# TrungMasterChef/CSWin-SimAM-UNet

Hardware: AMD Instinct MI355X
Metric: images/sec at 512×512 bf16, 1/2/4/8 MI355X; Dice parity vs reference (higher is better)
Workload: dtype bf16; 1 GPU; CSWin-UNet train step 512x512 depth [1, 2, 9, 1] split [1, 2, 8, 8] +SimAM, AdamW; model=CSWinTransformer, params=23567980, global_batch=16, per_gpu_batch=16, img=512, parallelism=dp1, workload_key=cswin|d1,2,9,1|s1,2,8,8|simam|bf16|512|16

## Files before the change

### cswin-simam-unet_amd/csrc/conv.hip

```cpp
#include <cstdlib>

#include "common.hpp"
#include "lds_dma.hpp"

namespace csu {
namespace {

constexpr int NT = 256;
constexpr int TBM = 64, TBN = 64, TBK = 32;

template <typename T> struct CT;
template <> struct CT<bf16> { static constexpr int AS = TBK; };
template <> struct CT<float> { static constexpr int AS = TBK + 4; };

__device__ __forceinline__ int cswz(int row, int col) {
    return row * TBK + ((((col >> 3) ^ (row >> 2)) & 3) << 3) + (col & 7);
}

struct Geo {
    int B, H, W, C, OH, OW, N, KH, KW, s, p;
};

template <int MODE>
__device__ __forceinline__ long gather_index(const Geo& g, long m, int k, long Mrows) {
// ... 1630 lines not shown
    if (!dy || !w_ihwo || !dx) return fail(CSU_E_ARG, "conv2d_dgrad: null buffer");
    const Geo g = to_geo(gm);
    const long M = (long)g.B * g.H * g.W;
    const int K = g.KH * g.KW * g.N;
    const bool vec = g.N % 8 == 0;
    hipStream_t st = as_stream(stream);
    if (dtype == CSU_BF16 && g.N % 4 == 0) {
        IG ph[4];
        int np = 0;
        for (int py = 0; py < g.s; ++py)
            for (int px = 0; px < g.s; ++px) {
                const IG ig = ig_dgrad_phase(*gm, py, px);
                if (ig.M == 0) continue;
                if (np == 4) {
                    if (int e = launch_ig(ph, np, dy, w_ihwo, bias, dx, st, cfg)) return e;
                    np = 0;
                }
                ph[np++] = ig;
            }
        if (np == 1) return launch_ig(ph, 1, dy, w_ihwo, bias, dx, st, cfg, (float*)ws, ws_bytes);
        return np ? launch_ig(ph, np, dy, w_ihwo, bias, dx, st, cfg) : 0;
    }
    if (cfg > 0) return fail(CSU_E_ARG, "conv2d_dgrad: igemm_dma needs bf16 with N % 64 == 0");
    if (dtype == CSU_BF16) return launch_gemm<bf16, 1>(g, M, g.C, K, dy, w_ihwo, bias, dx, vec, st);
    if (dtype == CSU_F32) return launch_gemm<float, 1>(g, M, g.C, K, dy, w_ihwo, bias, dx, vec, st);
    return fail(CSU_E_ARG, "conv2d_dgrad: bad dtype");
}

extern "C" int csu_conv2d_fwd(const csu_conv_geom* gm, int dtype, const void* x, const void* w_ohwi, const float* bias,
                              void* out, void* stream) {
    return conv_fwd_impl(gm, dtype, x, w_ohwi, bias, out, -1, stream);
}

extern "C" int csu_conv2d_dgrad(const csu_conv_geom* gm, int dtype, const void* dy, const void* w_ihwo,
                                const float* bias, void* dx, void* stream) {
    return conv_dgrad_impl(gm, dtype, dy, w_ihwo, bias, dx, -1, stream);
}

extern "C" size_t csu_conv2d_workspace(int op, const csu_conv_geom* gm, int dtype) {
    if (check_geo(gm) || dtype != CSU_BF16 || (op != 0 && op != 1)) return 0;
    if (op == 0) {
        if (gm->C % 4) return 0;
        const IG g = ig_forward(*gm);
        return id_pick(g, true) >= 0 ? 0 : ksplit_bytes(g, id_cus());
    }
    if (gm->N % 4 || gm->stride != 1) return 0;
    const IG g = ig_dgrad_phase(*gm, 0, 0);
    return id_pick(g, true) >= 0 ? 0 : ksplit_bytes(g, id_cus());
}

extern "C" int csu_conv2d_fwd_ws(const csu_conv_geom* gm, int dtype, const void* x, const void* w_ohwi, const float* bias,
                                 void* out, void* workspace, size_t ws_bytes, void* stream) {
    return conv_fwd_impl(gm, dtype, x, w_ohwi, bias, out, -1, stream, workspace, ws_bytes);
}

extern "C" int csu_conv2d_dgrad_ws(const csu_conv_geom* gm, int dtype, const void* dy, const void* w_ihwo, const float* bias,
                                   void* dx, void* workspace, size_t ws_bytes, void* stream) {
    return conv_dgrad_impl(gm, dtype, dy, w_ihwo, bias, dx, -1, stream, workspace, ws_bytes);
}

extern "C" int csu_conv2d_ex(int op, const csu_conv_geom* gm, int dtype, const void* src, const void* w, const float* bias,
                             void* out, int cfg, void* stream) {
    if (op == 0) return conv_fwd_impl(gm, dtype, src, w, bias, out, cfg, stream);
    if (op == 1) return conv_dgrad_impl(gm, dtype, src, w, bias, out, cfg, stream);
    return fail(CSU_E_ARG, "conv2d_ex: op must be 0 (forward) or 1 (input gradient)");
}

extern "C" size_t csu_conv2d_wgrad_workspace(const csu_conv_geom* gm) {
    if (check_geo(gm)) return 0;
    const size_t a = wgrad_ws(gm, -1);
    const int pk = wd_pick(gm, CSU_BF16, -1);
    const size_t b = pk >= 0 ? wgrad_ws(gm, pk) : 0;
    return a > b ? a : b;
}

extern "C" size_t csu_conv2d_wgrad_workspace_ex(const csu_conv_geom* gm, int cfg) {
    if (check_geo(gm)) return 0;
    if (cfg < 0) return csu_conv2d_wgrad_workspace(gm);
    const int pk = wd_pick(gm, CSU_BF16, cfg);
    return pk == -2 ? 0 : wgrad_ws(gm, pk);
}

static int conv_wgrad_impl(const csu_conv_geom* gm, int dtype, const void* x, const void* dy, int creal, float* dw_db,
                           void* workspace, size_t ws_bytes, int cfg, void* stream, const void* x2 = nullptr, int csplit = 0) {
    if (int e = check_geo(gm)) return e;
    if (!x || !dy || !dw_db) return fail(CSU_E_ARG, "conv2d_wgrad: null buffer");
    const int pick = wd_pick(gm, dtype, cfg);
    if (pick == -2) return fail(CSU_E_ARG, "conv2d_wgrad: configuration not eligible (bf16, C % 8 == 0, N % 8 == 0)");
    if (csplit && pick != kHalo64 && pick != kHalo128)
        return fail(CSU_E_UNSUPPORTED, "conv2d_wgrad: two-source input needs the halo kernel");
    if (!workspace || ws_bytes < wgrad_ws(gm, pick)) return fail(CSU_E_WORKSPACE, "conv2d_wgrad: workspace");
    if (creal > gm->C) return fail(CSU_E_ARG, "conv2d_wgrad: c_real > C");
    const Geo g = to_geo(gm);
    const long M = (long)g.B * g.OH * g.OW;
    const int K = g.KH * g.KW * g.C;
    const WPl p = wplan_any(gm, pick);
    const long used = (long)g.N * K + g.N;
    const long slab = (used + 3) & ~3L;
    float* part = (float*)workspace;
    const dim3 grid((g.N + TBN - 1) / TBN, (K + TBN - 1) / TBN, p.chunks);
    const bool vec = g.C % 8 == 0;
    hipStream_t st = as_stream(stream);
    if (pick >= 0) {
        wd_run(pick, g, M, g.N, K, p, x, dy, part, st, x2, csplit);
    } else if (dtype == CSU_BF16) {
        const bool small = (long)g.B * g.H * g.W * g.C * 2 < (1L << 31) && M * g.N * 2 < (1L << 31);
        if (vec && g.N % 8 == 0 && small)
            conv_wgrad_bf16<false><<<grid, NT, 0, st>>>(g, M, g.N, K, p.rpc, (const bf16*)x, (const bf16*)dy, part);
        else if (vec && g.N % 4 == 0 && small)
            conv_wgrad_bf16<true><<<grid, NT, 0, st>>>(g, M, g.N, K, p.rpc, (const bf16*)x, (const bf16*)dy, part);
        else if (vec) conv_wgrad_kernel<bf16, true><<<grid, NT, 0, st>>>(g, M, g.N, K, p.rpc, (const bf16*)x, (const bf16*)dy, part);
        else conv_wgrad_kernel<bf16, false><<<grid, NT, 0, st>>>(g, M, g.N, K, p.rpc, (const bf16*)x, (const bf16*)dy, part);
    } else if (dtype == CSU_F32) {
        if (vec) conv_wgrad_kernel<float, true><<<grid, NT, 0, st>>>(g, M, g.N, K, p.rpc, (const float*)x, (const float*)dy, part);
        else conv_wgrad_kernel<float, false><<<grid, NT, 0, st>>>(g, M, g.N, K, p.rpc, (const float*)x, (const float*)dy, part);
    } else {
        return fail(CSU_E_ARG, "conv2d_wgrad: bad dtype");
    }
    if (int e = check_launch("conv2d_wgrad")) return e;
    if (creal > 0) {
        const OutMap om{1, g.N, g.KH * g.KW, g.C, creal};
        return colsum_launch(p.chunks, slab, CSU_F32, part, dw_db, part + (size_t)p.chunks * slab, st, &om);
    }
    if (slab == used) return colsum_launch(p.chunks, slab, CSU_F32, part, dw_db, part + (size_t)p.chunks * slab, st);
    float* stage = part + (size_t)p.chunks * slab;
    if (int e = colsum_launch(p.chunks, slab, CSU_F32, part, stage, stage + slab, st)) return e;
    if (hipMemcpyAsync(dw_db, stage, used * sizeof(float), hipMemcpyDeviceToDevice, st) != hipSuccess)
        return fail(CSU_E_ARG, "conv2d_wgrad: copy-out failed");
    return 0;
}

extern "C" int csu_conv2d_wgrad(const csu_conv_geom* gm, int dtype, const void* x, const void* dy, float* dw_db,
                                void* workspace, size_t ws_bytes, void* stream) {
    return conv_wgrad_impl(gm, dtype, x, dy, 0, dw_db, workspace, ws_bytes, -1, stream);
}

extern "C" int csu_conv2d_wgrad_oihw(const csu_conv_geom* gm, int dtype, const void* x, const void* dy, int c_real,
                                     float* dw_db, void* workspace, size_t ws_bytes, void* stream) {
    if (c_real < 1) return fail(CSU_E_ARG, "conv2d_wgrad_oihw: c_real < 1");
    return conv_wgrad_impl(gm, dtype, x, dy, c_real, dw_db, workspace, ws_bytes, -1, stream);
}

extern "C" int csu_conv2d_wgrad_ex(const csu_conv_geom* gm, int dtype, const void* x, const void* dy, int c_real, float* dw_db,
                                   void* workspace, size_t ws_bytes, int cfg, void* stream) {
    if (c_real < 0) return fail(CSU_E_ARG, "conv2d_wgrad_ex: c_real < 0");
    return conv_wgrad_impl(gm, dtype, x, dy, c_real, dw_db, workspace, ws_bytes, cfg, stream);
}

extern "C" int csu_conv2d_split_ok(const csu_conv_geom* gm, int c_split) {
    if (check_geo(gm)) return 0;
    return c_split > 0 && c_split < gm->C && c_split % 64 == 0 && gm->C % 64 == 0 && gm->N % 64 == 0 &&
           (long)gm->B * gm->H * gm->W * gm->C * 2 < (1L << 31) && wd_pick(gm, CSU_BF16, -1) >= kHalo64;
}

extern "C" int csu_conv2d_fwd_split(const csu_conv_geom* gm, int dtype, const void* x, const void* x2, int c_split,
                                    const void* w_ohwi, const float* bias, void* y, void* stream) {
    if (int e = check_geo(gm)) return e;
    if (dtype != CSU_BF16 || !csu_conv2d_split_ok(gm, c_split)) return fail(CSU_E_UNSUPPORTED, "conv2d_fwd_split: not eligible");
    if (!x || !x2 || !w_ohwi || !y) return fail(CSU_E_ARG, "conv2d_fwd_split: null buffer");
    IG g = ig_forward(*gm);
    g.csplit = c_split;
    g.src2 = (const bf16*)x2;
    return launch_ig(g, x, w_ohwi, bias, y, as_stream(stream));
}

extern "C" int csu_conv2d_dgrad_split(const csu_conv_geom* gm, int dtype, const void* dy, const void* w_ihwo, void* dx, void* dx2,
                                      int c_split, void* stream) {
    if (int e = check_geo(gm)) return e;
    if (dtype != CSU_BF16 || !csu_conv2d_split_ok(gm, c_split)) return fail(CSU_E_UNSUPPORTED, "conv2d_dgrad_split: not eligible");
    if (!dy || !w_ihwo || !dx || !dx2) return fail(CSU_E_ARG, "conv2d_dgrad_split: null buffer");
    IG ph[4];
    int np = 0;
    for (int py = 0; py < gm->stride; ++py)
        for (int px = 0; px < gm->stride; ++px) {
            IG ig = ig_dgrad_phase(*gm, py, px);
            if (ig.M == 0) continue;
            ig.nsplit = c_split;
            ig.out2 = (bf16*)dx2;
            ph[np++] = ig;
        }
    return np ? launch_ig(ph, np, dy, w_ihwo, nullptr, dx, as_stream(stream)) : 0;
}

extern "C" int csu_conv2d_wgrad_split_oihw(const csu_conv_geom* gm, int dtype, const void* x, const void* x2, int c_split,
                                           const void* dy, float* dw_db, void* workspace, size_t ws_bytes, void* stream) {
    if (int e = check_geo(gm)) return e;
    if (dtype != CSU_BF16 || !csu_conv2d_split_ok(gm, c_split)) return fail(CSU_E_UNSUPPORTED, "conv2d_wgrad_split: not eligible");
    if (!x2) return fail(CSU_E_ARG, "conv2d_wgrad_split: null buffer");
    return conv_wgrad_impl(gm, dtype, x, dy, gm->C, dw_db, workspace, ws_bytes, -1, stream, x2, c_split);
}
```

### cswin-simam-unet_amd/csrc/glue.hip

```cpp
#include "common.hpp"

namespace csu {
namespace {

constexpr int NT = 256;

__device__ __forceinline__ void load8_any(int dt, const void* p, long e, float* v) {
    if (dt == CSU_BF16) load8((const bf16*)p + e, v);
    else load8((const float*)p + e, v);
}

__global__ __launch_bounds__(NT) void grad_join_kernel(long n8, int adt, const void* __restrict__ a, int bdt,
                                                       const void* __restrict__ b, float* __restrict__ out,
                                                       bf16* __restrict__ outb) {
    for (long g = (long)blockIdx.x * NT + threadIdx.x; g < n8; g += (long)gridDim.x * NT) {
        const long e = g * 8;
        float va[8], vb[8];
        load8_any(adt, a, e, va);
        if (b) {
            load8_any(bdt, b, e, vb);
#pragma unroll
            for (int j = 0; j < 8; ++j) va[j] += vb[j];
        }
        if (out) store8(out + e, va);
        if (outb) store8(outb + e, va);
    }
}

__device__ __forceinline__ float bce_term(float p, float t) {
    const float lp = fmaxf(logf(p), -100.f), lq = fmaxf(log1pf(-p), -100.f);
    return (t - 1.f) * lq - t * lp;
}

constexpr int BCE_BLOCKS = 1024;

__global__ __launch_bounds__(NT) void bce_partial(long n, const float* __restrict__ p, const float* __restrict__ t,
                                                  float* __restrict__ partial, int stats) {
    __shared__ float red[4][NT / 64];
    const long per = (n + gridDim.x - 1) / gridDim.x;
    const long b0 = (long)blockIdx.x * per, b1 = min(n, b0 + per);
    float s = 0.f, si = 0.f, sp = 0.f, st = 0.f;
    auto acc = [&](float pv, float tv) {
        s += bce_term(pv, tv);
        const float pr = pv > 0.5f ? 1.f : 0.f;
        si += pr * tv;
        sp += pr;
        st += tv;
    };
    if ((per & 3) == 0 && (n & 3) == 0) {
        for (long e = b0 + 4 * threadIdx.x; e < b1; e += 4 * NT) {
            float pv[4], tv[4];
            load4(p + e, pv);
            load4(t + e, tv);
#pragma unroll
            for (int j = 0; j < 4; ++j) acc(pv[j], tv[j]);
        }
    } else {
        for (long e = b0 + threadIdx.x; e < b1; e += NT) acc(p[e], t[e]);
    }
    const float v[4] = {s, si, sp, st};
    const int nk = stats ? 4 : 1;
    for (int k = 0; k < nk; ++k) {
        const float w = wave_sum(v[k]);
        if ((threadIdx.x & 63) == 0) red[k][threadIdx.x >> 6] = w;
    }
    __syncthreads();
    if (threadIdx.x < nk) {
        const int k = threadIdx.x;
        partial[(long)k * gridDim.x + blockIdx.x] = (red[k][0] + red[k][1]) + (red[k][2] + red[k][3]);
    }
}

__global__ __launch_bounds__(NT) void bce_final(int nb, long n, const float* __restrict__ partial, float* __restrict__ loss,
                                                float* __restrict__ stats) {
    __shared__ float red[NT / 64];
    const int nk = stats ? 4 : 1;
    for (int k = 0; k < nk; ++k) {
        float s = 0.f;
        for (int i = threadIdx.x; i < nb; i += NT) s += partial[(long)k * nb + i];
        s = wave_sum(s);
        if ((threadIdx.x & 63) == 0) red[threadIdx.x >> 6] = s;
        __syncthreads();
        if (threadIdx.x == 0) {
            const float tot = (red[0] + red[1]) + (red[2] + red[3]);
            if (k == 0) loss[0] = tot / (float)n;
            else stats[k - 1] = tot;
        }
        __syncthreads();
    }
}

__global__ __launch_bounds__(NT) void bce_backward(long n, const float* __restrict__ p, const float* __restrict__ t,
                                                   const float* __restrict__ dloss, float* __restrict__ dp) {
    const float g = dloss[0], inv = 1.f / (float)n;
    for (long e = (long)blockIdx.x * NT + threadIdx.x; e < n; e += (long)gridDim.x * NT) {
        const float pv = p[e];
        dp[e] = (g * (pv - t[e]) / fmaxf((1.f - pv) * pv, 1e-12f)) * inv;
    }
}

__global__ __launch_bounds__(NT) void pack_nhwc(long pixels, int C, int Cp, long hw, const float* __restrict__ x,
                                                bf16* __restrict__ y) {
    for (long q = (long)blockIdx.x * NT + threadIdx.x; q < pixels; q += (long)gridDim.x * NT) {
        const long b = q / hw, s = q - b * hw;
        const float* src = x + b * C * hw + s;
        for (int c0 = 0; c0 < Cp; c0 += 8) {
            bf16x8 v;
#pragma unroll
            for (int j = 0; j < 8; ++j) v[j] = (bf16)(c0 + j < C ? src[(long)(c0 + j) * hw] : 0.f);
            *reinterpret_cast<bf16x8*>(y + q * Cp + c0) = v;
        }
    }
}

unsigned grid_for(long work) {
    const long g = (work + NT - 1) / NT;
    return (unsigned)(g < 1 ? 1 : g > 8192 ? 8192 : g);
}

}
}

using namespace csu;

extern "C" int csu_grad_join(long n, int adtype, const void* a, int bdtype, const void* b, float* out, void* out_bf16,
                             void* stream) {
    if (n < 0 || !a || (!out && !out_bf16) || (n % 8))
        return fail(CSU_E_ARG, "grad_join: bad args (n must be a multiple of 8, one output at least)");
    if ((adtype != CSU_BF16 && adtype != CSU_F32) || (b && bdtype != CSU_BF16 && bdtype != CSU_F32))
        return fail(CSU_E_ARG, "grad_join: bad dtype");
    if (n == 0) return 0;
    grad_join_kernel<<<grid_for(n / 8), NT, 0, as_stream(stream)>>>(n / 8, adtype, a, bdtype, b, out, (bf16*)out_bf16);
    return check_launch("grad_join");
}

extern "C" size_t csu_bce_loss_workspace(long n) { return (size_t)4 * BCE_BLOCKS * sizeof(float); }

static int bce_fwd(long n, const float* p, const float* t, float* loss, float* stats, void* workspace, size_t ws_bytes,
                   void* stream) {
    if (n < 1 || !p || !t || !loss) return fail(CSU_E_ARG, "bce_loss_fwd: bad args");
    if (!workspace || ws_bytes < csu_bce_loss_workspace(n)) return fail(CSU_E_WORKSPACE, "bce_loss_fwd: workspace");
    const long want = (n + 4 * NT - 1) / (4 * NT);
    const int nb = (int)(want < BCE_BLOCKS ? want : BCE_BLOCKS);
    hipStream_t st = as_stream(stream);
    bce_partial<<<nb, NT, 0, st>>>(n, p, t, (float*)workspace, stats != nullptr);
    if (int e = check_launch("bce_loss_fwd")) return e;
    bce_final<<<1, NT, 0, st>>>(nb, n, (const float*)workspace, loss, stats);
    return check_launch("bce_loss_fwd");
}

extern "C" int csu_bce_loss_fwd(long n, const float* p, const float* t, float* loss, void* workspace, size_t ws_bytes,
                                void* stream) {
    return bce_fwd(n, p, t, loss, nullptr, workspace, ws_bytes, stream);
}

extern "C" int csu_bce_loss_fwd_stats(long n, const float* p, const float* t, float* loss, float* stats, void* workspace,
                                      size_t ws_bytes, void* stream) {
    if (!stats) return fail(CSU_E_ARG, "bce_loss_fwd_stats: null stats");
    return bce_fwd(n, p, t, loss, stats, workspace, ws_bytes, stream);
}

extern "C" int csu_bce_loss_bwd(long n, const float* p, const float* t, const float* dloss, float* dp, void* stream) {
    if (n < 1 || !p || !t || !dloss || !dp) return fail(CSU_E_ARG, "bce_loss_bwd: bad args");
    bce_backward<<<grid_for(n), NT, 0, as_stream(stream)>>>(n, p, t, dloss, dp);
    return check_launch("bce_loss_bwd");
}

extern "C" int csu_pack_nhwc_bf16(int B, int C, int H, int W, int Cp, const float* x, void* y, void* stream) {
    if (B < 1 || C < 1 || H < 1 || W < 1 || Cp < C || Cp % 8 || !x || !y) return fail(CSU_E_ARG, "pack_nhwc_bf16: bad args");
    const long pixels = (long)B * H * W;
    pack_nhwc<<<grid_for(pixels), NT, 0, as_stream(stream)>>>(pixels, C, Cp, (long)H * W, x, (bf16*)y);
    return check_launch("pack_nhwc_bf16");
}
```

### cswin-simam-unet_amd/csrc/reduce.hip

```cpp
#include "common.hpp"

namespace csu {
namespace {

constexpr int NT = 256;

__device__ __forceinline__ long out_index(const OutMap& m, long c) {
    if (!m.on) return c;
    const long k = (long)m.khw * m.C, w = (long)m.N * k;
    if (c >= w) return c < w + m.N ? (long)m.N * m.khw * m.creal + (c - w) : -1;
    const long n = c / k, rr = c - n * k, t = rr / m.C, ch = rr - t * m.C;
    return ch < m.creal ? (n * m.creal + ch) * m.khw + t : -1;
}

template <typename T>
__global__ __launch_bounds__(NT) void colsum_pass1(long rows, long cols, int tpr, long rows_per_chunk,
                                                   const T* __restrict__ in, float* __restrict__ out, OutMap om) {
    constexpr int V = 16 / sizeof(T);
    __shared__ float red[NT][V + 1];
    const int cl = threadIdx.x % tpr, rl = threadIdx.x / tpr, rpi = NT / tpr;
    const long c0 = ((long)blockIdx.x * tpr + cl) * V;
    const long r0 = (long)blockIdx.y * rows_per_chunk;
    const long r1 = min(rows, r0 + rows_per_chunk);
    float acc[V];
#pragma unroll
    for (int j = 0; j < V; ++j) acc[j] = 0.f;
    if (c0 < cols) {
        long r = r0 + rl;
        float a1[V], a2[V], a3[V];
#pragma unroll
        for (int j = 0; j < V; ++j) a1[j] = a2[j] = a3[j] = 0.f;
        for (; r + 3 * rpi < r1; r += 4 * rpi) {
            float v0[V], v1[V], v2[V], v3[V];
            if constexpr (V == 8) {
                load8(in + r * cols + c0, v0); load8(in + (r + rpi) * cols + c0, v1);
                load8(in + (r + 2 * rpi) * cols + c0, v2); load8(in + (r + 3 * rpi) * cols + c0, v3);
            } else {
                load4(in + r * cols + c0, v0); load4(in + (r + rpi) * cols + c0, v1);
                load4(in + (r + 2 * rpi) * cols + c0, v2); load4(in + (r + 3 * rpi) * cols + c0, v3);
            }
#pragma unroll
            for (int j = 0; j < V; ++j) { acc[j] += v0[j]; a1[j] += v1[j]; a2[j] += v2[j]; a3[j] += v3[j]; }
        }
        for (; r < r1; r += rpi) {
            float v[V];
            if constexpr (V == 8) load8(in + r * cols + c0, v); else load4(in + r * cols + c0, v);
#pragma unroll
            for (int j = 0; j < V; ++j) acc[j] += v[j];
        }
#pragma unroll
        for (int j = 0; j < V; ++j) acc[j] += (a1[j] + a2[j]) + a3[j];
    }
#pragma unroll
    for (int j = 0; j < V; ++j) red[threadIdx.x][j] = acc[j];
    __syncthreads();
    if (rl == 0 && c0 < cols) {
        for (int q = 1; q < rpi; ++q)
#pragma unroll
            for (int j = 0; j < V; ++j) acc[j] += red[q * tpr + cl][j];
        if (om.on) {
#pragma unroll
            for (int j = 0; j < V; ++j) {
                const long d = c0 + j < cols ? out_index(om, c0 + j) : -1;
                if (d >= 0) out[d] = acc[j];
            }
        } else {
            float* o = out + (long)blockIdx.y * cols + c0;
#pragma unroll
            for (int j = 0; j < V; ++j)
                if (c0 + j < cols) o[j] = acc[j];
        }
    }
}

__global__ __launch_bounds__(NT) void colsum_pass2(long cols, int nchunks, const float* __restrict__ part,
                                                   float* __restrict__ out, OutMap om) {
    __shared__ float red[8][33];
    const int cl = threadIdx.x & 31, lane = threadIdx.x >> 5;
    const long c = (long)blockIdx.x * 32 + cl;
    float s0 = 0.f, s1 = 0.f;
    if (c < cols) {
        int k = lane;
        for (; k + 8 < nchunks; k += 16) {
            s0 += part[(long)k * cols + c];
            s1 += part[(long)(k + 8) * cols + c];
        }
        if (k < nchunks) s0 += part[(long)k * cols + c];
    }
    red[lane][cl] = s0 + s1;
    __syncthreads();
    if (lane == 0 && c < cols) {
        float s = red[0][cl];
        for (int l = 1; l < 8; ++l) s += red[l][cl];
        const long d = out_index(om, c);
        if (d >= 0) out[d] = s;
    }
}

struct Plan {
    int tpr, colblocks, chunks;
    long rpc;
};

Plan plan(long rows, long cols, int V) {
    Plan p;
    const long vecs = (cols + V - 1) / V;
    p.tpr = (int)(vecs >= 64 ? 64 : vecs);
    int t = 1;
    while (t < p.tpr) t <<= 1;
    p.tpr = t;
    p.colblocks = (int)((vecs + p.tpr - 1) / p.tpr);
    const int rpi = NT / p.tpr;
    long want = (rows + 8L * rpi - 1) / (8L * rpi);
    if (want > 256) want = 256;
    if (want < 1) want = 1;
    p.chunks = (int)want;
    p.rpc = (rows + p.chunks - 1) / p.chunks;
    return p;
}

}

size_t colsum_workspace(long rows, long cols, int dtype) {
    const Plan p = plan(rows, cols, dtype == CSU_BF16 ? 8 : 4);
    return p.chunks > 1 ? (size_t)p.chunks * cols * sizeof(float) : 0;
}

int colsum_launch(long rows, long cols, int dtype, const void* in, float* out, float* ws, hipStream_t st,
                  const OutMap* map) {
    const OutMap om = map ? *map : OutMap{0, 0, 0, 0, 0};
    const int V = dtype == CSU_BF16 ? 8 : 4;
    if (cols % V) return fail(CSU_E_ARG, "colsum: cols must be a multiple of 16 bytes");
    const Plan p = plan(rows, cols, V);
    float* dst = p.chunks > 1 ? ws : out;
    const dim3 grid(p.colblocks, p.chunks);
    if (dtype == CSU_BF16)
        colsum_pass1<bf16><<<grid, NT, 0, st>>>(rows, cols, p.tpr, p.rpc, (const bf16*)in, dst,
                                                             p.chunks > 1 ? OutMap{0, 0, 0, 0, 0} : om);
    else
        colsum_pass1<float><<<grid, NT, 0, st>>>(rows, cols, p.tpr, p.rpc, (const float*)in, dst,
                                                              p.chunks > 1 ? OutMap{0, 0, 0, 0, 0} : om);
    if (p.chunks > 1) colsum_pass2<<<(unsigned)((cols + 31) / 32), NT, 0, st>>>(cols, p.chunks, ws, out, om);
    return check_launch("colsum");
}

}

using namespace csu;

extern "C" size_t csu_colsum_workspace(long rows, long cols, int dtype) { return colsum_workspace(rows, cols, dtype); }

extern "C" int csu_colsum(long rows, long cols, int dtype, const void* in, float* out, void* workspace,
                          size_t ws_bytes, void* stream) {
    if (rows < 1 || cols < 1 || !in || !out) return fail(CSU_E_ARG, "colsum: bad args");
    if (dtype != CSU_F32 && dtype != CSU_BF16) return fail(CSU_E_ARG, "colsum: bad dtype");
    if (ws_bytes < colsum_workspace(rows, cols, dtype) || (colsum_workspace(rows, cols, dtype) && !workspace))
        return fail(CSU_E_WORKSPACE, "colsum: workspace too small");
    return colsum_launch(rows, cols, dtype, in, out, (float*)workspace, as_stream(stream));
}
```

### cswin-simam-unet_amd/csrc/wgrad.hip

```cpp
#include <cstdlib>
#include <type_traits>

#include "common.hpp"

namespace csu {
namespace {

constexpr int NT = 256;
constexpr int TM = 64;

#ifdef WG_TIMING
__device__ unsigned long long wg_ts[4][16384];
#define WG_STAMP(k) do { if (threadIdx.x < 1 && blockIdx.x < 16384) wg_ts[k][blockIdx.x + threadIdx.x] = __builtin_amdgcn_s_memrealtime(); } while (0)
__device__ unsigned long long wg_steps[4][64];
#define STEP_STAMP(k, i) do { if (blockIdx.x == 0 && threadIdx.x < 1 && (i) < 64) wg_steps[k][(i) + threadIdx.x] = __builtin_amdgcn_s_memtime(); } while (0)
#else
#define WG_STAMP(k) do {} while (0)
#define STEP_STAMP(k, i) do {} while (0)
#endif

constexpr int TN32 = 64, TK32 = 64, S32 = TM + 4;

__device__ __forceinline__ void stage_t32(const float* __restrict__ g, long M, int ld, int ncols, long m0, int c0,
                                          float* img) {
    for (int it = threadIdx.x; it < (TM / 2) * 16; it += NT) {
        const int pr = it / 16, q = it % 16;
        const long m = m0 + 2 * pr;
        const int c = c0 + q * 4;
        float a[4], b[4];
        const bool cv = c < ncols;
        if (cv && m < M) load4(g + m * ld + c, a); else for (int j = 0; j < 4; ++j) a[j] = 0.f;
        if (cv && m + 1 < M) load4(g + (m + 1) * ld + c, b); else for (int j = 0; j < 4; ++j) b[j] = 0.f;
#pragma unroll
        for (int j = 0; j < 4; ++j) {
            float* p = img + (q * 4 + j) * S32 + 2 * pr;
            p[0] = a[j];
            p[1] = b[j];
        }
    }
}

__global__ __launch_bounds__(NT) void wgrad_f32(long M, int N, int K, long rows_per_chunk, const float* __restrict__ dy,
                                                const float* __restrict__ x, float* __restrict__ part) {
    __shared__ __attribute__((aligned(16))) float At[TN32 * S32];
    __shared__ __attribute__((aligned(16))) float Bt[TK32 * S32];
    __shared__ float bred[NT];
    const int n0 = blockIdx.x * TN32, k0 = blockIdx.y * TK32;
    const long m_begin = (long)blockIdx.z * rows_per_chunk;
    const long m_end = min(M, m_begin + rows_per_chunk);
    const int lane = threadIdx.x & 63, wave = threadIdx.x >> 6;
    const int r = lane & 31, h = lane >> 5;
    const int wn = (wave >> 1) * 32, wk = (wave & 1) * 32;
    const bool do_bias = blockIdx.y == 0;
    f32x16 acc = {};
    float bsum = 0.f;
    for (long m0 = m_begin; m0 < m_end; m0 += TM) {
        __syncthreads();
        stage_t32(dy, m_end, N, N, m0, n0, At);
        stage_t32(x, m_end, K, K, m0, k0, Bt);
        __syncthreads();
        if (do_bias) {
            const int n = threadIdx.x & 63, qq = threadIdx.x >> 6;
#pragma unroll
            for (int j = 0; j < TM / 4; ++j) bsum += At[n * S32 + qq * (TM / 4) + j];
        }
#pragma unroll
        for (int t = 0; t < TM / 2; ++t)
            acc = __builtin_amdgcn_mfma_f32_32x32x2f32(At[(wn + r) * S32 + 2 * t + h], Bt[(wk + r) * S32 + 2 * t + h], acc,
                                                      0, 0, 0);
    }
    const long slab = (long)N * K + N;
    float* out = part + (long)blockIdx.z * slab;
#pragma unroll
    for (int reg = 0; reg < 16; ++reg) {
        const int n = n0 + wn + crow(reg, h), k = k0 + wk + r;
        if (n < N && k < K) out[(long)n * K + k] = acc[reg];
    }
    if (do_bias) {
        bred[threadIdx.x] = bsum;
        __syncthreads();
        if (threadIdx.x < 64 && n0 + threadIdx.x < N)
            out[(long)N * K + n0 + threadIdx.x] =
// ... 164 lines not shown
#pragma unroll
        for (int a = 0; a < C::AN; ++a)
#pragma unroll
            for (int b = 0; b < C::AK; ++b)
#pragma unroll
                for (int reg = 0; reg < 16; ++reg) {
                    const int n = n0 + wn + 32 * a + crow(reg, h), k = k0 + wk + 32 * b + r;
                    const unsigned off = (n < N && k < K) ? (unsigned)(n * K + k) * 4u : kOOB;
                    __builtin_amdgcn_raw_buffer_store_b32(__float_as_uint(acc[a][b][reg]), rd, off, 0, 0);
                }
    } else {
        float* o = slab + ((long)tile * chunks + chunk) * (TN * TK);
#pragma unroll
        for (int a = 0; a < C::AN; ++a)
#pragma unroll
            for (int b = 0; b < C::AK; ++b)
#pragma unroll
                for (int reg = 0; reg < 16; ++reg)
                    o[(wn + 32 * a + crow(reg, h)) * TK + wk + 32 * b + r] = acc[a][b][reg];
    }
    if (do_bias) {
        float* red = reinterpret_cast<float*>(lds);
#pragma unroll
        for (int j = 0; j < 8; ++j) red[threadIdx.x * 9 + j] = bsum[j];
        __syncthreads();
        if (threadIdx.x < TN) {
            const int g = threadIdx.x >> 3, j = threadIdx.x & 7;
            float sum = 0.f;
            for (int q = g; q < NTH; q += C::CPRA) sum += red[q * 9 + j];
            if (chunks == 1) {
                if (n0 + threadIdx.x < N) dst[(long)N * K + n0 + threadIdx.x] = sum;
            } else {
                float* bs = slab + (long)tiles * chunks * (TN * TK);
                bs[((long)ntile * chunks + chunk) * TN + threadIdx.x] = sum;
            }
        }
    }
    asm volatile("s_waitcnt vmcnt(0)" ::: "memory");
}

template <int TN, int TK, int D, int NTH = NT>
__global__ __launch_bounds__(NTH, D > 2 || NTH > NT ? 1 : 2) void wgrad_tile(long M, int N, int K, long rpc, int chunks,
                                                    const bf16* __restrict__ dy, const bf16* __restrict__ x,
                                                    float* __restrict__ dst, float* __restrict__ slab) {
    __shared__ __attribute__((aligned(16))) bf16 lds[2 * TileCfg<TN, TK, NTH>::BUF];
    WG_STAMP(0);
    const int t = __builtin_amdgcn_readfirstlane((int)xcd_tile(blockIdx.x, gridDim.x));
    wgrad_tile_body<TN, TK, D, NTH>(lds, t, M, N, K, rpc, chunks, dy, x, dst, slab);
    WG_STAMP(3);
}

constexpr int WGG_MAX = 48;
struct WgGroup {
    const bf16* dy[WGG_MAX];
    const bf16* x[WGG_MAX];
    float* dst[WGG_MAX];
    float* slab[WGG_MAX];
    int M[WGG_MAX], N[WGG_MAX], K[WGG_MAX], chunks[WGG_MAX], rpc[WGG_MAX], b0[WGG_MAX + 1];
    int count;
};

template <int TN, int TK, int NTH = NT, int D = 2>
__global__ __launch_bounds__(NTH, NTH > NT || TN * TK > 256 * 128 ? 1 : 2) void wgrad_group(WgGroup g) {
    __shared__ __attribute__((aligned(16))) bf16 lds[2 * TileCfg<TN, TK, NTH>::BUF];
    const int lt = __builtin_amdgcn_readfirstlane((int)xcd_tile(blockIdx.x, gridDim.x));
    int i = 0;
    while (i + 1 < g.count && g.b0[i + 1] <= lt) ++i;
    i = __builtin_amdgcn_readfirstlane(i);
    wgrad_tile_body<TN, TK, D, NTH>(lds, lt - g.b0[i], g.M[i], g.N[i], g.K[i], g.rpc[i], g.chunks[i], g.dy[i], g.x[i],
                                    g.dst[i], g.slab[i]);
}

__host__ __device__ inline int wslab_groups(int chunks) {
    int g = 1;
    while (g < 16 && g * 8 < chunks) g <<= 1;
    return g;
}
inline long wslab_blocks(int N, int K, int chunks) {
    const long quads = ((long)N * K + N) / 4, qb = NT / wslab_groups(chunks);
    return (quads + qb - 1) / qb;
}

__device__ __forceinline__ void wslab_sum(long blk, int N, int K, int TN, int TK, int chunks,
                                          const float* __restrict__ slab, float* __restrict__ dst) {
    __shared__ f32x4 red[NT];
    const int G = wslab_groups(chunks), QB = NT / G;
    const int g = threadIdx.x / QB, qi = threadIdx.x % QB;
    const long e = (blk * QB + qi) * 4;
    const long NK = (long)N * K;
    const int kt = (K + TK - 1) / TK, nt = (N + TN - 1) / TN;
    const long step = (long)TN * TK;
    const float* p = slab;
    long stride = 0;
    const bool valid = e < NK + N;
    if (e < NK) {
        const int n = (int)(e / K), k = (int)(e % K);
        const long tile = (long)(n / TN) * kt + k / TK;
        p = slab + tile * chunks * step + (long)(n % TN) * TK + (k % TK);
        stride = step;
    } else if (valid) {
        const int n = (int)(e - NK);
        p = slab + (long)nt * kt * chunks * step + ((long)(n / TN) * chunks) * TN + (n % TN);
        stride = TN;
    }
    f32x4 a0 = {}, a1 = {}, a2 = {}, a3 = {};
    if (valid) {
        int c = g;
        for (; c + 3 * G < chunks; c += 4 * G) {
            a0 += *reinterpret_cast<const f32x4*>(p + c * stride);
            a1 += *reinterpret_cast<const f32x4*>(p + (c + G) * stride);
            a2 += *reinterpret_cast<const f32x4*>(p + (c + 2 * G) * stride);
            a3 += *reinterpret_cast<const f32x4*>(p + (c + 3 * G) * stride);
        }
        for (; c < chunks; c += G) a0 += *reinterpret_cast<const f32x4*>(p + c * stride);
    }
    const f32x4 s = (a0 + a1) + (a2 + a3);
    if (G == 1) {
        if (valid) *reinterpret_cast<f32x4*>(dst + e) = s;
        return;
    }
    red[threadIdx.x] = s;
    __syncthreads();
    if (g == 0 && valid) {
        f32x4 t = red[qi];
        for (int j = 1; j < G; ++j) t += red[j * QB + qi];
        *reinterpret_cast<f32x4*>(dst + e) = t;
    }
}

__global__ __launch_bounds__(NT) void wslab_reduce(int N, int K, int TN, int TK, int chunks,
                                                   const float* __restrict__ slab, float* __restrict__ dst) {
    wslab_sum(blockIdx.x, N, K, TN, TK, chunks, slab, dst);
}

constexpr int WSB_MAX = 40;
struct WsBatch {
    const float* slab[WSB_MAX];
    float* dst[WSB_MAX];
    int N[WSB_MAX], K[WSB_MAX], tn[WSB_MAX], tk[WSB_MAX], chunks[WSB_MAX], b0[WSB_MAX + 1];
    int count;
};

__global__ __launch_bounds__(NT) void wslab_reduce_batch(WsBatch t) {
    const int b = blockIdx.x;
    int i = 0;
    while (i + 1 < t.count && t.b0[i + 1] <= b) ++i;
    wslab_sum(b - t.b0[i], t.N[i], t.K[i], t.tn[i], t.tk[i], t.chunks[i], t.slab[i], t.dst[i]);
}

int num_cus() {
    static int v = 0;
    if (!v) {
        int dev = 0, n = 0;
        if (hipGetDevice(&dev) == hipSuccess && hipDeviceGetAttribute(&n, hipDeviceAttributeMultiprocessorCount, dev) == hipSuccess
            && n > 0)
            v = n;
        else
            v = 256;
    }
    return v;
}

struct Plan {
    int tn, tk, nt, kt, chunks, depth;
    long rpc;
};

double model_us(long M, int N, int K, int tn, int tk, long c) {
    const long cus = num_cus();
    const long tiles = (long)((N + tn - 1) / tn) * ((K + tk - 1) / tk);
    const long rounds = (tiles * c + cus - 1) / cus;
    const double tile_us = (double)M * (tn + tk) * 2.0 / 70e3;
    double t = (double)rounds * (tile_us / (double)c + 3.0);
    if (c > 1) t += 2.0 + (double)c * ((double)N * K + N) * 8.0 / 8e6;
    return t;
}

Plan make_plan(long M, int N, int K, int tn, int tk, int chunks) {
    Plan p;
    if (tn == 256) {
        p.tn = 256;
        p.tk = 128;
        p.nt = (N + 255) / 256;
        p.kt = (K + 127) / 128;
        const long c = chunks > 0 ? chunks : 1;
        p.rpc = ((M + c - 1) / c + TM - 1) / TM * TM;
        p.chunks = (int)((M + p.rpc - 1) / p.rpc);
        p.depth = 2;
        return p;
    }
    double best = 1e30;
    p.tn = p.tk = 64;
    long want = 1;
    const int sizes[2] = {64, 128};
    for (int a = 0; a < 2; ++a)
        for (int b = 0; b < 2; ++b) {
            const int ctn = sizes[a], ctk = sizes[b];
            if ((tn > 0 && ctn != tn) || (tk > 0 && ctk != tk)) continue;
            if (tn <= 0 && tk <= 0 && ctn != ctk) continue;
            if ((ctn == 128 && N % 128) || (ctk == 128 && K % 128)) continue;
            const long tiles = (long)((N + ctn - 1) / ctn) * ((K + ctk - 1) / ctk);
            const long mintok = tiles <= 2 ? 2048 : 1024;
            const long maxc = chunks > 0 ? chunks : (M + mintok - 1) / mintok;
            for (long c = chunks > 0 ? chunks : 1; c <= maxc && c <= 4 * num_cus(); ++c) {
                const double t = model_us(M, N, K, ctn, ctk, c);
                if (t < best - 1e-9) {
                    best = t;
                    p.tn = ctn;
                    p.tk = ctk;
                    want = c;
                }
            }
        }
    p.nt = (N + p.tn - 1) / p.tn;
    p.kt = (K + p.tk - 1) / p.tk;
    if (want < 1) want = 1;
    p.rpc = ((M + want - 1) / want + TM - 1) / TM * TM;
    p.chunks = (int)((M + p.rpc - 1) / p.rpc);
    p.depth = 2;
    return p;
}

size_t plan_bytes(const Plan& p) {
    if (p.chunks == 1) return 0;
    return ((size_t)p.nt * p.kt * p.tn * p.tk + (size_t)p.nt * p.tn) * p.chunks * sizeof(float);
}

template <int TN, int TK>
void launch_tile(const Plan& p, unsigned grid, long M, int N, int K, const bf16* dy, const bf16* x, float* dst,
                 float* slab, hipStream_t st) {
// ... 75 lines not shown
    *item = csu_wslab_item{(const float*)workspace, dw_db, N, K, p.tn, p.tk, p.chunks, 0};
    return run_bf16(p, M, N, K, (const bf16*)dy, (const bf16*)x, dw_db, workspace, as_stream(stream), true);
}

constexpr int kSlabDiv = 32;
#ifndef WG_RECT
#define WG_RECT 1
#endif
static void group_plan(long M, int N, int K, int* tn, int* tk, int* chunks, long* rpc) {
    const int t = (N % 256 == 0 && K % 128 == 0) ? 256 : (N % 128 == 0 && K % 128 == 0) ? 128 : 64;
    long c = (long)((double)M * (N + K) / ((double)kSlabDiv * N * K) + 0.5);
    const long maxc = M / 1024 > 0 ? M / 1024 : 1;
    if (c > maxc) c = maxc;
    if (c < 1) c = 1;
    long r = ((M + c - 1) / c + TM - 1) / TM * TM;
    c = (M + r - 1) / r;
    *tn = t;
    *tk = t == 256 ? 128 : t;
    if (WG_RECT && t == 64) {
        if (N % 128 == 0) *tn = 128;
        else if (K % 128 == 0) *tk = 128;
    }
    *chunks = (int)c;
    *rpc = r;
}

extern "C" size_t csu_linear_wgrad_group_plan(long M, int N, int K, int* tn, int* tk, int* chunks) {
    int a, b, c;
    long r;
    group_plan(M, N, K, &a, &b, &c, &r);
    if (tn) *tn = a;
    if (tk) *tk = b;
    if (chunks) *chunks = c;
    if (c == 1) return 0;
    const long nt = (N + a - 1) / a, kt = (K + b - 1) / b;
    return ((size_t)nt * kt * a * b + (size_t)nt * a) * c * sizeof(float);
}

extern "C" int csu_linear_wgrad_group(const csu_wgrad_group_item* items, int count, void* stream) {
    if (count < 0 || (count && !items)) return fail(CSU_E_ARG, "linear_wgrad_group: bad args");
    hipStream_t st = as_stream(stream);
    constexpr int kPass[5][2] = {{256, 128}, {128, 128}, {128, 64}, {64, 128}, {64, 64}};
    for (int pass = 0; pass < 5; ++pass) {
        const int T = kPass[pass][0], TK = kPass[pass][1];
        WgGroup g;
        g.count = 0;
        g.b0[0] = 0;
        auto flush = [&]() -> int {
            if (!g.count) return 0;
            if (T == 256) wgrad_group<256, 128, 2 * NT><<<(unsigned)g.b0[g.count], 2 * NT, 0, st>>>(g);
            else if (T == 128 && TK == 128) wgrad_group<128, 128><<<(unsigned)g.b0[g.count], NT, 0, st>>>(g);
            else if (T == 128) wgrad_group<128, 64><<<(unsigned)g.b0[g.count], NT, 0, st>>>(g);
            else if (TK == 128) wgrad_group<64, 128><<<(unsigned)g.b0[g.count], NT, 0, st>>>(g);
            else wgrad_group<64, 64><<<(unsigned)g.b0[g.count], NT, 0, st>>>(g);
            g.count = 0;
            return check_launch("linear_wgrad_group");
        };
        for (int i = 0; i < count; ++i) {
            const csu_wgrad_group_item& it = items[i];
            if (it.M < 1 || it.N % 8 || it.K % 8 || !it.dy || !it.x || !it.dw_db)
                return fail(CSU_E_ARG, "linear_wgrad_group: bad item");
            int tn, tk, c;
            long r;
            group_plan(it.M, it.N, it.K, &tn, &tk, &c, &r);
            if (tn != T || tk != TK) continue;
            if (c > 1 && !it.slab) return fail(CSU_E_WORKSPACE, "linear_wgrad_group: item needs a slab workspace");
            const long tiles = (long)((it.N + tn - 1) / tn) * ((it.K + tk - 1) / tk);
            if (g.count == WGG_MAX || (long)g.b0[g.count] + tiles * c > (1L << 30))
                if (int e = flush()) return e;
            const int k = g.count;
            g.dy[k] = (const bf16*)it.dy;
            g.x[k] = (const bf16*)it.x;
            g.dst[k] = it.dw_db;
            g.slab[k] = it.slab;
            g.M[k] = (int)it.M; g.N[k] = it.N; g.K[k] = it.K; g.chunks[k] = c; g.rpc[k] = (int)r;
            g.b0[k + 1] = g.b0[k] + (int)(tiles * c);
            g.count = k + 1;
        }
        if (int e = flush()) return e;
    }
    return 0;
}

extern "C" int csu_wslab_reduce_batch(const csu_wslab_item* items, int count, void* stream) {
    if (count < 0 || (count && !items)) return fail(CSU_E_ARG, "wslab_reduce_batch: bad args");
    WsBatch t;
    t.count = 0;
    t.b0[0] = 0;
    auto flush = [&]() -> int {
        if (!t.count) return 0;
        wslab_reduce_batch<<<(unsigned)t.b0[t.count], NT, 0, as_stream(stream)>>>(t);
        t.count = 0;
        return check_launch("wslab_reduce_batch");
    };
    for (int i = 0; i < count; ++i) {
        const csu_wslab_item& it = items[i];
        if (it.chunks <= 1) continue;
        if (!it.slab || !it.dst || it.N % 4 || it.K % 4) return fail(CSU_E_ARG, "wslab_reduce_batch: bad item");
        const long blocks = wslab_blocks(it.N, it.K, it.chunks);
        if (t.count == WSB_MAX || (long)t.b0[t.count] + blocks > (1L << 30))
            if (int e = flush()) return e;
        const int c = t.count;
        t.slab[c] = it.slab;
        t.dst[c] = it.dst;
        t.N[c] = it.N; t.K[c] = it.K; t.tn[c] = it.tn; t.tk[c] = it.tk; t.chunks[c] = it.chunks;
        t.b0[c + 1] = t.b0[c] + (int)blocks;
        t.count = c + 1;
    }
    return flush();
}

#ifdef WG_TIMING
extern "C" int csu_debug_wgrad_ts(unsigned long long* host) {
    return (int)hipMemcpyFromSymbol(host, HIP_SYMBOL(csu::wg_ts), sizeof(csu::wg_ts), 0, hipMemcpyDeviceToHost);
}
extern "C" int csu_debug_wgrad_steps(unsigned long long* host) {
    return (int)hipMemcpyFromSymbol(host, HIP_SYMBOL(csu::wg_steps), sizeof(csu::wg_steps), 0, hipMemcpyDeviceToHost);
}
#endif
```

### cswin-simam-unet_amd/csu/_lib.py

```python
from __future__ import annotations

import ctypes
import os
import threading

import torch

LIB_PATH = os.environ.get("CSU_LIB_PATH") or os.path.join(os.path.dirname(os.path.abspath(__file__)), "_lib", "libcsu_hip.so")

c_int32, c_float, c_void_p, c_size_t = ctypes.c_int32, ctypes.c_float, ctypes.c_void_p, ctypes.c_size_t

CSU_F32, CSU_BF16 = 0, 1


class StripeBranch(ctypes.Structure):
    _fields_ = [("H_sp", c_int32), ("W_sp", c_int32), ("ch_off", c_int32), ("_pad", c_int32),
                ("lepe_w", c_void_p), ("lepe_b", c_void_p), ("lepe_dw", c_void_p), ("lepe_db", c_void_p)]


class StripeArgs(ctypes.Structure):
    _fields_ = [("B", c_int32), ("reso", c_int32), ("C", c_int32), ("heads", c_int32), ("head_dim", c_int32),
                ("nbranch", c_int32), ("scale", c_float), ("_pad", c_int32), ("br", StripeBranch * 2),
                ("drop_rng", c_void_p), ("drop_site", ctypes.c_uint32), ("drop_p", c_float)]


class LnParamItem(ctypes.Structure):
    _fields_ = [("workspace", c_void_p), ("dgamma", c_void_p), ("dbeta", c_void_p), ("rows", c_int32), ("C", c_int32),
                ("nblocks", c_int32), ("_pad", c_int32)]


class WslabItem(ctypes.Structure):
    _fields_ = [("slab", c_void_p), ("dst", c_void_p), ("N", c_int32), ("K", c_int32), ("tn", c_int32), ("tk", c_int32),
                ("chunks", c_int32), ("_pad", c_int32)]


class WgradGroupItem(ctypes.Structure):
    _fields_ = [("dy", c_void_p), ("x", c_void_p), ("dw_db", c_void_p), ("slab", c_void_p), ("M", ctypes.c_int64),
                ("N", c_int32), ("K", c_int32)]


class LepeReduceItem(ctypes.Structure):
    _fields_ = [("part", c_void_p), ("dw", c_void_p * 2), ("db", c_void_p * 2), ("nblk", c_int32), ("channels", c_int32),
                ("nbranch", c_int32), ("_pad", c_int32)]


class MlpDropout(ctypes.Structure):
    _fields_ = [("rng", c_void_p), ("site_hidden", ctypes.c_uint32), ("site_out", ctypes.c_uint32), ("p", c_float),
                ("row_scale", c_void_p), ("rows_per_sample", ctypes.c_int64)]


class GemmDesc(ctypes.Structure):
    _fields_ = [("M", ctypes.c_int64), ("N", c_int32), ("K", c_int32), ("a", c_void_p), ("b", c_void_p),
                ("lda", c_int32), ("ldb", c_int32), ("b_trans", c_int32), ("a_gelu", c_int32), ("bias", c_void_p),
                ("gelu_aux", c_void_p), ("resid", c_void_p), ("out", c_void_p), ("gelu_out", c_void_p),
                ("ldc", c_int32), ("out_dtype", c_int32), ("cfg", c_int32), ("_pad", c_int32)]


class HeadFold(ctypes.Structure):
    _fields_ = [("O", c_int32), ("w_out", c_void_p), ("b_out", c_void_p), ("w_h", c_void_p), ("dw_out", c_void_p),
                ("db_out", c_void_p), ("dw_h", c_void_p)]


class AugmentConfig(ctypes.Structure):
    _fields_ = [(n, c_float) for n in ("p_hflip", "p_vflip", "p_rot90", "p_rotate", "rotate_lo", "rotate_hi", "p_scale",
                                       "scale_lo", "scale_hi", "p_translate", "translate_x", "translate_y", "p_contrast",
                                       "contrast_lo", "contrast_hi", "p_brightness", "brightness_lo", "brightness_hi",
                                       "p_gamma", "gamma_lo", "gamma_hi", "p_noise", "noise_lo", "noise_hi", "p_elastic",
                                       "elastic_lo", "elastic_hi")] + [("spacing", c_int32)]


class ConvGeom(ctypes.Structure):
    _fields_ = [(n, c_int32) for n in ("B", "H", "W", "C", "OH", "OW", "N", "KH", "KW", "stride", "pad")]


_SIGS = {
    "csu_last_error_string": (ctypes.c_char_p, []),
    "csu_build_info": (ctypes.c_char_p, []),
    "csu_event_create": (ctypes.c_int, [ctypes.POINTER(c_void_p)]),
    "csu_event_destroy": (ctypes.c_int, [c_void_p]),
    "csu_event_record_ext": (ctypes.c_int, [c_void_p, c_void_p]),
    "csu_event_elapsed_ms": (ctypes.c_int, [c_void_p, c_void_p, ctypes.POINTER(c_float)]),
    "csu_stripe_attn_fwd": (ctypes.c_int, [ctypes.POINTER(StripeArgs), ctypes.c_int, c_void_p, c_void_p, c_void_p, c_void_p]),
    "csu_stripe_attn_bwd_workspace": (c_size_t, [ctypes.POINTER(StripeArgs)]),
    "csu_stripe_attn_bwd": (ctypes.c_int, [ctypes.POINTER(StripeArgs), ctypes.c_int, c_void_p, c_void_p, c_void_p,
                                           c_void_p, c_void_p, c_void_p, c_void_p, c_size_t, c_void_p]),
    "csu_layernorm_fwd": (ctypes.c_int, [ctypes.c_int, ctypes.c_int, c_float, ctypes.c_int, c_void_p, c_void_p, c_void_p,
                                         ctypes.c_int, c_void_p, c_void_p, c_void_p, c_void_p]),
    "csu_layernorm_bwd_workspace": (c_size_t, [ctypes.c_int, ctypes.c_int]),
    "csu_layernorm_bwd": (ctypes.c_int, [ctypes.c_int, ctypes.c_int, ctypes.c_int, c_void_p, c_void_p, c_void_p, c_void_p,
                                         ctypes.c_int, c_void_p, c_void_p, c_void_p, c_void_p, c_void_p, c_size_t,
                                         c_void_p]),
    "csu_layernorm_bwd_ex": (ctypes.c_int, [ctypes.c_int, ctypes.c_int, ctypes.c_int, c_void_p, c_void_p, c_void_p,
                                            c_void_p, ctypes.c_int, c_void_p, c_void_p, c_void_p, c_void_p, c_void_p,
                                            c_void_p, c_void_p, c_size_t, c_void_p]),
    "csu_simam_workspace": (c_size_t, [ctypes.c_int, ctypes.c_int, ctypes.c_int]),
    "csu_simam_fwd": (ctypes.c_int, [ctypes.c_int, ctypes.c_int, ctypes.c_int, c_float, ctypes.c_int, c_void_p, ctypes.c_int,
                                     c_void_p, c_void_p, c_void_p, c_size_t, c_void_p]),
    "csu_simam_bwd": (ctypes.c_int, [ctypes.c_int, ctypes.c_int, ctypes.c_int, ctypes.c_int, c_void_p, c_void_p, ctypes.c_int,
                                     c_void_p, c_void_p, c_void_p, c_size_t, c_void_p]),
    "csu_simam_fwd_fork": (ctypes.c_int, [ctypes.c_int, ctypes.c_int, ctypes.c_int, c_float, c_void_p, c_void_p, c_void_p,
                                          c_void_p, c_void_p, c_size_t, c_void_p]),
    "csu_simam_bwd_join": (ctypes.c_int, [ctypes.c_int, ctypes.c_int, ctypes.c_int, c_void_p, c_void_p, ctypes.c_int,
                                          c_void_p, c_void_p, c_void_p, c_void_p, c_void_p, c_size_t, c_void_p]),
    "csu_carafe_fwd": (ctypes.c_int, [ctypes.c_int] * 6 + [c_void_p] * 5),
    "csu_carafe_bwd": (ctypes.c_int, [ctypes.c_int] * 6 + [c_void_p] * 6),
    "csu_carafe_head_fwd": (ctypes.c_int, [ctypes.c_int] * 6 + [c_void_p] * 7),
    "csu_carafe_head_bwd_workspace": (c_size_t, [ctypes.c_int] * 5),
    "csu_carafe_head_bwd": (ctypes.c_int, [ctypes.c_int] * 6 + [c_void_p] * 11 + [c_size_t, c_void_p]),
    "csu_carafe_head_bwd_fold": (ctypes.c_int, [ctypes.c_int] * 6 + [c_void_p] * 9 + [ctypes.POINTER(HeadFold), c_void_p,
                                                                                     c_size_t, c_void_p]),
    "csu_head_fold_fwd": (ctypes.c_int, [ctypes.c_int, ctypes.c_int] + [c_void_p] * 6),
    "csu_head_fwd": (ctypes.c_int, [ctypes.c_long, ctypes.c_int, ctypes.c_int, c_void_p, c_void_p, c_void_p, c_void_p]),
    "csu_head_bwd_workspace": (c_size_t, [ctypes.c_long, ctypes.c_int]),
    "csu_head_bwd": (ctypes.c_int, [ctypes.c_long, ctypes.c_int, ctypes.c_int] + [c_void_p] * 7 + [c_size_t, c_void_p]),
    "csu_colsum_workspace": (c_size_t, [ctypes.c_long, ctypes.c_long, ctypes.c_int]),
    "csu_colsum": (ctypes.c_int, [ctypes.c_long, ctypes.c_long, ctypes.c_int, c_void_p, c_void_p, c_void_p, c_size_t,
                                  c_void_p]),
    "csu_linear_wgrad_workspace": (c_size_t, [ctypes.c_long, ctypes.c_int, ctypes.c_int]),
    "csu_linear_wgrad": (ctypes.c_int, [ctypes.c_long, ctypes.c_int, ctypes.c_int, ctypes.c_int, c_void_p, c_void_p,
                                        c_void_p, c_void_p, c_size_t, c_void_p]),
    "csu_linear_wgrad_tuned_workspace": (c_size_t, [ctypes.c_long, ctypes.c_int, ctypes.c_int, ctypes.c_int, ctypes.c_int,
                                                    ctypes.c_int]),
    "csu_linear_wgrad_tuned": (ctypes.c_int, [ctypes.c_long, ctypes.c_int, ctypes.c_int, ctypes.c_int, c_void_p, c_void_p,
                                              c_void_p, c_void_p, c_size_t, ctypes.c_int, ctypes.c_int, ctypes.c_int,
                                              c_void_p]),
    "csu_gemm": (ctypes.c_int, [ctypes.c_long, ctypes.c_int, ctypes.c_int, c_void_p, ctypes.c_int, c_void_p, ctypes.c_int,
                                ctypes.c_int, ctypes.c_int, c_void_p, c_void_p, c_void_p, c_void_p, ctypes.c_int,
                                ctypes.c_int, c_void_p]),
    "csu_cast_bf16_batch": (ctypes.c_int, [c_void_p, ctypes.c_int, ctypes.c_long, c_void_p]),
    "csu_adamw_chunk_elems": (ctypes.c_long, []),
    "csu_adamw_step": (ctypes.c_int, [c_void_p, ctypes.c_int, ctypes.c_long, c_void_p, c_float, c_float, c_float, c_float,
                                      c_float, c_void_p, c_float, c_void_p]),
    "csu_adam_l2_step": (ctypes.c_int, [c_void_p, ctypes.c_int, ctypes.c_long, c_void_p, c_float, c_float, c_float, c_float,
                                      c_float, c_void_p, c_float, c_void_p]),
    "csu_grad_norm_workspace": (c_size_t, [ctypes.c_long]),
    "csu_grad_sumsq": (ctypes.c_int, [c_void_p, ctypes.c_int, ctypes.c_long, c_void_p, c_void_p]),
    "csu_grad_norm_finish": (ctypes.c_int, [c_void_p, ctypes.c_long, c_float, c_void_p, c_void_p]),
    "csu_grad_scale": (ctypes.c_int, [c_void_p, ctypes.c_int, ctypes.c_long, c_void_p, c_void_p]),
    "csu_adamw_step_ex": (ctypes.c_int, [c_void_p, ctypes.c_int, ctypes.c_long, c_void_p, c_float, c_float, c_float,
                                         c_float, c_float, c_void_p, c_float, c_void_p, ctypes.c_int, ctypes.c_int,
                                         c_void_p]),
    "csu_adamw_step_ema": (ctypes.c_int, [c_void_p, ctypes.c_int, ctypes.c_long, c_void_p, c_float, c_float, c_float,
                                          c_float, c_float, c_void_p, c_float, c_void_p, ctypes.c_int, ctypes.c_int,
                                          c_void_p, c_void_p, c_float, ctypes.c_int, c_void_p]),
    "csu_ema_update": (ctypes.c_int, [c_void_p, c_void_p, ctypes.c_int, ctypes.c_long, c_void_p, c_float, ctypes.c_int,
                                      c_void_p]),
    "csu_ema_swap": (ctypes.c_int, [c_void_p, c_void_p, ctypes.c_int, ctypes.c_long, c_void_p]),
    "csu_gemm_ex": (ctypes.c_int, [ctypes.POINTER(GemmDesc), c_void_p]),
    "csu_mlp_fwd_ln": (ctypes.c_int, [ctypes.c_long, ctypes.c_int] + [c_void_p] * 8 + [c_void_p, c_void_p, c_float, c_void_p,
                                                                               c_void_p, c_void_p, c_void_p]),
    "csu_gemm_ws_supported": (ctypes.c_int, [ctypes.c_long, ctypes.c_int, ctypes.c_int, ctypes.c_int, ctypes.c_int]),
    "csu_gemm_ws": (ctypes.c_int, [ctypes.c_long, ctypes.c_int, ctypes.c_int, c_void_p, ctypes.c_int, c_void_p, c_void_p,
                                   c_void_p, ctypes.c_int, c_void_p, c_void_p]),
    "csu_gemm_ws_ln_supported": (ctypes.c_int, [ctypes.c_long, ctypes.c_int, ctypes.c_int]),
    "csu_gemm_ws_ln": (ctypes.c_int, [ctypes.c_long, ctypes.c_int, c_void_p, ctypes.c_int, c_void_p, c_void_p, c_void_p,
                                      c_void_p, c_void_p, c_void_p, c_float, c_void_p, c_void_p, c_void_p, c_void_p]),
    "csu_gemm_ws_lnbwd_supported": (ctypes.c_int, [ctypes.c_long, ctypes.c_int, ctypes.c_int]),
    "csu_gemm_ws_lnbwd": (ctypes.c_int, [ctypes.c_long, ctypes.c_int, ctypes.c_int] + [c_void_p] * 11),
    "csu_frag_layout_batch": (ctypes.c_int, [c_void_p, ctypes.c_int, ctypes.c_long, c_void_p]),
    "csu_frag8_layout_batch": (ctypes.c_int, [c_void_p, ctypes.c_int, ctypes.c_long, c_void_p]),
    "csu_gemm_ws_e4m3": (ctypes.c_int, [ctypes.c_long, ctypes.c_int, ctypes.c_int, c_void_p, ctypes.c_int, c_void_p,
                                        c_void_p, ctypes.c_int, c_void_p, c_void_p, ctypes.c_int, c_void_p, c_void_p]),
    "csu_gemm_ws_ln_e4m3": (ctypes.c_int, [ctypes.c_long, ctypes.c_int, c_void_p, ctypes.c_int, c_void_p, c_void_p,
                                           c_void_p, c_void_p, c_void_p, c_void_p, c_void_p, ctypes.c_float, c_void_p,
                                           c_void_p, c_void_p, c_void_p]),
    "csu_gemm_f32_workspace": (c_size_t, [ctypes.c_int, ctypes.c_long, ctypes.c_int, ctypes.c_long]),
    "csu_gemm_f32": (ctypes.c_int, [ctypes.c_int, ctypes.c_long, ctypes.c_int, ctypes.c_long, c_void_p, c_void_p, c_void_p,
                                    c_void_p, c_void_p, c_void_p, c_void_p, c_size_t, c_void_p]),
    "csu_quant_e4m3_batch": (ctypes.c_int, [c_void_p, ctypes.c_int, ctypes.c_long, c_void_p]),
    "csu_fp8_gemm": (ctypes.c_int, [ctypes.c_long, ctypes.c_int, ctypes.c_int] + [c_void_p] * 7),
    "csu_layernorm_fwd_fp8": (ctypes.c_int, [ctypes.c_int, ctypes.c_int, c_float, ctypes.c_int] + [c_void_p] * 8),
    "csu_layernorm_fwd_fp8_dq": (ctypes.c_int, [ctypes.c_int, ctypes.c_int, c_float, ctypes.c_int] + [c_void_p] * 9),
    "csu_dequant_e4m3_rows": (ctypes.c_int, [ctypes.c_long, ctypes.c_int, c_void_p, c_void_p, c_void_p, c_void_p]),
    "csu_e4m3_layout_batch": (ctypes.c_int, [c_void_p, ctypes.c_int, ctypes.c_long, c_void_p]),
    "csu_quant_e4m3_shadow_batch": (ctypes.c_int, [c_void_p, ctypes.c_int, ctypes.c_long, c_void_p]),
    "csu_mlp_fp8_supported": (ctypes.c_int, [ctypes.c_int]),
    "csu_mlp_fwd_ex": (ctypes.c_int, [ctypes.c_long, ctypes.c_int] + [c_void_p] * 7 + [ctypes.POINTER(MlpDropout), ctypes.c_int,
                                                                                       c_void_p]),
    "csu_mlp_bwd_ex": (ctypes.c_int, [ctypes.c_long, ctypes.c_int] + [c_void_p] * 8 + [ctypes.POINTER(MlpDropout), ctypes.c_int,
                                                                                       c_void_p]),
    "csu_mlp_fp8_fwd": (ctypes.c_int, [ctypes.c_long, ctypes.c_int] + [c_void_p] * 9 + [ctypes.POINTER(MlpDropout), c_void_p]),
    "csu_mlp_fp8_fwd_ln": (ctypes.c_int, [ctypes.c_long, ctypes.c_int] + [c_void_p] * 9 + [ctypes.POINTER(MlpDropout), c_void_p,
                                          c_void_p, c_float, c_void_p, c_void_p, c_void_p, c_void_p]),
    "csu_mlp_fp8_bwd": (ctypes.c_int, [ctypes.c_long, ctypes.c_int] + [c_void_p] * 11 + [ctypes.POINTER(MlpDropout),
                                                                                         c_void_p]),
    "csu_mlp_supported": (ctypes.c_int, [ctypes.c_int]),
    "csu_dropout_apply": (ctypes.c_int, [ctypes.c_long, ctypes.c_int, ctypes.c_int, c_void_p, c_void_p, ctypes.c_int,
                                         c_void_p, c_void_p, ctypes.c_long, c_void_p, ctypes.c_uint, c_float, c_void_p]),
    "csu_dropout_mask": (ctypes.c_int, [ctypes.c_long, c_void_p, ctypes.c_uint, c_float, c_void_p, c_void_p]),
    "csu_rng_advance": (ctypes.c_int, [c_void_p, c_void_p, c_void_p]),
    "csu_droppath_scale": (ctypes.c_int, [ctypes.c_long, c_void_p, ctypes.c_uint, c_float, c_void_p, c_void_p]),
    "csu_layernorm_param_reduce": (ctypes.c_int, [ctypes.c_int, ctypes.c_int, c_void_p, c_void_p, c_void_p, c_void_p]),
    "csu_layernorm_param_reduce_batch": (ctypes.c_int, [c_void_p, ctypes.c_int, c_void_p]),
    "csu_linear_wgrad_deferred": (ctypes.c_int, [ctypes.c_long, ctypes.c_int, ctypes.c_int, c_void_p, c_void_p, c_void_p,
                                                 c_void_p, c_size_t, ctypes.POINTER(WslabItem), c_void_p]),
    "csu_wslab_reduce_batch": (ctypes.c_int, [c_void_p, ctypes.c_int, c_void_p]),
    "csu_stripe_attn_bwd_ex": (ctypes.c_int, [ctypes.POINTER(StripeArgs), ctypes.c_int, c_void_p, c_void_p, c_void_p,
                                              c_void_p, c_void_p, c_void_p, c_void_p, c_size_t, ctypes.c_int, c_void_p]),
    "csu_stripe_lepe_nblk": (ctypes.c_int, [ctypes.POINTER(StripeArgs), ctypes.c_int]),
    "csu_stripe_lepe_reduce_batch": (ctypes.c_int, [c_void_p, ctypes.c_int, c_void_p]),
    "csu_linear_wgrad_group_plan": (c_size_t, [ctypes.c_long, ctypes.c_int, ctypes.c_int, ctypes.POINTER(ctypes.c_int),
                                               ctypes.POINTER(ctypes.c_int), ctypes.POINTER(ctypes.c_int)]),
    "csu_linear_wgrad_group": (ctypes.c_int, [c_void_p, ctypes.c_int, c_void_p]),
    "csu_augment_batch": (ctypes.c_int, [ctypes.c_int, ctypes.c_int, c_void_p, c_void_p, c_void_p, c_void_p, c_void_p,
                                         c_void_p]),
    "csu_augment_draw": (ctypes.c_int, [ctypes.POINTER(AugmentConfig)] + [ctypes.c_int] * 3 + [c_void_p, ctypes.c_uint,
                                                                                                ctypes.c_uint, c_void_p,
                                                                                                c_void_p, c_void_p]),
    "csu_augment_mean": (ctypes.c_int, [ctypes.c_int, ctypes.c_long] + [c_void_p] * 4),
    "csu_augment_warp": (ctypes.c_int, [ctypes.c_int] * 3 + [c_void_p] * 4 + [ctypes.c_int, c_void_p, c_void_p,
                                                                             ctypes.c_uint, ctypes.c_int, c_float,
                                                                             ctypes.c_int, ctypes.c_int, c_void_p, c_void_p,
                                                                             c_void_p]),
    "csu_tile_gather": (ctypes.c_int, [ctypes.c_int] * 5 + [c_void_p] * 4),
    "csu_tile_blend": (ctypes.c_int, [ctypes.c_int] * 7 + [c_void_p] + [ctypes.c_long] * 3 + [ctypes.c_int]
                       + [c_void_p] * 3 + [ctypes.c_int] * 4 + [c_void_p]),
    "csu_tile_finish": (ctypes.c_int, [ctypes.c_int] * 3 + [c_void_p] * 3 + [c_float] + [c_void_p] * 3),
    "csu_surface_workspace": (c_size_t, [ctypes.c_int] * 4),
    "csu_surface_metrics": (ctypes.c_int, [ctypes.c_int] * 7 + [c_void_p, ctypes.c_int, c_void_p] + [ctypes.c_double] * 4
                            + [c_void_p, c_size_t, c_void_p, ctypes.c_int, ctypes.c_int, c_void_p]),
    "csu_edt_workspace": (c_size_t, [ctypes.c_int] * 3),
    "csu_edt": (ctypes.c_int, [ctypes.c_int] * 4 + [c_void_p, ctypes.c_double, ctypes.c_double, c_void_p, c_size_t,
                                                    c_void_p, c_void_p]),
    "csu_signed_distance_workspace": (c_size_t, [ctypes.c_int] * 4),
    "csu_signed_distance": (ctypes.c_int, [ctypes.c_int] * 6 + [c_void_p] + [ctypes.c_double] * 3
                            + [c_void_p, c_size_t, c_void_p, ctypes.c_int, ctypes.c_int, c_void_p]),
    "csu_ccl_workspace": (c_size_t, [ctypes.c_int] * 3),
    "csu_ccl": (ctypes.c_int, [ctypes.c_int] * 4 + [c_void_p, ctypes.c_int, c_void_p, c_size_t] + [c_void_p] * 4),
    "csu_cc_filter_workspace": (c_size_t, [ctypes.c_int] * 3),
    "csu_cc_filter": (ctypes.c_int, [ctypes.c_int] * 4 + [c_void_p, ctypes.c_int, ctypes.c_int, c_void_p, ctypes.c_uint,
                                                          ctypes.c_int, ctypes.c_int, c_void_p, c_size_t, c_void_p, c_void_p]),
    "csu_bn_workspace": (c_size_t, [ctypes.c_long, ctypes.c_int]),
    "csu_bn_relu_fwd": (ctypes.c_int, [ctypes.c_long, ctypes.c_int, ctypes.c_int, c_void_p, c_void_p, c_void_p, c_void_p,
                                       c_void_p, c_float, c_float, ctypes.c_int, ctypes.c_int, c_void_p, c_void_p,
                                       c_void_p, c_size_t, c_void_p]),
    "csu_bn_relu_bwd": (ctypes.c_int, [ctypes.c_long, ctypes.c_int, ctypes.c_int, c_void_p, c_void_p, c_void_p, c_void_p,
                                       ctypes.c_int, ctypes.c_int, ctypes.c_int, c_void_p, c_void_p, c_void_p, c_void_p,
                                       c_void_p, c_size_t, c_void_p]),
    "csu_maxpool2_fwd": (ctypes.c_int, [ctypes.c_int] * 5 + [c_void_p, c_void_p, c_void_p]),
    "csu_maxpool2_bwd": (ctypes.c_int, [ctypes.c_int] * 5 + [c_void_p, ctypes.c_int, c_void_p, c_void_p, c_void_p]),
    "csu_grad_join": (ctypes.c_int, [ctypes.c_long, ctypes.c_int, c_void_p, ctypes.c_int, c_void_p, c_void_p, c_void_p,
                                     c_void_p]),
    "csu_bce_loss_workspace": (c_size_t, [ctypes.c_long]),
    "csu_bce_loss_fwd": (ctypes.c_int, [ctypes.c_long, c_void_p, c_void_p, c_void_p, c_void_p, c_size_t, c_void_p]),
    "csu_bce_loss_fwd_stats": (ctypes.c_int, [ctypes.c_long] + [c_void_p] * 5 + [c_size_t, c_void_p]),
    "csu_bce_loss_bwd": (ctypes.c_int, [ctypes.c_long, c_void_p, c_void_p, c_void_p, c_void_p, c_void_p]),
    "csu_seg_loss_workspace": (c_size_t, [ctypes.c_long, ctypes.c_int]),
    "csu_seg_loss_fwd": (ctypes.c_int, [ctypes.c_long, ctypes.c_int, c_void_p, c_void_p] + [c_float] * 6
                         + [c_void_p] * 4 + [c_size_t, c_void_p]),
    "csu_seg_loss_bwd": (ctypes.c_int, [ctypes.c_long, ctypes.c_int] + [c_void_p] * 4 + [c_float] * 3 + [c_void_p, c_void_p]),
    "csu_seg_ce_workspace": (c_size_t, [ctypes.c_int, ctypes.c_int, ctypes.c_long]),
    "csu_seg_ce_fwd": (ctypes.c_int, [ctypes.c_int, ctypes.c_int, ctypes.c_long, ctypes.c_int, ctypes.c_int, c_void_p]
                       + [ctypes.c_long] * 3 + [ctypes.c_int, ctypes.c_int, c_void_p, ctypes.c_long, c_void_p]
                       + [c_float] * 5 + [ctypes.c_int] + [c_void_p] * 4 + [c_size_t, c_void_p]),
    "csu_seg_ce_bwd": (ctypes.c_int, [ctypes.c_int, ctypes.c_int, ctypes.c_long, ctypes.c_int, ctypes.c_int, c_void_p]
                       + [ctypes.c_long] * 3 + [ctypes.c_int, ctypes.c_int, c_void_p, ctypes.c_long, c_void_p]
                       + [c_void_p, c_void_p, c_float, c_float, ctypes.c_int, c_void_p, c_void_p]),
    "csu_seg_bd_workspace": (c_size_t, [ctypes.c_int, ctypes.c_int, ctypes.c_long]),
    "csu_seg_bd_fwd": (ctypes.c_int, [ctypes.c_int, ctypes.c_int, ctypes.c_long, ctypes.c_int, ctypes.c_int, c_void_p]
                       + [ctypes.c_long] * 3 + [ctypes.c_int, ctypes.c_int, c_void_p, ctypes.c_long, c_void_p]
                       + [c_float] * 5 + [ctypes.c_int, c_void_p, c_void_p, ctypes.c_int] + [c_void_p] * 5
                       + [c_size_t, c_void_p]),
    "csu_seg_bd_bwd": (ctypes.c_int, [ctypes.c_int, ctypes.c_int, ctypes.c_long, ctypes.c_int, ctypes.c_int, c_void_p]
                       + [ctypes.c_long] * 3 + [ctypes.c_int, ctypes.c_int, c_void_p, ctypes.c_long, c_void_p]
                       + [c_void_p, c_void_p, c_float, c_float, ctypes.c_int, c_void_p, c_void_p, ctypes.c_int, c_void_p,
                          c_void_p]),
    "csu_pack_nhwc_bf16": (ctypes.c_int, [ctypes.c_int, ctypes.c_int, ctypes.c_int, ctypes.c_int, ctypes.c_int, c_void_p,
                                          c_void_p, c_void_p]),
    "csu_stripe_lepe_wgrad": (ctypes.c_int, [ctypes.POINTER(StripeArgs), ctypes.c_int, c_void_p, c_void_p, c_void_p, c_size_t,
                                             c_void_p]),
    "csu_mlp_fwd": (ctypes.c_int, [ctypes.c_long, ctypes.c_int, c_void_p, c_void_p, c_void_p, c_void_p, c_void_p, c_void_p,
                                   c_void_p, c_void_p]),
    "csu_mlp_fwd_dp": (ctypes.c_int, [ctypes.c_long, ctypes.c_int, c_void_p, c_void_p, c_void_p, c_void_p, c_void_p, c_void_p,
                                      c_void_p, ctypes.POINTER(MlpDropout), c_void_p]),
    "csu_mlp_bwd_dp": (ctypes.c_int, [ctypes.c_long, ctypes.c_int, c_void_p, c_void_p, c_void_p, c_void_p, c_void_p, c_void_p,
                                      c_void_p, c_void_p, ctypes.POINTER(MlpDropout), c_void_p]),
    "csu_mlp_bwd_ln_supported": (ctypes.c_int, [ctypes.c_long, ctypes.c_int]),
    "csu_mlp_bwd_ln": (ctypes.c_int, [ctypes.c_long, ctypes.c_int] + [c_void_p] * 7 + [ctypes.c_long] + [c_void_p] * 9),
    "csu_mlp_bwd_wgrad_supported": (ctypes.c_int, [ctypes.c_int]),
    "csu_mlp_bwd_wgrad_workspace": (ctypes.c_int, [ctypes.c_long, ctypes.c_int, ctypes.POINTER(c_size_t),
                                                   ctypes.POINTER(c_size_t)]),
    "csu_mlp_bwd_wgrad": (ctypes.c_int, [ctypes.c_long, ctypes.c_int] + [c_void_p] * 6 + [ctypes.POINTER(MlpDropout), c_void_p,
                                                                                          c_void_p, ctypes.POINTER(WslabItem),
                                                                                          ctypes.POINTER(WslabItem), c_void_p,
                                                                                          c_void_p, c_void_p]),
    "csu_mlp_bwd": (ctypes.c_int, [ctypes.c_long, ctypes.c_int, c_void_p, c_void_p, c_void_p, c_void_p, c_void_p, c_void_p,
                                   c_void_p, c_void_p, c_void_p]),
    "csu_conv2d_fwd": (ctypes.c_int, [ctypes.POINTER(ConvGeom), ctypes.c_int, c_void_p, c_void_p, c_void_p, c_void_p,
                                      c_void_p]),
    "csu_conv2d_dgrad": (ctypes.c_int, [ctypes.POINTER(ConvGeom), ctypes.c_int, c_void_p, c_void_p, c_void_p, c_void_p,
                                        c_void_p]),
    "csu_conv2d_ex": (ctypes.c_int, [ctypes.c_int, ctypes.POINTER(ConvGeom), ctypes.c_int, c_void_p, c_void_p, c_void_p,
                                     c_void_p, ctypes.c_int, c_void_p]),
    "csu_conv2d_workspace": (c_size_t, [ctypes.c_int, ctypes.POINTER(ConvGeom), ctypes.c_int]),
    "csu_conv2d_fwd_ws": (ctypes.c_int, [ctypes.POINTER(ConvGeom), ctypes.c_int] + [c_void_p] * 5 + [c_size_t, c_void_p]),
    "csu_conv2d_dgrad_ws": (ctypes.c_int, [ctypes.POINTER(ConvGeom), ctypes.c_int] + [c_void_p] * 5 + [c_size_t, c_void_p]),
    "csu_conv2d_wgrad_workspace": (c_size_t, [ctypes.POINTER(ConvGeom)]),
    "csu_conv2d_wgrad_workspace_ex": (c_size_t, [ctypes.POINTER(ConvGeom), ctypes.c_int]),
    "csu_conv2d_split_ok": (ctypes.c_int, [ctypes.POINTER(ConvGeom), ctypes.c_int]),
    "csu_conv2d_fwd_split": (ctypes.c_int, [ctypes.POINTER(ConvGeom), ctypes.c_int, c_void_p, c_void_p, ctypes.c_int, c_void_p,
                                            c_void_p, c_void_p, c_void_p]),
    "csu_conv2d_dgrad_split": (ctypes.c_int, [ctypes.POINTER(ConvGeom), ctypes.c_int, c_void_p, c_void_p, c_void_p, c_void_p,
                                              ctypes.c_int, c_void_p]),
    "csu_conv2d_wgrad_split_oihw": (ctypes.c_int, [ctypes.POINTER(ConvGeom), ctypes.c_int, c_void_p, c_void_p, ctypes.c_int,
                                                   c_void_p, c_void_p, c_void_p, c_size_t, c_void_p]),
    "csu_conv2d_wgrad_ex": (ctypes.c_int, [ctypes.POINTER(ConvGeom), ctypes.c_int, c_void_p, c_void_p, ctypes.c_int,
                                           c_void_p, c_void_p, c_size_t, ctypes.c_int, c_void_p]),
    "csu_conv2d_wgrad": (ctypes.c_int, [ctypes.POINTER(ConvGeom), ctypes.c_int, c_void_p, c_void_p, c_void_p, c_void_p,
                                        c_size_t, c_void_p]),
    "csu_conv2d_wgrad_oihw": (ctypes.c_int, [ctypes.POINTER(ConvGeom), ctypes.c_int, c_void_p, c_void_p, ctypes.c_int,
                                             c_void_p, c_void_p, c_size_t, c_void_p]),
}

_lib = None
_lock = threading.Lock()


class CsuError(RuntimeError):
    pass


def lib():
    global _lib
    if _lib is None:
        with _lock:
            if _lib is None:
                if not os.path.exists(LIB_PATH):
                    raise CsuError(f"libcsu_hip.so not built ({LIB_PATH}); run `python __graft_entry__.py build` "
                                   "or `make -C cswin-simam-unet_amd/csrc`")
                L = ctypes.CDLL(LIB_PATH)
                for name, (res, args) in _SIGS.items():
                    fn = getattr(L, name)
                    fn.restype, fn.argtypes = res, args
                _lib = L
    return _lib


def check(rc: int, what: str):
    if rc != 0:
        msg = lib().csu_last_error_string().decode(errors="replace")
        raise CsuError(f"{what} failed (code {rc}): {msg}")


def dtype_code(t: torch.Tensor) -> int:
    if t.dtype == torch.float32:
        return CSU_F32
    if t.dtype == torch.bfloat16:
        return CSU_BF16
    raise CsuError(f"unsupported dtype {t.dtype} (float32 or bfloat16)")


def ptr(t):
    return None if t is None else ctypes.c_void_p(t.data_ptr())


def stream_ptr(device=None):
    return ctypes.c_void_p(torch.cuda.current_stream(device).cuda_stream)


def require_device(*ts: torch.Tensor):
    for t in ts:
        if t is not None and not t.is_cuda:
            raise CsuError("csu kernels run on the MI355X only: got a CPU tensor (there is no CPU fallback)")
```

### cswin-simam-unet_amd/csu/ops.py

```python
from __future__ import annotations

import ctypes
import os
import threading
import weakref
from typing import List, Optional, Sequence, Tuple

import torch

from . import _lib
from ._lib import CSU_BF16, CSU_F32, CsuError, check, dtype_code, lib, ptr, require_device, stream_ptr
from .ledger import esize, launch as _launch, prec_of


def _stripe_fwd_work(geom, B, esize):
    L = geom.reso * geom.reso
    nb = len(geom.branches)
    hs, ws, _ = geom.branches[0]
    N = hs * ws
    nbytes = B * L * (3 * geom.C + geom.C) * esize + nb * B * geom.heads * L * 4
    flops = B * L * nb * geom.heads * 4 * N * geom.head_dim + 18 * B * L * geom.C
    return nbytes, flops


# ... 182 lines not shown
            e = _USES.get(id(p))
            if e is not None and e[0]() is p:
                e[1] += 1
            else:
                _USES[id(p)] = [weakref.ref(p), 1]


def _uses(p) -> int:
    e = _USES.get(id(p))
    return e[1] if e is not None and e[0]() is p else 0


_LATE_DEFER: list = []
_LATE_SIDE: list = []
STATS = {"late_grad_fixups": 0}


def _late(params, grads, side: bool = False):
    lst = _LATE_SIDE if side else _LATE_DEFER
    for p, g in zip(params, grads):
        p = _leaf(p)
        if p is not None and g is not None:
            lst.append((weakref.ref(p), g.data_ptr(), g.untyped_storage(), g.storage_offset(), tuple(g.shape),
                        tuple(g.stride()), g.dtype))


def _check_late(lst):
    items, lst[:] = list(lst), []
    for pref, dptr, st, off, shape, stride, dt in items:
        p = pref()
        if p is None or p.grad is None or p.grad.data_ptr() == dptr:
            continue
        src = torch.empty(0, dtype=dt, device=p.grad.device).set_(st, off, shape, stride)
        p.grad.copy_(src)
        STATS["late_grad_fixups"] += 1


def take_late(params):
    want = {id(_leaf(p)) for p in params}
    out = []
    for lst in (_LATE_DEFER, _LATE_SIDE):
        keep = []
        for e in lst:
            p = e[0]()
            if p is not None and id(p) in want:
                pref, dptr, st, off, shape, stride, dt = e
                out.append((p, torch.empty(0, dtype=dt, device=st.device).set_(st, off, shape, stride)))
            else:
                keep.append(e)
        lst[:] = keep
    return out


def _reducer_hooks_only(hooks) -> bool:
    from .dist import GradAllReduce
    return all(getattr(h, "__func__", None) is GradAllReduce._hook for h in hooks.values())


def _deferrable(*params) -> bool:
    _queue_flush()
    if torch.is_grad_enabled():
        return False
    if not _DIST_SAFE[0]:
        dist = torch.distributed
        if dist.is_available() and dist.is_initialized() and dist.get_world_size() > 1:
            return False
    for p in params:
        p = _leaf(p)
        if p is None:
            continue
        if not p.is_leaf:
            return False
        if p.grad is not None or p._backward_hooks:
            return False
        hooks = getattr(p, "_post_accumulate_grad_hooks", None)
        if hooks and not _reducer_hooks_only(hooks):
            return False
        if _uses(p) > 1:
            return False
    return True


def deferred_pending() -> bool:
    return bool(_LN_PENDING or _WG_DEFER or _WG_PENDING or _WG_POST or _LEPE_PENDING)


def _ln_param_reduce(pend, nbytes):
    dev = pend[0][1].device
    items = (_lib.LnParamItem * len(pend))()
    for i, (work, dgb, rows, C, nblk) in enumerate(pend):
        items[i].workspace, items[i].dgamma, items[i].dbeta = work.data_ptr(), dgb.data_ptr(), dgb.data_ptr() + C * 4
        items[i].rows, items[i].C, items[i].nblocks = rows, C, nblk
    _launch("layernorm_bwd", lambda: lib().csu_layernorm_param_reduce_batch(items, len(pend), stream_ptr(dev)), 0, nbytes)


def _ln_param_flush():
    pend, _LN_PENDING[:] = list(_LN_PENDING), []
    if pend:
        _ln_param_reduce(pend, sum(e[0].numel() for e in pend) + sum(2 * e[3] for e in pend) * 4)


def _queue_flush():
    if not _LN_QUEUED[0] and torch._C._current_graph_task_id() != -1:
        torch.autograd.Variable._execution_engine.queue_callback(_end_of_backward_flush)
        _LN_QUEUED[0] = True


def _end_of_backward_flush():
    _LN_QUEUED[0] = False
    flush_deferred()
    _check_late(_LATE_DEFER)
    _USES.clear()


def flush_deferred():
    _ln_param_flush()
    _wgrad_flush()
    _lepe_flush()


_LEPE_PENDING: list = []


def _lepe_flush():
    pend, _LEPE_PENDING[:] = list(_LEPE_PENDING), []
    if not pend:
        return
    dev = pend[0][1].device
    items = (_lib.LepeReduceItem * len(pend))()
    nbytes = 0
    for i, (it, work, _) in enumerate(pend):
        items[i] = it
        nbytes += it.nbranch * it.channels * 10 * (it.nblk + 1) * 4
    _launch("stripe_attn_bwd", lambda: lib().csu_stripe_lepe_reduce_batch(items, len(pend), stream_ptr(dev)), 0, nbytes)


def _ln_params(ctx, rows, C, work, dgb, nblocks=0):
    if not (DEFER_LN and all(dt == torch.float32 for dt in ctx.pdtypes) and _deferrable(*ctx.params)):
        return False
    _LN_PENDING.append((work, dgb, rows, C, nblocks))
    _late(ctx.params, (dgb[:C], dgb[C:]))
    _queue_flush()
    return True


def _ln_param_grads(ctx, rows, C, work, nblk):
    dgb = _grad_dest(ctx.params)
    if dgb is None:
        dgb = torch.empty(2 * C, dtype=torch.float32, device=work.device)
    if not _ln_params(ctx, rows, C, work, dgb, nblocks=nblk):
        _ln_param_reduce([(work, dgb, rows, C, nblk)], work.numel() * 4 + 2 * C * 4)
    return dgb[:C].to(ctx.pdtypes[0]), dgb[C:].to(ctx.pdtypes[1])


DEFER_WGRAD = True
GROUP_WGRAD = True
_WG_PENDING: list = []
_WG_DEFER: list = []
_WG_POST: list = []


def _wgrad_flush():
    defer, _WG_DEFER[:] = list(_WG_DEFER), []
    if defer:
        L = lib()
        dev = defer[0][0].device
        gitems = (_lib.WgradGroupItem * len(defer))()
        keep, flops, nbytes = [], 0, 0
        for i, (dy2, x2, out) in enumerate(defer):
            M, N = dy2.shape
            K = x2.shape[1]
            tn, tk, ch = ctypes.c_int(), ctypes.c_int(), ctypes.c_int()
            nws = L.csu_linear_wgrad_group_plan(M, N, K, ctypes.byref(tn), ctypes.byref(tk), ctypes.byref(ch))
            slab = torch.empty(nws // 4, dtype=torch.float32, device=dev) if nws else None
            keep.append(slab)
            it = gitems[i]
            it.dy, it.x, it.dw_db, it.slab, it.M, it.N, it.K = dy2.data_ptr(), x2.data_ptr(), out.data_ptr(), \
                (slab.data_ptr() if slab is not None else None), M, N, K
            if ch.value > 1:
                w = _lib.WslabItem()
                w.slab, w.dst, w.N, w.K, w.tn, w.tk, w.chunks = slab.data_ptr(), out.data_ptr(), N, K, tn.value, tk.value, \
                    ch.value
                _WG_PENDING.append((w, out, slab))
            flops += 2 * M * N * K
            nbytes += M * (N + K) * 2 + (N * K + N) * 4
        _launch("linear_wgrad", lambda: L.csu_linear_wgrad_group(gitems, len(defer), stream_ptr(dev)), flops, nbytes)
    pend, _WG_PENDING[:] = list(_WG_PENDING), []
    if not pend:
        _wgrad_post()
        return
    dev = pend[0][1].device
    items = (_lib.WslabItem * len(pend))()
    nbytes = 0
    for i, (it, out, work) in enumerate(pend):
        items[i] = it
        nbytes += it.chunks * (it.N * it.K + it.N) * 4 + (it.N * it.K + it.N) * 4
    _launch("linear_wgrad", lambda: lib().csu_wslab_reduce_batch(items, len(pend), stream_ptr(dev)), 0, nbytes)
    _wgrad_post()


def _wgrad_post():
    post, _WG_POST[:] = list(_WG_POST), []
    for fn in post:
        fn()


def _wgrad_deferrable(dy2, wdt, bdt, params) -> bool:
    return (DEFER_WGRAD and dy2.dtype == torch.bfloat16 and bool(params) and wdt in (None, torch.float32)
            and bdt in (None, torch.float32) and _deferrable(*params))


def _ln_forward(x, weight, bias, eps, out_dtype, pre):
    C = x.shape[-1]
    rows = x.numel() // C
    w = _f32(weight)
    if pre is not None:
        return w, pre[3].view(x.shape), pre[4], pre[5]
    b = _f32(bias)
    y = torch.empty(x.shape, dtype=out_dtype, device=x.device)
    mean = torch.empty(rows, dtype=torch.float32, device=x.device)
    rstd = torch.empty(rows, dtype=torch.float32, device=x.device)
    _launch("layernorm_fwd", lambda: lib().csu_layernorm_fwd(rows, C, float(eps), dtype_code(x), ptr(x), ptr(w), ptr(b),
                                                             dtype_code(y), ptr(y), ptr(mean), ptr(rstd),
                                                             stream_ptr(x.device)),
            8 * rows * C, rows * C * (esize(x) + esize(y)) + rows * 8, prec=prec_of(x))
    return w, y, mean, rstd


class _LayerNormFn(torch.autograd.Function):
    @staticmethod
    def forward(ctx, x, weight, bias, eps: float, out_dtype, pre=None):
        require_device(x, weight, bias)
        x = x.contiguous()
        w, y, mean, rstd = _ln_forward(x, weight, bias, eps, out_dtype, pre)
        ctx.save_for_backward(x, w, mean, rstd)
        ctx.pdtypes = (weight.dtype, bias.dtype)
        ctx.params = (weight, bias)
        _note_use(ctx, *ctx.params)
        return y

    @staticmethod
    def backward(ctx, dy):
        x, w, mean, rstd = ctx.saved_tensors
        dx, dg, db = _ln_fork_backward(ctx, x, w, mean, rstd, None, dy)
        return dx, dg, db, None, None, None


def _ln_pre(x, weight, bias, eps, od):
    pre = getattr(x, "_csu_ln", None)
    if (pre is not None and pre[0] is weight and pre[1] is bias and pre[2] == float(eps) and pre[3].dtype == od
            and pre[3].numel() == x.numel() and x.is_contiguous() and pre[6] == x._version):
        return pre
    return None


def layer_norm(x: torch.Tensor, weight: torch.Tensor, bias: torch.Tensor, eps: float = 1e-5,
               out_dtype: Optional[torch.dtype] = None) -> torch.Tensor:
    od = out_dtype or x.dtype
    pre = _ln_pre(x, weight, bias, eps, od)
    if pre is not None:
        return _LayerNormFn.apply(x, weight, bias, eps, od, pre)
    return _LayerNormFn.apply(x, weight, bias, eps, od)


def _bf16_of(g: torch.Tensor) -> torch.Tensor:
    b = getattr(g, "_csu_bf16", None)
    if b is not None and b.shape == g.shape:
        return b
    return g.reshape(g.shape).to(torch.bfloat16).contiguous()


class _LayerNormForkFn(torch.autograd.Function):

    @staticmethod
    def forward(ctx, x, weight, bias, eps: float, out_dtype, pre=None):
        require_device(x, weight, bias)
        x = x.contiguous()
        w, y, mean, rstd = _ln_forward(x, weight, bias, eps, out_dtype, pre)
        ctx.save_for_backward(x, w, mean, rstd)
        ctx.pdtypes = (weight.dtype, bias.dtype)
        ctx.params = (weight, bias)
# ... 552 lines not shown
        _note_use(ctx, *ctx.params)
        return y

    @staticmethod
    def backward(ctx, dy):
        xc, wc = ctx.saved_tensors
        xdt, wdt, bdt = ctx.meta
        K, N = xc.shape[-1], dy.shape[-1]
        if dy.dtype != wc.dtype and wc.dtype == torch.bfloat16:
            dy2 = _bf16_of(dy).reshape(-1, N)
        else:
            dy2 = dy.reshape(-1, N)
            if dy2.dtype != wc.dtype:
                dy2 = dy2.to(wc.dtype)
        dy2 = dy2.contiguous()
        dx = dw = db = None
        if ctx.needs_input_grad[0]:
            if ctx.fast:
                odt = xdt if xdt in (torch.float32, torch.bfloat16) else wc.dtype
                dx = _token_gemm(dy2, wc, ctx.wtf, K, odt).view(xc.shape)
            else:
                dx = gemm_f32(1, dy2, wc.contiguous(), dy2.shape[0], K, N).view(xc.shape)
            if dx.dtype != xdt:
                dx = dx.to(xdt)
        vec = 16 // dy2.element_size()
        if N % vec == 0 and K % vec == 0 and dy2.dtype in (torch.float32, torch.bfloat16):
            dw, db = _linear_param_grads(ctx.needs_input_grad[1:3], dy2, xc.reshape(-1, K), wdt, bdt, ctx.params)
            return dx, dw, db, None, None, None
        if ctx.needs_input_grad[1] or (bdt is not None and ctx.needs_input_grad[2]):
            raise CsuError(f"linear backward: no csu weight-gradient kernel for {dy2.dtype} with in/out features "
                           f"{K}/{N}")
        return dx, dw, db, None, None, None


class _SharedCastFn(torch.autograd.Function):

    @staticmethod
    def forward(ctx, x, dtype):
        ctx.xdt = x.dtype
        if x.dtype == dtype:
            return x.view_as(x), x.view_as(x)
        if x.is_cuda and dtype == torch.bfloat16 and x.dtype == torch.float32 and x.numel() % 8 == 0:
            xc = x.contiguous()
            y = torch.empty(x.shape, dtype=dtype, device=x.device)
            n = x.numel()
            _launch("grad_join", lambda: lib().csu_grad_join(n, CSU_F32, ptr(xc), 0, None, None, ptr(y),
                                                             stream_ptr(x.device)), 0, n * 6, prec="f32")
        else:
            y = x.to(dtype)
        return y, y.view_as(y)

    @staticmethod
    def backward(ctx, g1, g2):
        if g1 is None and g2 is None:
            return None, None
        return grad_join(g1, g2, ctx.xdt), None


def grad_join(g1: Optional[torch.Tensor], g2: Optional[torch.Tensor], dtype: torch.dtype) -> torch.Tensor:
    a, b = (g1, g2) if g1 is not None else (g2, None)
    if dtype == torch.bfloat16 and a.is_cuda and a.numel() % 8 == 0 and b is not None:
        a, b = a.contiguous(), b.contiguous()
        outb = torch.empty(a.shape, dtype=torch.bfloat16, device=a.device)
        n = a.numel()
        _launch("grad_join", lambda: lib().csu_grad_join(n, dtype_code(a), ptr(a), dtype_code(b), ptr(b), None, ptr(outb),
                                                         stream_ptr(a.device)),
                n, n * (esize(a) + esize(b) + 2), prec="bf16")
        return outb
    if dtype != torch.float32 or not a.is_cuda or a.numel() % 8:
        g = a.to(dtype)
        return g.add_(b) if b is not None else g
    a = a.contiguous()
    b = b.contiguous() if b is not None else None
    out = torch.empty(a.shape, dtype=torch.float32, device=a.device)
    outb = torch.empty(a.shape, dtype=torch.bfloat16, device=a.device)
    n = a.numel()
    _launch("grad_join", lambda: lib().csu_grad_join(n, dtype_code(a), ptr(a), dtype_code(b) if b is not None else 0,
                                                     ptr(b), ptr(out), ptr(outb), stream_ptr(a.device)),
            n, n * (esize(a) + (esize(b) if b is not None else 0) + 6), prec="f32")
    out._csu_bf16 = outb
    return out


class _BCELossFn(torch.autograd.Function):

    @staticmethod
    def forward(ctx, p, t, with_stats: bool = False):
        p, t = p.contiguous(), t.contiguous()
        n = p.numel()
        loss = torch.empty((), dtype=torch.float32, device=p.device)
        stats = torch.empty(3, dtype=torch.float32, device=p.device) if with_stats else None
        nws = lib().csu_bce_loss_workspace(n)
        ws = torch.empty(nws // 4, dtype=torch.float32, device=p.device)
        if with_stats:
            _launch("bce_loss", lambda: lib().csu_bce_loss_fwd_stats(n, ptr(p), ptr(t), ptr(loss), ptr(stats), ptr(ws), nws,
                                                                     stream_ptr(p.device)), 12 * n, 8 * n, prec="f32")
        else:
            _launch("bce_loss", lambda: lib().csu_bce_loss_fwd(n, ptr(p), ptr(t), ptr(loss), ptr(ws), nws,
                                                               stream_ptr(p.device)), 8 * n, 8 * n, prec="f32")
        ctx.save_for_backward(p, t)
        if with_stats:
            ctx.mark_non_differentiable(stats)
            return loss, stats
        return loss

    @staticmethod
    def backward(ctx, g, *unused):
        p, t = ctx.saved_tensors
        g = g.float().contiguous()
        dp = torch.empty_like(p)
        n = p.numel()
        _launch("bce_loss_bwd", lambda: lib().csu_bce_loss_bwd(n, ptr(p), ptr(t), ptr(g), ptr(dp), stream_ptr(p.device)),
                6 * n, 12 * n, prec="f32")
        return dp, None, None


def bce_loss(prob: torch.Tensor, target: torch.Tensor) -> torch.Tensor:
    require_device(prob, target)
    if prob.dtype != torch.float32 or target.dtype != torch.float32 or prob.shape != target.shape:
        raise ValueError("bce_loss: fp32 probabilities and targets of one shape")
    return _BCELossFn.apply(prob, target)


def bce_loss_stats(prob: torch.Tensor, target: torch.Tensor) -> Tuple[torch.Tensor, torch.Tensor]:
    require_device(prob, target)
    if prob.dtype != torch.float32 or target.dtype != torch.float32 or prob.shape != target.shape:
        raise ValueError("bce_loss: fp32 probabilities and targets of one shape")
    return _BCELossFn.apply(prob, target, True)


class _SegLossFn(torch.autograd.Function):

    @staticmethod
    def forward(ctx, p, t, params, rows: int, with_stats: bool = False):
        p, t = p.contiguous(), t.contiguous()
        n = p.numel()
        w_bce, pos_weight, w_tv, alpha, beta, smooth = (float(v) for v in params)
        loss = torch.empty((), dtype=torch.float32, device=p.device)
        stats = torch.empty(3, dtype=torch.float32, device=p.device) if with_stats else None
        coef = torch.empty(rows, 2, dtype=torch.float32, device=p.device)
        nws = lib().csu_seg_loss_workspace(n, rows)
        ws = torch.empty(nws // 4, dtype=torch.float32, device=p.device)
        _launch("seg_loss", lambda: lib().csu_seg_loss_fwd(n, rows, ptr(p), ptr(t), w_bce, pos_weight, w_tv, alpha, beta,
                                                           smooth, ptr(loss), ptr(stats), ptr(coef), ptr(ws), nws,
                                                           stream_ptr(p.device)), 16 * n, 8 * n, prec="f32")
        ctx.save_for_backward(p, t, coef)
        ctx.seg = (rows, w_bce, pos_weight, w_tv)
        if with_stats:
            ctx.mark_non_differentiable(stats)
            return loss, stats
        return loss

    @staticmethod
    def backward(ctx, g, *unused):
        p, t, coef = ctx.saved_tensors
        rows, w_bce, pos_weight, w_tv = ctx.seg
        g = g.float().contiguous()
        dp = torch.empty_like(p)
        n = p.numel()
        _launch("seg_loss_bwd", lambda: lib().csu_seg_loss_bwd(n, rows, ptr(p), ptr(t), ptr(g), ptr(coef), w_bce, pos_weight,
                                                               w_tv, ptr(dp), stream_ptr(p.device)),
                10 * n, 12 * n, prec="f32")
        return dp, None, None, None, None


def seg_loss(prob: torch.Tensor, target: torch.Tensor, params, rows: int, with_stats: bool = False):
    require_device(prob, target)
    if prob.dtype != torch.float32 or target.dtype != torch.float32 or prob.shape != target.shape:
        raise ValueError("seg_loss: fp32 probabilities and targets of one shape")
    rows = int(rows)
    if rows < 1 or prob.numel() < 1 or prob.numel() % rows:
        raise ValueError("seg_loss: rows must divide the number of elements")
    if len(params) != 6:
        raise ValueError("seg_loss: params = (w_bce, pos_weight, w_tversky, alpha, beta, smooth)")
    return _SegLossFn.apply(prob, target, tuple(params), rows, bool(with_stats))


SEG_CE_MAX_CLASSES = 32


def _seg_ce_bucket(K: int) -> int:
    return 4 if K <= 4 else 8 if K <= 8 else 16 if K <= 16 else 32


def _seg_ce_layout(z: torch.Tensor):
    B, K = z.shape[0], z.shape[1]
    sp, n = z.stride(-1) if z.dim() > 2 else 1, 1
    ok = z.stride(0) >= 0 and z.stride(1) >= 1 and sp >= 1
    for d in range(z.dim() - 1, 1, -1):
        ok = ok and (z.shape[d] == 1 or z.stride(d) == sp * n)
        n *= z.shape[d]
    if not ok:
        z = z.contiguous()
        sp = 1
    sb, sk = z.stride(0), z.stride(1)
    KB = _seg_ce_bucket(K)
# ... 214 lines not shown
    from .augment import control_grid
    require_device(snap)
    if snap.dtype != torch.int64 or snap.numel() != 2:
        raise ValueError("augment_draw: snap is an int64 [seed, counter] snapshot (csu.rng)")
    B, H, W = int(B), int(H), int(W)
    site = rng.SITE_AUGMENT_DRAW if site is None else int(site)
    site_ctrl = rng.SITE_AUGMENT_CTRL if site_ctrl is None else int(site_ctrl)
    table = torch.empty(B, AUGMENT_P, dtype=torch.float32, device=snap.device)
    ctrl = None
    if elastic:
        if int(cfg.spacing) < 4:
            raise ValueError("augment_draw: elastic control-grid spacing must be >= 4 pixels")
        ctrl = torch.empty((B, 2) + control_grid(H, W, int(cfg.spacing)), dtype=torch.float32, device=snap.device)
    _launch("augment_draw", lambda: lib().csu_augment_draw(ctypes.byref(cfg), B, H, W, ptr(snap), site, site_ctrl,
                                                           ptr(table), ptr(ctrl), stream_ptr(snap.device)),
            0, 4 * (table.numel() + (ctrl.numel() if ctrl is not None else 0)), prec="f32")
    return table, ctrl


def augment_mean(images: torch.Tensor) -> torch.Tensor:
    require_device(images)
    if images.dtype != torch.uint8 or images.dim() < 2:
        raise ValueError("augment_mean: uint8 images (B, ...)")
    img = images.contiguous()
    B, n = img.shape[0], img[0].numel()
    sums = torch.empty(B, dtype=torch.int64, device=img.device)
    mean = torch.empty(B, dtype=torch.float32, device=img.device)
    _launch("augment_mean", lambda: lib().csu_augment_mean(B, n, ptr(img), ptr(sums), ptr(mean), stream_ptr(img.device)),
            0, B * n + 12 * B, prec="f32")
    return mean


def augment_warp(images: torch.Tensor, masks: torch.Tensor, table: torch.Tensor, ctrl: Optional[torch.Tensor] = None,
                 spacing: int = 0, mean: Optional[torch.Tensor] = None, snap: Optional[torch.Tensor] = None,
                 border: str = "constant", image_fill: float = 0.0, pad_label: int = 0, mask_mode: str = "bilinear",
                 out: str = "binary", noise_site: Optional[int] = None) -> Tuple[torch.Tensor, torch.Tensor]:
    from . import rng
    from .augment import control_grid
    require_device(images, masks, table, ctrl, mean, snap)
    if images.dtype != torch.uint8 or masks.dtype != torch.uint8:
        raise ValueError("augment_warp: uint8 images and masks")
    if images.dim() != 4 or images.shape[3] != 3 or tuple(masks.shape) != tuple(images.shape[:3]):
        raise ValueError("augment_warp: images (B, H, W, 3) and masks (B, H, W)")
    B, H, W = images.shape[:3]
    if table.dtype != torch.float32 or tuple(table.shape) != (B, AUGMENT_P):
        raise ValueError(f"augment_warp: table is fp32 (B, {AUGMENT_P})")
    if border not in AUGMENT_BORDERS or (mask_mode, out) not in AUGMENT_MASK_MODES:
        raise ValueError("augment_warp: border constant / replicate; mask_mode bilinear / nearest; out binary, or labels "
                         "with nearest")
    if not 0 <= int(pad_label) <= 255 and out != "labels":
        raise ValueError("augment_warp: pad_label outside 0..255 needs out='labels'")
    if ctrl is not None:
        spacing = int(spacing)
        if spacing < 4 or ctrl.dtype != torch.float32 or tuple(ctrl.shape) != (B, 2) + control_grid(H, W, spacing):
            raise ValueError("augment_warp: ctrl is fp32 (B, 2, ceil(H / spacing) + 3, ceil(W / spacing) + 3), spacing >= 4")
        ctrl = ctrl.contiguous()
    if snap is not None and (snap.dtype != torch.int64 or snap.numel() != 2):
        raise ValueError("augment_warp: snap is an int64 [seed, counter] snapshot (csu.rng)")
    img, msk, tab = images.contiguous(), masks.contiguous(), table.contiguous()
    if mean is None:
        mean = augment_mean(img)
    elif mean.dtype != torch.float32 or tuple(mean.shape) != (B,) or not mean.is_contiguous():
        raise ValueError("augment_warp: mean is a contiguous fp32 (B,)")
    mode = AUGMENT_MASK_MODES[(mask_mode, out)]
    oimg = torch.empty(B, 3, H, W, dtype=torch.float32, device=img.device)
    if out == "labels":
        om = torch.empty(B, H, W, dtype=torch.int64, device=img.device)
    else:
        om = torch.empty(B, 1, H, W, dtype=torch.float32, device=img.device)
    site = rng.SITE_AUGMENT_NOISE if noise_site is None else int(noise_site)
    _launch("augment_warp", lambda: lib().csu_augment_warp(B, H, W, ptr(img), ptr(msk), ptr(tab), ptr(ctrl), int(spacing),
                                                           ptr(mean), ptr(snap), site, AUGMENT_BORDERS[border],
                                                           float(image_fill), int(pad_label), mode, ptr(oimg), ptr(om),
                                                           stream_ptr(img.device)),
            0, B * H * W * (4 + 12 + om.element_size()), prec="f32")
    return oimg, om


def shared_cast(x: torch.Tensor, dtype: torch.dtype):
    return _SharedCastFn.apply(x, dtype)


def _concat_wgrad(dy2, a2, b2, defer: bool = False, dest=None):
    dwa, db = linear_wgrad(dy2, a2, defer=defer)
    dwb, _ = linear_wgrad(dy2, b2, defer=defer)
    if not defer:
        return torch.cat([dwa, dwb], 1), db
    N, K = dwa.shape[0], dwa.shape[1] + dwb.shape[1]
    if dest is None:
        buf = torch.empty(N * K, dtype=torch.float32, device=dy2.device)
        _WG_POST.append(lambda: torch.cat([dwa, dwb], 1, out=buf.view(N, K)))
        return buf.view(N, K), db

    def join():
        torch.cat([dwa, dwb], 1, out=dest[:N * K].view(N, K))
        dest[N * K:].copy_(db)
    _WG_POST.append(join)
    return dest[:N * K].view(N, K), dest[N * K:]


class _ConcatLinearFn(torch.autograd.Function):

    @staticmethod
    def forward(ctx, a, b, weight, bias, wc):
        Ca, Cb, N = a.shape[-1], b.shape[-1], weight.shape[0]
        a2 = a.reshape(-1, Ca).contiguous()
        b2 = b.reshape(-1, Cb).contiguous()
        bf = _f32(bias)
        y1 = gemm(a2, wc[:, :Ca], False, torch.float32, bias=bf)
        y = gemm(b2, wc[:, Ca:], False, torch.float32, resid=y1)
        ctx.save_for_backward(a2, b2, _weight_t(weight, wc))
        ctx.meta = (a.shape, b.shape, a.dtype, b.dtype, weight.dtype, bias.dtype)
        ctx.params = (weight, bias)
        _note_use(ctx, *ctx.params)
        return y.view(*a.shape[:-1], N)

    @staticmethod
    def backward(ctx, dy):
        a2, b2, wt = ctx.saved_tensors
        ashape, bshape, adt, bdt_in, wdt, bdt = ctx.meta
        Ca = a2.shape[1]
        dy2 = _bf16_of(dy).reshape(-1, dy.shape[-1]).contiguous()
        da = gemm(dy2, wt[:Ca], False, adt).view(ashape) if ctx.needs_input_grad[0] else None
        db_in = gemm(dy2, wt[Ca:], False, bdt_in).view(bshape) if ctx.needs_input_grad[1] else None
        if _wgrad_deferrable(dy2, wdt, bdt, ctx.params):
            dw, dbias = _concat_wgrad(dy2, a2, b2, defer=True, dest=_grad_dest(ctx.params))
            _late(ctx.params, (dw, dbias))
        elif _side_ok(dy2, wdt, bdt, params=ctx.params):
            dw, dbias = _side_run(lambda: _concat_wgrad(dy2, a2, b2), dy2, a2, b2)
            _late(ctx.params, (dw, dbias), side=True)
        else:
            dw, dbias = _concat_wgrad(dy2, a2, b2)
        return da, db_in, dw.to(wdt), dbias.to(bdt), None


def concat_linear(a: torch.Tensor, b: torch.Tensor, weight: torch.Tensor, bias: torch.Tensor) -> torch.Tensor:
    Ca, Cb, N = a.shape[-1], b.shape[-1], weight.shape[0]
    if fused_ok(a, Ca, Cb, N) and a.dtype == b.dtype == torch.bfloat16 and bias is not None:
        wc = _cached(weight, torch.bfloat16)
        if wc is None:
            wc = weight.to(torch.bfloat16)
        with torch.autocast("cuda", enabled=False):
            return _ConcatLinearFn.apply(a, b, weight, bias, wc)
    return linear(torch.cat([a, b], -1), weight, bias, out_dtype=torch.float32 if a.is_cuda else None)


class _LinearResidualFn(torch.autograd.Function):

    @staticmethod
    def forward(ctx, res, x, weight, bias, wc, ln=None):
        res2 = res.float().contiguous().view(-1, res.shape[-1])
        x2 = x.reshape(-1, x.shape[-1]).contiguous()
        M, K, N = x2.shape[0], x2.shape[1], wc.shape[0]
        bf = _f32(bias)
        wf = _ws_operand(weight)
        if (ln is not None and wf is not None and USE_GEMM_WS and K == N
                and lib().csu_gemm_ws_ln_supported(M, N, K)):
            gf, bf_, eps, h, mean, rstd, stash = _mlp_ln_side(ln, M, N, x2.device)
            y = torch.empty(M, N, dtype=torch.float32, device=x2.device)
            if isinstance(wf, tuple):
                wq, sc, _ = wf
                _launch("gemm", lambda: lib().csu_gemm_ws_ln_e4m3(M, N, ptr(x2), K, ptr(wq), ptr(sc), ptr(bf), ptr(res2),
                                                                  ptr(y), ptr(gf), ptr(bf_), eps, ptr(h), ptr(mean),
                                                                  ptr(rstd), stream_ptr(x2.device)),
                        2 * M * N * K + 8 * M * N, M * K * 2 + N * K + M * N * (4 + 4 + 2) + 8 * M,
                        tag=f"{M}x{N}x{K}rbln:ws8")
# ... 906 lines not shown
        return y.view(x.shape)

    @staticmethod
    def backward(ctx, dy):
        x, g, mean, rstd, h2, w1c, b1f, w2c = ctx.saved_tensors
        w1dt, b1dt, w2dt, b2dt = ctx.mmeta
        M, C = h2.shape
        dev = x.device
        dyb = _bf16_of(dy).reshape(M, C).contiguous()
        dres = dy.float().contiguous()
        dh = torch.empty(M, 4 * C, dtype=torch.bfloat16, device=dev)
        gl = torch.empty_like(dh)
        dx = torch.empty_like(x)
        dxb = torch.empty(x.shape, dtype=torch.bfloat16, device=dev)
        nblk = M // 64
        work = torch.empty(nblk * 2 * C, dtype=torch.float32, device=dev)
        _launch("mlp_bwd", lambda: lib().csu_mlp_bwd_ln(M, C, ptr(h2), ptr(dyb), ptr(w1c), ptr(b1f), ptr(w2c), ptr(dh), ptr(gl),
                                                        ctx.rpi, ptr(x), ptr(g), ptr(mean), ptr(rstd), ptr(dres), ptr(dx),
                                                        ptr(dxb), ptr(work), stream_ptr(dev)),
                24 * M * C * C + 12 * M * C,
                M * C * (2 + 2) + M * 4 * C * (2 + 2) + 16 * C * C + M * C * (4 + 4) + M * 8 + C * 4 + M * C * (4 + 2)
                + work.numel() * 4,
                prec="bf16", tag=f"{M}x{C}:lnbwd")
        dg, dbeta = _ln_param_grads(ctx, M, C, work, nblk)
        dw2, db2 = wgrad_maybe_side(dyb, gl, w2dt, b2dt, params=ctx.mlp[2:])
        dw1, db1 = wgrad_maybe_side(dh, h2, w1dt, b1dt, params=ctx.mlp[:2])
        dx._csu_bf16 = dxb
        return dx, dg, dbeta, None, dw1.to(w1dt), db1.to(b1dt), dw2.to(w2dt), db2.to(b2dt), None, None, None, None


FUSE_LN_MLP = os.environ.get("CSU_FUSE_LN_MLP", "1") != "0"


def ln_mlp_residual(x: torch.Tensor, ln: torch.nn.LayerNorm, fc1: torch.nn.Linear, fc2: torch.nn.Linear,
                    drop: Optional[MlpDrop] = None, ln_next=None):
    C = x.shape[-1]
    if not (FUSE_LN_MLP and FUSED_MLP and drop is None and _ACTIVE_FP8 is None and x.dtype == torch.float32
            and fused_ok(x, C, fc1.out_features)):
        return None
    if (fc1.out_features != 4 * C or fc2.in_features != 4 * C or ln.weight.numel() != C
            or ln.weight.dtype != torch.float32 or ln.bias.dtype != torch.float32):
        return None
    M = x.numel() // C
    if not (lib().csu_mlp_supported(C) and lib().csu_mlp_bwd_ln_supported(M, C)):
        return None
    lnn = _usable_ln_next(ln_next, C, FUSE_NEXT_LN)
    pre = _ln_pre(x, ln.weight, ln.bias, ln.eps, torch.bfloat16)
    return _apply_ln_stash(_LnMlpResidualFn, lnn, x, ln.weight, ln.bias, ln.eps, fc1.weight, fc1.bias, fc2.weight, fc2.bias,
                           _weight_bf16(fc1.weight), _weight_bf16(fc2.weight), pre, lnn)


FP8_QKV = os.environ.get("CSU_FP8_QKV", "0") != "0"


def ln_linear_fp8(x: torch.Tensor, ln: torch.nn.LayerNorm, lin: torch.nn.Linear):
    if _ACTIVE_FP8 is None or not x.is_cuda or not FP8_QKV:
        return None
    got = _ACTIVE_FP8.lookup(lin.weight)
    N, K = lin.weight.shape
    if got is None or N % 64 or K % 64 or K > 512:
        return None
    wc = _cached(lin.weight, torch.bfloat16)
    if wc is None:
        return None
    wt = _weight_t(lin.weight, wc)
    with torch.autocast("cuda", enabled=False):
        return _LnLinearFp8Fn.apply(x, ln.weight, ln.bias, lin.weight, lin.bias, ln.eps, got[0], got[1], wt)


def linear(x: torch.Tensor, weight: torch.Tensor, bias: Optional[torch.Tensor] = None,
           out_dtype: Optional[torch.dtype] = None) -> torch.Tensor:
    cd = _compute_dtype(x, weight)
    with torch.autocast("cuda", enabled=False):
        return _LinearFn.apply(x, weight, bias, cd, _cached(weight, cd), out_dtype)


def _conv_geom(B, H, W, C, N, KH, KW, stride, pad):
    g = _lib.ConvGeom()
    g.B, g.H, g.W, g.C, g.N, g.KH, g.KW, g.stride, g.pad = B, H, W, C, N, KH, KW, stride, pad
    g.OH, g.OW = (H + 2 * pad - KH) // stride + 1, (W + 2 * pad - KW) // stride + 1
    return g


def _conv_wgrad(g, x, dy, dt, c_real=None, out=None):
    L = lib()
    cr = g.C if c_real is None else c_real
    if out is None:
        out = torch.empty(g.N * g.KH * g.KW * cr + g.N, dtype=torch.float32, device=x.device)
    n = L.csu_conv2d_wgrad_workspace(ctypes.byref(g))
    work = torch.empty(max(n, 16), dtype=torch.uint8, device=x.device)
    _launch("conv_wgrad", lambda: L.csu_conv2d_wgrad_oihw(ctypes.byref(g), dt, ptr(x), ptr(dy), cr, ptr(out), ptr(work),
                                                          n, stream_ptr(x.device)),
            2 * g.B * g.OH * g.OW * g.N * g.KH * g.KW * g.C,
            (g.B * g.H * g.W * g.C + g.B * g.OH * g.OW * g.N) * x.element_size() + out.numel() * 4, prec=prec_of(x))
    k = g.N * g.KH * g.KW * cr
    return out[:k].view(g.N, cr, g.KH, g.KW), out[k:]


def _pad_channels(C: int) -> int:
    return (C + 7) // 8 * 8 if (C % 8 and PAD_CHANNELS) else C


def _conv_ws(op: int, g, t: torch.Tensor):
    n = lib().csu_conv2d_workspace(op, ctypes.byref(g), dtype_code(t))
    if not n:
        return None, 0
    return torch.empty(n, dtype=torch.uint8, device=t.device), n


class _Conv2dFn(torch.autograd.Function):
    @staticmethod
    def forward(ctx, x, weight, bias, stride: int, pad: int, cd):
        require_device(x, weight)
        B, H, W, C = x.shape
        N, Cw, KH, KW = weight.shape
        if Cw != C:
            raise ValueError(f"conv2d: input has {C} channels, weight expects {Cw}")
        cp = _pad_channels(C)
        if cp != C:
            xn = x.permute(0, 3, 1, 2)
            if cd == torch.bfloat16 and x.dtype == torch.float32 and xn.is_contiguous():
                xc = torch.empty(B, H, W, cp, dtype=cd, device=x.device)
                _launch("pack_nhwc", lambda: lib().csu_pack_nhwc_bf16(B, C, H, W, cp, ptr(xn), ptr(xc), stream_ptr(x.device)),
                        0, x.numel() * 4 + xc.numel() * 2, prec="f32")
            else:
                xc = torch.zeros(B, H, W, cp, dtype=cd, device=x.device)
                xc[..., :C] = x
            cached = _cached_conv(weight, cd)
            if cached is not None and cached[0].shape[-1] == cp:
                w_ohwi = cached[0]
            else:
                w_ohwi = torch.nn.functional.pad(weight.detach().permute(0, 2, 3, 1).to(cd), (0, cp - C)).contiguous()
            cached = None
        else:
            xc = (x if x.dtype == cd else x.to(cd)).contiguous()
            cached = _cached_conv(weight, cd)
            w_ohwi = cached[0] if cached else weight.detach().permute(0, 2, 3, 1).to(cd).contiguous()
        g = _conv_geom(B, H, W, cp, N, KH, KW, stride, pad)
        y = torch.empty(B, g.OH, g.OW, N, dtype=cd, device=x.device)
        bf = _f32(bias)
        ws, nws = _conv_ws(0, g, xc)
        _launch("conv_fwd", lambda: lib().csu_conv2d_fwd_ws(ctypes.byref(g), dtype_code(xc), ptr(xc), ptr(w_ohwi), ptr(bf),
                                                            ptr(y), ptr(ws), nws, stream_ptr(x.device)),
                2 * y.numel() * KH * KW * cp, (xc.numel() + w_ohwi.numel() + y.numel()) * xc.element_size(), prec=prec_of(xc))
        ctx.save_for_backward(xc, weight)
        ctx.w_ihwo = cached[1] if cached else None
        ctx.bias = bias
        _note_use(ctx, weight, bias)
        ctx.conf = (stride, pad, cd, x.dtype, bias is not None, None if bias is None else bias.dtype)
        return y

    @staticmethod
    def backward(ctx, dy):
        xc, weight = ctx.saved_tensors
        stride, pad, cd, xdt, has_b, bdt = ctx.conf
        B, H, W, cp = xc.shape
        N, C, KH, KW = weight.shape
        g = _conv_geom(B, H, W, cp, N, KH, KW, stride, pad)
        dy = dy.to(cd).contiguous()
        dx = None
        if ctx.needs_input_grad[0]:
            if cp != C:
                w_ihwo = torch.nn.functional.pad(weight.detach().permute(1, 2, 3, 0).to(cd), (0, 0, 0, 0, 0, 0, 0, cp - C))
                w_ihwo = w_ihwo.contiguous()
            else:
                w_ihwo = ctx.w_ihwo if ctx.w_ihwo is not None else weight.detach().permute(1, 2, 3, 0).to(cd).contiguous()
            dx = torch.empty(B, H, W, cp, dtype=cd, device=dy.device)
            ws, nws = _conv_ws(1, g, dy)
            _launch("conv_dgrad", lambda: lib().csu_conv2d_dgrad_ws(ctypes.byref(g), dtype_code(dy), ptr(dy), ptr(w_ihwo),
                                                                    None, ptr(dx), ptr(ws), nws, stream_ptr(dy.device)),
                    2 * dy.numel() * KH * KW * cp, (dy.numel() + w_ihwo.numel() + dx.numel()) * dy.element_size(),
                    prec=prec_of(dy))
            if cp != C:
                dx = dx[..., :C]
            if dx.dtype != xdt:
                dx = dx.to(xdt)

        dest = None
        if has_b and weight.dtype == torch.float32 and bdt == torch.float32:
            dest = _grad_dest((weight, ctx.bias))
            if dest is not None and dest.numel() != N * KH * KW * C + N:
                dest = None

        def wg():
            return _conv_wgrad(g, xc, dy, dtype_code(dy), C, out=dest)
        if _side_ok(dy, weight.dtype, bdt if has_b else None, params=(weight, ctx.bias)):
            dw, db = _side_run(wg, xc, dy)
            _late((weight, ctx.bias), (dw, db if has_b else None), side=True)
            return dx, dw, (db if has_b else None), None, None, None
        dw, db = wg()
        return dx, dw.to(weight.dtype), (db.to(bdt) if has_b else None), None, None, None


def conv2d(x_nhwc: torch.Tensor, weight: torch.Tensor, bias: Optional[torch.Tensor], stride: int = 1,
           pad: int = 0) -> torch.Tensor:
    cd = _compute_dtype(x_nhwc, weight)
    with torch.autocast("cuda", enabled=False):
        return _Conv2dFn.apply(x_nhwc, weight, bias, stride, pad, cd)


class _CatConv2dFn(torch.autograd.Function):

    @staticmethod
    def forward(ctx, xa, xb, weight, bias, pad: int, cd):
        require_device(xa, xb, weight)
        xa, xb = xa.to(cd).contiguous(), xb.to(cd).contiguous()
        B, H, W, Ca = xa.shape
        N, C, KH, KW = weight.shape
        g = _conv_geom(B, H, W, C, N, KH, KW, 1, pad)
        cached = _cached_conv(weight, cd)
        w_ohwi = cached[0] if cached else weight.detach().permute(0, 2, 3, 1).to(cd).contiguous()
        y = torch.empty(B, g.OH, g.OW, N, dtype=cd, device=xa.device)
        bf = _f32(bias)
        _launch("conv_fwd", lambda: lib().csu_conv2d_fwd_split(ctypes.byref(g), dtype_code(xa), ptr(xa), ptr(xb), Ca, ptr(w_ohwi),
                                                               ptr(bf), ptr(y), stream_ptr(xa.device)),
                2 * y.numel() * KH * KW * C, (xa.numel() + xb.numel() + w_ohwi.numel() + y.numel()) * 2, prec=prec_of(xa))
        ctx.save_for_backward(xa, xb, weight)
        ctx.w_ihwo = cached[1] if cached else None
        ctx.bias = bias
        _note_use(ctx, weight, bias)
        ctx.conf = (pad, cd, bias is not None, None if bias is None else bias.dtype)
        return y

    @staticmethod
    def backward(ctx, dy):
        xa, xb, weight = ctx.saved_tensors
        pad, cd, has_b, bdt = ctx.conf
        B, H, W, Ca = xa.shape
        N, C, KH, KW = weight.shape
        g = _conv_geom(B, H, W, C, N, KH, KW, 1, pad)
        dy = dy.to(cd).contiguous()
        dxa = dxb = None
        if ctx.needs_input_grad[0] or ctx.needs_input_grad[1]:
            w_ihwo = ctx.w_ihwo if ctx.w_ihwo is not None else weight.detach().permute(1, 2, 3, 0).to(cd).contiguous()
            dxa = torch.empty_like(xa)
            dxb = torch.empty_like(xb)
            _launch("conv_dgrad", lambda: lib().csu_conv2d_dgrad_split(ctypes.byref(g), dtype_code(dy), ptr(dy), ptr(w_ihwo),
                                                                       ptr(dxa), ptr(dxb), Ca, stream_ptr(dy.device)),
                    2 * dy.numel() * KH * KW * C, (dy.numel() + w_ihwo.numel() + dxa.numel() + dxb.numel()) * 2, prec=prec_of(dy))

        def wg():
            L = lib()
            out = torch.empty(N * KH * KW * C + N, dtype=torch.float32, device=dy.device)
            n = L.csu_conv2d_wgrad_workspace(ctypes.byref(g))
            work = torch.empty(max(n, 16), dtype=torch.uint8, device=dy.device)
            _launch("conv_wgrad", lambda: L.csu_conv2d_wgrad_split_oihw(ctypes.byref(g), dtype_code(dy), ptr(xa), ptr(xb), Ca,
                                                                        ptr(dy), ptr(out), ptr(work), n, stream_ptr(dy.device)),
                    2 * dy.numel() * KH * KW * C, (xa.numel() + xb.numel() + dy.numel()) * 2 + out.numel() * 4, prec=prec_of(dy))
            k = N * KH * KW * C
            return out[:k].view(N, C, KH, KW), out[k:]
        if _side_ok(dy, weight.dtype, bdt if has_b else None, params=(weight, ctx.bias)):
            dw, db = _side_run(wg, xa, xb, dy)
            _late((weight, ctx.bias), (dw, db if has_b else None), side=True)
            return dxa, dxb, dw, (db if has_b else None), None, None
        dw, db = wg()
        return dxa, dxb, dw.to(weight.dtype), (db.to(bdt) if has_b else None), None, None


def conv2d_cat(xa: torch.Tensor, xb: torch.Tensor, weight: torch.Tensor, bias: Optional[torch.Tensor],
               pad: int = 1) -> torch.Tensor:
    cd = _compute_dtype(xa, xb, weight)
    B, H, W, Ca = xa.shape
    N, C, KH, KW = weight.shape
    if Ca + xb.shape[-1] != C:
        raise ValueError(f"conv2d_cat: {Ca} + {xb.shape[-1]} input channels, weight expects {C}")
    g = _conv_geom(B, H, W, C, N, KH, KW, 1, pad)
    if cd == torch.bfloat16 and xa.is_cuda and lib().csu_conv2d_split_ok(ctypes.byref(g), Ca):
        with torch.autocast("cuda", enabled=False):
            return _CatConv2dFn.apply(xa, xb, weight, bias, pad, cd)
    return conv2d(torch.cat([xa.to(cd), xb.to(cd)], dim=-1), weight, bias, 1, pad)


# ... 49 lines not shown
```

### cswin-simam-unet_amd/csu/train.py

```python
from __future__ import annotations

from typing import Dict, List, Optional

import contextlib
import gc
import warnings

import torch
import torch.distributed as dist
import torch.nn.functional as F

try:
    from tqdm import tqdm
except ImportError:
    tqdm = None


def sync_shadows(model):
    from .ops import sync_shadows as sync
    sync(model)


def bce_loss(prob: torch.Tensor, target: torch.Tensor) -> torch.Tensor:
    with torch.autocast(prob.device.type, enabled=False):
        if prob.is_cuda:
            from . import ops
            return ops.bce_loss(prob.float(), target.float())
        return F.binary_cross_entropy(prob.float(), target.float())


def bce_loss_stats(prob: torch.Tensor, target: torch.Tensor):
    with torch.autocast(prob.device.type, enabled=False):
        if prob.is_cuda:
            from . import ops
            return ops.bce_loss_stats(prob.float(), target.float())
        p, t = prob.float(), target.float()
        pred = (p > 0.5).float()
        return F.binary_cross_entropy(p, t), torch.stack([(pred * t).sum(), pred.sum(), t.sum()]).detach()


def _dice_t(pred, target, smooth=1e-6):
    pred, target = pred.reshape(-1), target.reshape(-1)
    inter = (pred * target).sum()
    return (2.0 * inter + smooth) / (pred.sum() + target.sum() + smooth)


def _iou_t(pred, target, smooth=1e-6):
    pred, target = pred.reshape(-1), target.reshape(-1)
    inter = (pred * target).sum()
    return (inter + smooth) / (pred.sum() + target.sum() - inter + smooth)


def dice_coefficient(pred, target, smooth=1e-6) -> float:
    return _dice_t(pred, target, smooth).item()


def iou_score(pred, target, smooth=1e-6) -> float:
    return _iou_t(pred, target, smooth).item()


def _world():
    return dist.get_world_size() if dist.is_available() and dist.is_initialized() else 1


def _is_label_map(outputs, masks) -> bool:
    if masks.is_floating_point() or masks.dtype == torch.bool or outputs.dim() < 2:
        return False
    return masks.dim() == outputs.dim() - 1 or (masks.dim() == outputs.dim() and masks.shape[1] == 1 and outputs.shape[1] > 1)


def _step_stats(loss, outputs, masks):
    if _is_label_map(outputs, masks):
        K = outputs.shape[1]
        t = (masks[:, 0] if masks.dim() == outputs.dim() else masks).reshape(-1).long()
        o = outputs.detach().reshape(outputs.shape[0], K, -1)
        ar = torch.arange(K, device=o.device).view(1, K, 1)
        pred = torch.where(o == o.max(1, keepdim=True).values, ar, torch.full_like(ar, K)).min(1).values.reshape(-1)
        cls = torch.arange(K, device=o.device).view(K, 1)
        pm, tm = pred.view(1, -1) == cls, t.view(1, -1) == cls
        sums = torch.cat([(pm & tm).sum(1), pm.sum(1), tm.sum(1)])
        return torch.cat([loss.detach().double().view(1), sums.double()])
    preds = (outputs > 0.5).to(torch.float64).reshape(-1)
    t = masks.to(torch.float64).reshape(-1)
    return torch.stack([loss.detach().double(), (preds * t).sum(), preds.sum(), t.sum()])


def _epoch_means(stats: List[torch.Tensor], smooth: float = 1e-6, per_class: bool = False):
# ... 271 lines not shown
            criterion.on_epoch(epoch)
        if hasattr(criterion, "boundary_weight"):
            history["boundary_weight"].append(criterion.boundary_weight)
        model.train()
        sampler = getattr(train_loader, "sampler", None)
        if hasattr(sampler, "set_epoch"):
            sampler.set_epoch(epoch)
        it = train_loader
        if verbose and rank0 and tqdm is not None:
            it = tqdm(train_loader, desc=f"Epoch {epoch + 1}/{num_epochs} [TRAIN]")
        stats, norms = [], []
        skipped0 = getattr(optimizer, "skipped_steps", None)
        skipped0 = skipped0.clone() if isinstance(skipped0, torch.Tensor) else None
        for images, masks in it:
            images = images.to(device, non_blocking=True)
            masks = masks.to(device, non_blocking=True)
            if use_graph:
                key = ("train", tuple(images.shape), tuple(masks.shape), amp_dtype, criterion,
                       id(getattr(optimizer, "ema", None)), id(optimizer), id(reducer))
                g = cache.get(key)
                if g is None:
                    g = cache[key] = _GraphedTrain(model, optimizer, criterion, amp_dtype, reducer)
                stats.append(g(images, masks))
            else:
                stats.append(train_step(model, images, masks, criterion, optimizer, reducer, amp_dtype=amp_dtype))
            if clips and isinstance(getattr(optimizer, "grad_norm", None), torch.Tensor):
                norms.append(optimizer.grad_norm.detach().clone())
        train_loss, train_dice, train_iou, train_cd, train_ci = _epoch_means(stats, per_class=True)
        if clips:
            gn, sk = _clip_epoch(norms, optimizer, skipped0)
            history["grad_norm"].append(gn)
            history["skipped_steps"].append(sk)
        test_loss, test_dice, test_iou, test_cd, test_ci = evaluate_model(model, test_loader, criterion, device,
                                                                          amp_dtype=amp_dtype, graph=use_graph, per_class=True)
        ema_cd = ema_ci = None
        if ema is not None:
            with ema.applied():
                ema_loss, ema_dice, ema_iou, ema_cd, ema_ci = evaluate_model(
                    model, test_loader, criterion, device, amp_dtype=amp_dtype, graph=use_graph, per_class=True)
            for k, v in (("ema_test_loss", ema_loss), ("ema_test_dice", ema_dice), ("ema_test_iou", ema_iou)):
                history[k].append(v)
        if scheduler is not None:
            scheduler.step(test_loss)
            if hasattr(optimizer, "sync_lr"):
                optimizer.sync_lr()
        current_lr = optimizer.param_groups[0]["lr"]
        for k, v in zip(history, (train_loss, train_dice, train_iou, test_loss, test_dice, test_iou, current_lr)):
            history[k].append(v)
        for k, v in (("train_class_dice", train_cd), ("train_class_iou", train_ci), ("test_class_dice", test_cd),
                     ("test_class_iou", test_ci), ("ema_test_class_dice", ema_cd), ("ema_test_class_iou", ema_ci)):
            if v is not None:
                history.setdefault(k, []).append(v)
        if checkpoint_path is not None:
            from .report import save_checkpoint
            save_checkpoint(checkpoint_path, model, optimizer, scheduler, epoch + 1, history, ema=ema)
        if verbose and rank0:
            print(f'\n{"=" * 70}\nEpoch {epoch + 1}/{num_epochs}:')
            print(f"  [TRAIN] Loss: {train_loss:.4f} | Dice: {train_dice:.4f} | IoU: {train_iou:.4f}")
            print(f"  [TEST]  Loss: {test_loss:.4f} | Dice: {test_dice:.4f} | IoU: {test_iou:.4f}")
            print(f'  [LR]    Learning Rate: {current_lr:.6f}\n{"=" * 70}\n')
    return history


def make_optimizer(model, lr=1e-4, weight_decay=1e-4, capturable=False, max_grad_norm=None, skip_nonfinite=False,
                   ema_decay=None, ema_warmup=True):
    if max_grad_norm is not None and not float(max_grad_norm) > 0.0:
        raise ValueError(f"invalid max_grad_norm {max_grad_norm} (None: no clipping)")
    ema = None
    if ema_decay is not None:
        from .ema import WeightEMA
        ema = WeightEMA(model, decay=ema_decay, warmup=ema_warmup)
    if next(model.parameters()).is_cuda:
        from .optim import FusedAdamW
        return FusedAdamW(model.parameters(), lr=lr, weight_decay=weight_decay, capturable=capturable,
                          max_grad_norm=max_grad_norm, skip_nonfinite=skip_nonfinite, ema=ema)
    if skip_nonfinite:
        raise ValueError("make_optimizer(skip_nonfinite=True) needs csu.optim.FusedAdamW (a model on the GPU)")
    opt = torch.optim.AdamW(model.parameters(), lr=lr, weight_decay=weight_decay)
    opt.max_grad_norm = None if max_grad_norm is None else float(max_grad_norm)
    opt.ema = ema
    return opt


class GraphedTrainStep:

    def __init__(self, model, optimizer, criterion, example_x, example_t, autocast_dtype=None, warmup=3,
                 reducer=None, metrics=False, capture=True):
        self.model, self.opt, self.crit = model, optimizer, criterion
        self.metrics = metrics
        self.stats = None
        self.reducer = reducer
        self.x = example_x.clone()
        self.t = example_t.clone()
        self.dtype = autocast_dtype
        self.capture = bool(capture)
        self.graph = None
        if not self.capture:
            for _ in range(warmup):
                self._body()
            return
        side = torch.cuda.Stream()
        side.wait_stream(torch.cuda.current_stream())
        with warnings.catch_warnings(record=True) as caught:
            warnings.simplefilter("always")
            with torch.cuda.stream(side):
                for _ in range(warmup):
                    self._body()
        torch.cuda.current_stream().wait_stream(side)
        for w in caught:
            if "AccumulateGrad node's stream does not match" in str(w.message):
                raise RuntimeError(
                    "GraphedTrainStep: an autograd graph of an earlier step is still referenced (a kept "
                    "output or loss of an eager step); delete those references before capturing")
            warnings.warn_explicit(w.message, w.category, w.filename, w.lineno)
        torch.cuda.synchronize()
        mode = "global"
        if reducer is not None:
            from .dist import drain_collectives
            drain_collectives()
            mode = "thread_local"
        prep = getattr(self.opt, "prepare_capture", None)
        if prep is not None:
            prep()
        self.graph = torch.cuda.CUDAGraph()
        self.opt.zero_grad(set_to_none=True)
        with _gc_paused(), torch.cuda.graph(self.graph, capture_error_mode=mode):
            self.loss, self.out = self._body(zero=False)
            self.stats = self._stats
        fin = getattr(self.opt, "finish_capture", None)
        if fin is not None:
            fin()

    def _body(self, zero=True):
        if zero:
            self.opt.zero_grad(set_to_none=True)
        with torch.autocast("cuda", dtype=self.dtype or torch.float32, enabled=self.dtype is not None):
            out = self.model(self.x)
        if self.metrics:
            if self.crit is bce_loss:
                loss, self._stats = bce_loss_stats(out, self.t)
            elif hasattr(self.crit, "loss_stats"):
                loss, self._stats = self.crit.loss_stats(out, self.t)
            else:
                raise ValueError("GraphedTrainStep(metrics=True) needs criterion=csu.train.bce_loss or one with a "
                                 "loss_stats method (csu.losses.SegLoss)")
        else:
            loss, self._stats = self.crit(out, self.t), None
        loss.backward()
        if self.reducer is not None:
            self.reducer.finish()
        _clip_for(self.opt)
        self.opt.step()
        _ema_for(self.opt)
        return loss.detach(), out.detach()

    def __call__(self, x, t):
        self.x.copy_(x, non_blocking=True)
        self.t.copy_(t, non_blocking=True)
        if not self.capture:
            self.loss, self.out = self._body()
            self.stats = self._stats
            return self.loss, self.out
        sync_shadows(self.model)
        self.graph.replay()
        return self.loss, self.out


def make_scheduler(optimizer, factor=0.5, patience=5, min_lr=1e-7):
    return torch.optim.lr_scheduler.ReduceLROnPlateau(optimizer, mode="min", factor=factor, patience=patience,
                                                      min_lr=min_lr)
```

### include/csu.h

```cpp
#ifndef CSU_H_
#define CSU_H_

#include <stddef.h>
#include <stdint.h>

#ifdef __cplusplus
extern "C" {
#endif

enum csu_dtype { CSU_F32 = 0, CSU_BF16 = 1 };

enum csu_status {
    CSU_OK = 0,
    CSU_E_ARG = -1,
    CSU_E_UNSUPPORTED = -2,
    CSU_E_WORKSPACE = -3
};

const char* csu_last_error_string(void);
const char* csu_build_info(void);

int csu_event_create(void** event);
int csu_event_destroy(void* event);
int csu_event_record_ext(void* event, void* stream);
// ... 32 lines not shown
                        void* workspace, size_t workspace_bytes, void* stream);
int csu_stripe_lepe_wgrad(const csu_stripe_args* a, int dtype, const void* qkv, const void* dout,
                          void* workspace, size_t workspace_bytes, void* stream);
int csu_stripe_attn_bwd_ex(const csu_stripe_args* a, int dtype, const void* qkv, const void* out, const void* dout,
                           const float* lse, float* delta, void* dqkv, void* workspace, size_t workspace_bytes,
                           int lepe_deferred, void* stream);
int csu_stripe_lepe_nblk(const csu_stripe_args* a, int dtype);
typedef struct {
    const float* part;
    float* dw[2];
    float* db[2];
    int32_t nblk, channels, nbranch, _pad;
} csu_lepe_reduce_item;
int csu_stripe_lepe_reduce_batch(const csu_lepe_reduce_item* items, int count, void* stream);

int csu_layernorm_fwd(int rows, int C, float eps, int xdtype, const void* x, const float* gamma,
                      const float* beta, int ydtype, void* y, float* mean, float* rstd, void* stream);
size_t csu_layernorm_bwd_workspace(int rows, int C);
int csu_layernorm_bwd(int rows, int C, int xdtype, const void* x, const float* gamma,
                      const float* mean, const float* rstd, int dydtype, const void* dy,
                      void* dx, float* dgamma, float* dbeta, void* workspace, size_t ws_bytes,
                      void* stream);
int csu_layernorm_bwd_ex(int rows, int C, int xdtype, const void* x, const float* gamma,
                         const float* mean, const float* rstd, int dydtype, const void* dy,
                         const float* dres, void* dx, void* dx_bf16, float* dgamma, float* dbeta,
                         void* workspace, size_t ws_bytes, void* stream);

int csu_layernorm_param_reduce(int rows, int C, const void* workspace, float* dgamma, float* dbeta, void* stream);
typedef struct {
    const void* workspace;
    float* dgamma;
    float* dbeta;
    int32_t rows, C;
    int32_t nblocks;
    int32_t _pad;
} csu_ln_param_item;
int csu_layernorm_param_reduce_batch(const csu_ln_param_item* items, int count, void* stream);

size_t csu_simam_workspace(int B, int L, int C);
int csu_simam_fwd(int B, int L, int C, float lambda, int xdtype, const void* x, int ydtype, void* y, float* stats,
                  void* workspace, size_t ws_bytes, void* stream);
int csu_simam_bwd(int B, int L, int C, int xdtype, const void* x, const float* stats, int gdtype, const void* dy,
                  void* dx, void* workspace, size_t ws_bytes, void* stream);
int csu_simam_fwd_fork(int B, int L, int C, float lambda, const float* x, void* y, void* xc, float* stats,
                       void* workspace, size_t ws_bytes, void* stream);
int csu_simam_bwd_join(int B, int L, int C, const float* x, const float* stats, int gdtype, const void* dy,
                       const void* g2, float* dx, void* dxb, void* workspace, size_t ws_bytes, void* stream);

int csu_carafe_fwd(int B, int H, int W, int C, int s, int dtype, const void* x, const void* enc,
                   void* out, float* wsave, void* stream);
int csu_carafe_bwd(int B, int H, int W, int C, int s, int dtype, const void* x, const float* wsave,
                   const void* dout, void* dx, void* denc, void* stream);

int csu_head_fwd(long P, int C, int dtype, const void* x, const float* w, float* prob, void* stream);
size_t csu_head_bwd_workspace(long P, int C);
int csu_head_bwd(long P, int C, int dtype, const void* x, const float* w, const float* prob,
                 const float* dprob, void* dx, float* dw, void* workspace, size_t ws_bytes, void* stream);

int csu_carafe_head_fwd(int B, int H, int W, int C, int s, int dtype, const void* x, const void* enc,
                        const float* u, const float* cb, float* z, float* prob, void* stream);
size_t csu_carafe_head_bwd_workspace(int B, int H, int W, int C, int s);
int csu_carafe_head_bwd(int B, int H, int W, int C, int s, int dtype, const void* x, const void* enc,
                        const float* z, const float* u, const float* prob, const float* dprob, void* dx,
                        void* denc, float* du, float* dcb, void* workspace, size_t ws_bytes, void* stream);
int csu_head_fold_fwd(int O, int C, const float* w_out, const float* b_out, const float* w_h, float* u, float* cb,
                      void* stream);
typedef struct {
    int32_t O;
    const float* w_out;
    const float* b_out;
    const float* w_h;
    float* dw_out;
    float* db_out;
    float* dw_h;
} csu_head_fold;
int csu_carafe_head_bwd_fold(int B, int H, int W, int C, int s, int dtype, const void* x, const void* enc,
                             const float* z, const float* u, const float* prob, const float* dprob, void* dx,
                             void* denc, float* du, const csu_head_fold* fold, void* workspace, size_t ws_bytes,
                             void* stream);

size_t csu_colsum_workspace(long rows, long cols, int dtype);
int csu_colsum(long rows, long cols, int dtype, const void* in, float* out, void* workspace,
               size_t ws_bytes, void* stream);

size_t csu_linear_wgrad_workspace(long M, int N, int K);
int csu_linear_wgrad(long M, int N, int K, int dtype, const void* dy, const void* x, float* dw_db,
                     void* workspace, size_t ws_bytes, void* stream);
typedef struct {
    const float* slab;
    float* dst;
    int32_t N, K, tn, tk, chunks, _pad;
} csu_wslab_item;
int csu_linear_wgrad_deferred(long M, int N, int K, const void* dy, const void* x, float* dw_db,
                              void* workspace, size_t ws_bytes, csu_wslab_item* item, void* stream);
int csu_wslab_reduce_batch(const csu_wslab_item* items, int count, void* stream);
typedef struct {
    const void* dy;
    const void* x;
    float* dw_db;
    float* slab;
    int64_t M;
    int32_t N, K;
} csu_wgrad_group_item;
size_t csu_linear_wgrad_group_plan(long M, int N, int K, int* tn, int* tk, int* chunks);
int csu_linear_wgrad_group(const csu_wgrad_group_item* items, int count, void* stream);
size_t csu_linear_wgrad_tuned_workspace(long M, int N, int K, int tn, int tk, int chunks);
int csu_linear_wgrad_tuned(long M, int N, int K, int dtype, const void* dy, const void* x, float* dw_db,
                           void* workspace, size_t ws_bytes, int tn, int tk, int chunks, void* stream);

int csu_gemm(long M, int N, int K, const void* a, int lda, const void* b, int ldb, int b_trans, int a_gelu,
             const float* bias, const void* gelu_aux, const float* resid, void* out, int ldc, int out_dtype,
             void* stream);
typedef struct {
    int64_t M;
    int32_t N, K;
    const void* a;
    const void* b;
    int32_t lda, ldb;
    int32_t b_trans, a_gelu;
    const float* bias;
    const void* gelu_aux;
    const float* resid;
    void* out;
    void* gelu_out;
    int32_t ldc, out_dtype;
    int32_t cfg, _pad;
} csu_gemm_desc;
int csu_gemm_ex(const csu_gemm_desc* d, void* stream);

int csu_gemm_ws_ln_supported(long M, int C, int K);
int csu_gemm_ws_ln(long M, int C, const void* x, int ldx, const void* w_frag, const float* bias, const float* resid,
                   float* out, const float* gamma, const float* beta, float eps, void* ln_out, float* mean, float* rstd,
                   void* stream);

int csu_gemm_ws_supported(long M, int N, int K, int resid, int out_dtype);
int csu_gemm_ws(long M, int N, int K, const void* x, int ldx, const void* w_frag, const float* bias, const float* resid,
                int out_dtype, void* out, void* stream);
int csu_gemm_ws_lnbwd_supported(long M, int C, int K);
int csu_gemm_ws_lnbwd(long M, int C, int K, const void* dy, const void* wt_frag, const float* x, const float* gamma,
                      const float* mean, const float* rstd, const float* dres, float* dx, void* dx_bf16, float* part,
                      void* stream);
typedef struct {
    const void* src;
    void* dst;
    int32_t rows, cols;
    int64_t chunk0;
} csu_frag_item;
int csu_frag_layout_batch(const csu_frag_item* items, int count, long total_chunks, void* stream);

int csu_gemm_ws_e4m3(long M, int N, int K, const void* x, int ldx, const void* w_frag8, const float* w_scale,
                     int scale_mode, const float* bias, const float* resid, int out_dtype, void* out, void* stream);
int csu_gemm_ws_ln_e4m3(long M, int C, const void* x, int ldx, const void* w_frag8, const float* w_scale,
                        const float* bias, const float* resid, float* out, const float* gamma, const float* beta,
                        float eps, void* ln_out, float* mean, float* rstd, void* stream);
typedef struct {
    const void* src;
    void* dst;
    int32_t N, K;
    int32_t transpose, _pad;
    int64_t block0;
} csu_frag8_item;
int csu_frag8_layout_batch(const csu_frag8_item* items, int count, long total_blocks, void* stream);

typedef struct {
    const float* src;
    void* dst;
    void* dst_t;
    int32_t rows, cols;
    int64_t tile0;
    int32_t taps;
    int32_t cols_pad;
} csu_cast_item;
int csu_cast_bf16_batch(const csu_cast_item* items, int count, long total_tiles, void* stream);

typedef struct {
    const float* src;
    float* dst;
    uint8_t* dst_q;
// ... 77 lines not shown
int csu_rng_advance(uint64_t* state, uint64_t* snap, void* stream);
int csu_droppath_scale(long n, const uint64_t* rng, unsigned site, float p, float* out, void* stream);

size_t csu_gemm_f32_workspace(int layout, long M, int N, long K);
int csu_gemm_f32(int layout, long M, int N, long K, const float* A, const float* B, const float* bias,
                 const float* resid, float* C, float* asum, void* workspace, size_t ws_bytes, void* stream);

int csu_mlp_supported(int C);
int csu_mlp_fwd(long M, int C, const void* x, const void* w1, const float* b1, const void* w2, const float* b2,
                const float* res, float* out, void* stream);
int csu_mlp_bwd(long M, int C, const void* x, const void* dy, const void* w1, const float* b1, const void* w2,
                void* dh, void* g, void* dx, void* stream);
typedef struct {
    const uint64_t* rng;
    uint32_t site_hidden, site_out;
    float p;
    const float* row_scale;
    int64_t rows_per_sample;
} csu_mlp_dropout;
int csu_mlp_fwd_dp(long M, int C, const void* x, const void* w1, const float* b1, const void* w2, const float* b2,
                   const float* res, float* out, const csu_mlp_dropout* d, void* stream);
int csu_mlp_bwd_dp(long M, int C, const void* x, const void* dy, const void* w1, const float* b1, const void* w2,
                   void* dh, void* g, void* dx, const csu_mlp_dropout* d, void* stream);
int csu_mlp_bwd_ln_supported(long M, int C);
int csu_mlp_bwd_ln(long M, int C, const void* h, const void* dy, const void* w1, const float* b1, const void* w2,
                   void* dh, void* g, long rows_per_image, const float* x, const float* gamma, const float* mean,
                   const float* rstd, const float* dres, float* dx, void* dx_bf16, float* part, void* stream);
int csu_mlp_bwd_wgrad_supported(int C);
int csu_mlp_bwd_wgrad_workspace(long M, int C, size_t* slab1_bytes, size_t* slab2_bytes);
int csu_mlp_bwd_wgrad(long M, int C, const void* x, const void* dy, const void* w1, const float* b1, const void* w2,
                      void* dx, const csu_mlp_dropout* d, float* slab1, float* slab2, csu_wslab_item* item1,
                      csu_wslab_item* item2, float* dw1_db1, float* dw2_db2, void* stream);
int csu_mlp_fwd_ln(long M, int C, const void* x, const void* w1, const float* b1, const void* w2, const float* b2,
                   const float* res, float* out, const csu_mlp_dropout* d, const float* ln_gamma, const float* ln_beta,
                   float ln_eps, void* ln_out, float* ln_mean, float* ln_rstd, void* stream);
int csu_mlp_fwd_ex(long M, int C, const void* x, const void* w1, const float* b1, const void* w2, const float* b2,
                   const float* res, float* out, const csu_mlp_dropout* d, int cfg, void* stream);
int csu_mlp_bwd_ex(long M, int C, const void* x, const void* dy, const void* w1, const float* b1, const void* w2,
                   void* dh, void* g, void* dx, const csu_mlp_dropout* d, int cfg, void* stream);
int csu_mlp_fp8_supported(int C);
int csu_mlp_fp8_fwd(long M, int C, const void* x, const void* w1q, const float* sw1, const float* b1,
                    const void* w2p, const float* sw2, const float* b2, const float* res, float* out,
                    const csu_mlp_dropout* d, void* stream);
int csu_mlp_fp8_fwd_ln(long M, int C, const void* x, const void* w1q, const float* sw1, const float* b1,
                       const void* w2p, const float* sw2, const float* b2, const float* res, float* out,
                       const csu_mlp_dropout* d, const float* ln_gamma, const float* ln_beta, float ln_eps, void* ln_out,
                       float* ln_mean, float* ln_rstd, void* stream);
int csu_mlp_fp8_bwd(long M, int C, const void* x, const void* dy, const void* w1q, const float* sw1,
                    const float* b1, const void* w2t, const float* sw2, const void* w1tp, void* dh, void* g,
                    void* dx, const csu_mlp_dropout* d, void* stream);

typedef struct {
    int32_t B, H, W, C;
    int32_t OH, OW, N;
    int32_t KH, KW, stride, pad;
} csu_conv_geom;

int csu_conv2d_fwd(const csu_conv_geom* g, int dtype, const void* x, const void* w_ohwi, const float* bias,
                   void* y, void* stream);
int csu_conv2d_dgrad(const csu_conv_geom* g, int dtype, const void* dy, const void* w_ihwo, const float* bias,
                     void* dx, void* stream);
int csu_conv2d_ex(int op, const csu_conv_geom* g, int dtype, const void* src, const void* w, const float* bias, void* out,
                  int cfg, void* stream);
size_t csu_conv2d_workspace(int op, const csu_conv_geom* g, int dtype);
int csu_conv2d_fwd_ws(const csu_conv_geom* g, int dtype, const void* x, const void* w_ohwi, const float* bias, void* y,
                      void* workspace, size_t ws_bytes, void* stream);
int csu_conv2d_dgrad_ws(const csu_conv_geom* g, int dtype, const void* dy, const void* w_ihwo, const float* bias,
                        void* dx, void* workspace, size_t ws_bytes, void* stream);
size_t csu_conv2d_wgrad_workspace(const csu_conv_geom* g);
int csu_conv2d_wgrad(const csu_conv_geom* g, int dtype, const void* x, const void* dy, float* dw_db,
                     void* workspace, size_t ws_bytes, void* stream);
int csu_conv2d_wgrad_oihw(const csu_conv_geom* g, int dtype, const void* x, const void* dy, int c_real, float* dw_db,
                          void* workspace, size_t ws_bytes, void* stream);
size_t csu_conv2d_wgrad_workspace_ex(const csu_conv_geom* g, int cfg);
int csu_conv2d_split_ok(const csu_conv_geom* g, int c_split);
int csu_conv2d_fwd_split(const csu_conv_geom* g, int dtype, const void* x, const void* x2, int c_split, const void* w_ohwi,
                         const float* bias, void* y, void* stream);
int csu_conv2d_dgrad_split(const csu_conv_geom* g, int dtype, const void* dy, const void* w_ihwo, void* dx, void* dx2,
                           int c_split, void* stream);
int csu_conv2d_wgrad_split_oihw(const csu_conv_geom* g, int dtype, const void* x, const void* x2, int c_split, const void* dy,
                                float* dw_db, void* workspace, size_t ws_bytes, void* stream);
int csu_conv2d_wgrad_ex(const csu_conv_geom* g, int dtype, const void* x, const void* dy, int c_real, float* dw_db,
                        void* workspace, size_t ws_bytes, int cfg, void* stream);

int csu_grad_join(long n, int adtype, const void* a, int bdtype, const void* b, float* out, void* out_bf16,
                  void* stream);
size_t csu_bce_loss_workspace(long n);
int csu_bce_loss_fwd(long n, const float* p, const float* t, float* loss, void* workspace, size_t ws_bytes,
                     void* stream);
int csu_bce_loss_fwd_stats(long n, const float* p, const float* t, float* loss, float* stats, void* workspace,
                           size_t ws_bytes, void* stream);
int csu_bce_loss_bwd(long n, const float* p, const float* t, const float* dloss, float* dp, void* stream);
int csu_pack_nhwc_bf16(int B, int C, int H, int W, int Cp, const float* x, void* y, void* stream);

size_t csu_seg_loss_workspace(long n, int rows);
int csu_seg_loss_fwd(long n, int rows, const float* p, const float* t, float w_bce, float pos_weight, float w_tversky,
                     float alpha, float beta, float smooth, float* loss, float* stats, float* coef, void* workspace,
                     size_t ws_bytes, void* stream);
int csu_seg_loss_bwd(long n, int rows, const float* p, const float* t, const float* dloss, const float* coef,
                     float w_bce, float pos_weight, float w_tversky, float* dp, void* stream);

size_t csu_seg_ce_workspace(int B, int K, long HW);
int csu_seg_ce_fwd(int B, int K, long HW, int rows, int dtype, const void* z, long s_b, long s_k, long s_pix, int pad_ok,
                   int label_dtype, const void* t, long ignore_index, const float* class_weight, float w_ce,
                   float w_tversky, float alpha, float beta, float smooth, int include_background, float* loss,
                   double* stats, float* coef, void* workspace, size_t ws_bytes, void* stream);
int csu_seg_ce_bwd(int B, int K, long HW, int rows, int dtype, const void* z, long s_b, long s_k, long s_pix, int pad_ok,
                   int label_dtype, const void* t, long ignore_index, const float* class_weight, const float* dloss,
                   const float* coef, float w_ce, float w_tversky, int include_background, void* dz, void* stream);

size_t csu_seg_bd_workspace(int B, int K, long HW);
int csu_seg_bd_fwd(int B, int K, long HW, int rows, int dtype, const void* z, long s_b, long s_k, long s_pix, int pad_ok,
                   int label_dtype, const void* t, long ignore_index, const float* class_weight, float w_ce,
                   float w_tversky, float alpha, float beta, float smooth, int include_background, const float* phi,
                   const float* w_bd, int bd_background, float* loss, float* terms, double* stats, float* coef,
                   void* workspace, size_t ws_bytes, void* stream);
int csu_seg_bd_bwd(int B, int K, long HW, int rows, int dtype, const void* z, long s_b, long s_k, long s_pix, int pad_ok,
                   int label_dtype, const void* t, long ignore_index, const float* class_weight, const float* dloss,
                   const float* coef, float w_ce, float w_tversky, int include_background, const float* phi,
                   const float* w_bd, int bd_background, void* dz, void* stream);

int csu_augment_batch(int B, int S, const void* img, const void* mask, const int* params, float* out_img,
                      float* out_mask, void* stream);

#define CSU_AUGMENT_P 20
enum csu_augment_border { CSU_AUG_CONSTANT = 0, CSU_AUG_REPLICATE = 1 };
enum csu_augment_mask_mode { CSU_AUG_MASK_BILINEAR = 0, CSU_AUG_MASK_NEAREST = 1, CSU_AUG_MASK_LABELS = 2 };
typedef struct {
    float p_hflip, p_vflip, p_rot90;
    float p_rotate, rotate_lo, rotate_hi;
    float p_scale, scale_lo, scale_hi;
    float p_translate, translate_x, translate_y;
    float p_contrast, contrast_lo, contrast_hi;
    float p_brightness, brightness_lo, brightness_hi;
    float p_gamma, gamma_lo, gamma_hi;
    float p_noise, noise_lo, noise_hi;
    float p_elastic, elastic_lo, elastic_hi;
    int32_t spacing;
} csu_augment_config;
int csu_augment_draw(const csu_augment_config* cfg, int B, int H, int W, const uint64_t* rng, unsigned site,
                     unsigned site_ctrl, float* table, float* ctrl, void* stream);
int csu_augment_mean(int B, long n, const void* img, uint64_t* sums, float* mean, void* stream);
int csu_augment_warp(int B, int H, int W, const void* img, const void* mask, const float* table, const float* ctrl,
                     int spacing, const float* mean, const uint64_t* rng, unsigned noise_site, int border,
                     float image_fill, int pad_label, int mask_mode, float* out_img, void* out_mask, void* stream);

enum csu_tile_src { CSU_TILE_SRC_U8_HWC = 0, CSU_TILE_SRC_F32_CHW = 1 };
enum csu_tile_form { CSU_TILE_PROB = 0, CSU_TILE_LOGITS = 1 };
int csu_tile_gather(int B, int S, int H, int W, int src_kind, const void* image, const int* table, float* out,
                    void* stream);
int csu_tile_blend(int B, int S, int H, int W, int K, int form, int dtype, const void* z, long s_b, long s_k, long s_pix,
                   int pad_ok, const int* table, const float* w1, float* canvas, int ry0, int rx0, int ry1, int rx1,
                   void* stream);
int csu_tile_finish(int K, int H, int W, const float* canvas, const float* ry, const float* rx, float n_tta, float* prob,
                    void* labels, void* stream);

enum csu_surface_dtype { CSU_SURFACE_U8 = 0, CSU_SURFACE_I64 = 1 };
enum csu_surface_mode { CSU_SURFACE_LABELS = 0, CSU_SURFACE_BINARY = 1 };
size_t csu_surface_workspace(int B, int C, int H, int W);
int csu_surface_metrics(int B, int C, int H, int W, int mode, int class0, int pred_dtype, const void* pred,
                        int target_dtype, const void* target, double sy, double sx, double tolerance, double percentile,
                        void* workspace, size_t ws_bytes, double* out, int out_classes, int out_c0, void* stream);
size_t csu_edt_workspace(int B, int H, int W);
int csu_edt(int B, int H, int W, int dtype, const void* mask, double sy, double sx, void* workspace, size_t ws_bytes,
            float* out, void* stream);

size_t csu_signed_distance_workspace(int B, int C, int H, int W);
int csu_signed_distance(int B, int C, int H, int W, int class0, int dtype, const void* labels, double sy, double sx,
                        double clip, void* workspace, size_t ws_bytes, float* out, int out_classes, int out_c0,
                        void* stream);

enum csu_cc_connectivity { CSU_CC_4 = 4, CSU_CC_8 = 8 };
size_t csu_ccl_workspace(int B, int H, int W);
int csu_ccl(int B, int H, int W, int dtype, const void* labels, int connectivity, void* workspace, size_t ws_bytes,
            int* comp, int* area, int* count, void* stream);
size_t csu_cc_filter_workspace(int B, int H, int W);
// ... 20 lines not shown
```

Measured before the change: 1604 images/sec.

## Batch deferred conv wgrad reductions and read graph inputs through pointer slots

Conv weight-gradient column-sum reductions can now be deferred and run as batched multi-item pass1/pass2 kernels, cutting per-layer launch count. The wslab reduction gains a leading-dimension variant. The graphed train step also gets device-side pointer slots, so the input pack and BCE kernels read the caller's x and t directly instead of copying them into static buffers each step. This removes two input copies and many small launches, at the cost of an extra slot-setting kernel and more complex capture and aliasing logic.

Result: no change. 1611 images/sec, median of 6 (+0.4%).

```diff
diff --git a/cswin-simam-unet_amd/csrc/conv.hip b/cswin-simam-unet_amd/csrc/conv.hip
--- a/cswin-simam-unet_amd/csrc/conv.hip
+++ b/cswin-simam-unet_amd/csrc/conv.hip
@@ -1736,7 +1736,8 @@
 }
 
 static int conv_wgrad_impl(const csu_conv_geom* gm, int dtype, const void* x, const void* dy, int creal, float* dw_db,
-                           void* workspace, size_t ws_bytes, int cfg, void* stream, const void* x2 = nullptr, int csplit = 0) {
+                           void* workspace, size_t ws_bytes, int cfg, void* stream, const void* x2 = nullptr, int csplit = 0,
+                           csu_colsum_item* defer = nullptr) {
     if (int e = check_geo(gm)) return e;
     if (!x || !dy || !dw_db) return fail(CSU_E_ARG, "conv2d_wgrad: null buffer");
     const int pick = wd_pick(gm, dtype, cfg);
@@ -1772,6 +1773,10 @@
         return fail(CSU_E_ARG, "conv2d_wgrad: bad dtype");
     }
     if (int e = check_launch("conv2d_wgrad")) return e;
+    if (defer) {
+        *defer = csu_colsum_item{part, dw_db, part + (size_t)p.chunks * slab, p.chunks, slab, 1, g.N, g.KH * g.KW, g.C, creal, 0};
+        return 0;
+    }
     if (creal > 0) {
         const OutMap om{1, g.N, g.KH * g.KW, g.C, creal};
         return colsum_launch(p.chunks, slab, CSU_F32, part, dw_db, part + (size_t)p.chunks * slab, st, &om);
@@ -1799,6 +1804,13 @@
                                    void* workspace, size_t ws_bytes, int cfg, void* stream) {
     if (c_real < 0) return fail(CSU_E_ARG, "conv2d_wgrad_ex: c_real < 0");
     return conv_wgrad_impl(gm, dtype, x, dy, c_real, dw_db, workspace, ws_bytes, cfg, stream);
+}
+
+extern "C" int csu_conv2d_wgrad_deferred(const csu_conv_geom* gm, int dtype, const void* x, const void* dy, int c_real,
+                                         float* dw_db, void* workspace, size_t ws_bytes, int cfg, csu_colsum_item* item,
+                                         void* stream) {
+    if (c_real < 1 || !item) return fail(CSU_E_ARG, "conv2d_wgrad_deferred: c_real < 1 or null item");
+    return conv_wgrad_impl(gm, dtype, x, dy, c_real, dw_db, workspace, ws_bytes, cfg, stream, nullptr, 0, item);
 }
 
 extern "C" int csu_conv2d_split_ok(const csu_conv_geom* gm, int c_split) {
diff --git a/cswin-simam-unet_amd/csrc/glue.hip b/cswin-simam-unet_amd/csrc/glue.hip
--- a/cswin-simam-unet_amd/csrc/glue.hip
+++ b/cswin-simam-unet_amd/csrc/glue.hip
@@ -34,8 +34,9 @@
 
 constexpr int BCE_BLOCKS = 1024;
 
-__global__ __launch_bounds__(NT) void bce_partial(long n, const float* __restrict__ p, const float* __restrict__ t,
-                                                  float* __restrict__ partial, int stats) {
+__global__ __launch_bounds__(NT) void bce_partial(long n, const float* __restrict__ p, const float* t_arg,
+                                                  const float* const* tslot, float* __restrict__ partial, int stats) {
+    const float* __restrict__ t = tslot ? *tslot : t_arg;
     __shared__ float red[4][NT / 64];
     const long per = (n + gridDim.x - 1) / gridDim.x;
     const long b0 = (long)blockIdx.x * per, b1 = min(n, b0 + per);
@@ -90,8 +91,10 @@
     }
 }
 
-__global__ __launch_bounds__(NT) void bce_backward(long n, const float* __restrict__ p, const float* __restrict__ t,
-                                                   const float* __restrict__ dloss, float* __restrict__ dp) {
+__global__ __launch_bounds__(NT) void bce_backward(long n, const float* __restrict__ p, const float* t_arg,
+                                                   const float* const* tslot, const float* __restrict__ dloss,
+                                                   float* __restrict__ dp) {
+    const float* __restrict__ t = tslot ? *tslot : t_arg;
     const float g = dloss[0], inv = 1.f / (float)n;
     for (long e = (long)blockIdx.x * NT + threadIdx.x; e < n; e += (long)gridDim.x * NT) {
         const float pv = p[e];
@@ -99,8 +102,9 @@
     }
 }
 
-__global__ __launch_bounds__(NT) void pack_nhwc(long pixels, int C, int Cp, long hw, const float* __restrict__ x,
-                                                bf16* __restrict__ y) {
+__global__ __launch_bounds__(NT) void pack_nhwc(long pixels, int C, int Cp, long hw, const float* x_arg,
+                                                const float* const* xslot, bf16* __restrict__ y) {
+    const float* __restrict__ x = xslot ? *xslot : x_arg;
     for (long q = (long)blockIdx.x * NT + threadIdx.x; q < pixels; q += (long)gridDim.x * NT) {
         const long b = q / hw, s = q - b * hw;
         const float* src = x + b * C * hw + s;
@@ -111,6 +115,11 @@
             *reinterpret_cast<bf16x8*>(y + q * Cp + c0) = v;
         }
     }
+}
+
+__global__ void ptr_slots_set(const void** slots, const void* a, const void* b) {
+    if (threadIdx.x == 0) slots[0] = a;
+    if (threadIdx.x == 1) slots[1] = b;
 }
 
 unsigned grid_for(long work) {
@@ -137,13 +146,13 @@
 extern "C" size_t csu_bce_loss_workspace(long n) { return (size_t)4 * BCE_BLOCKS * sizeof(float); }
 
 static int bce_fwd(long n, const float* p, const float* t, float* loss, float* stats, void* workspace, size_t ws_bytes,
-                   void* stream) {
-    if (n < 1 || !p || !t || !loss) return fail(CSU_E_ARG, "bce_loss_fwd: bad args");
+                   void* stream, const float* const* tslot = nullptr) {
+    if (n < 1 || !p || (!t && !tslot) || !loss) return fail(CSU_E_ARG, "bce_loss_fwd: bad args");
     if (!workspace || ws_bytes < csu_bce_loss_workspace(n)) return fail(CSU_E_WORKSPACE, "bce_loss_fwd: workspace");
     const long want = (n + 4 * NT - 1) / (4 * NT);
     const int nb = (int)(want < BCE_BLOCKS ? want : BCE_BLOCKS);
     hipStream_t st = as_stream(stream);
-    bce_partial<<<nb, NT, 0, st>>>(n, p, t, (float*)workspace, stats != nullptr);
+    bce_partial<<<nb, NT, 0, st>>>(n, p, t, tslot, (float*)workspace, stats != nullptr);
     if (int e = check_launch("bce_loss_fwd")) return e;
     bce_final<<<1, NT, 0, st>>>(nb, n, (const float*)workspace, loss, stats);
     return check_launch("bce_loss_fwd");
@@ -162,13 +171,40 @@
 
 extern "C" int csu_bce_loss_bwd(long n, const float* p, const float* t, const float* dloss, float* dp, void* stream) {
     if (n < 1 || !p || !t || !dloss || !dp) return fail(CSU_E_ARG, "bce_loss_bwd: bad args");
-    bce_backward<<<grid_for(n), NT, 0, as_stream(stream)>>>(n, p, t, dloss, dp);
+    bce_backward<<<grid_for(n), NT, 0, as_stream(stream)>>>(n, p, t, nullptr, dloss, dp);
     return check_launch("bce_loss_bwd");
+}
+
+extern "C" int csu_bce_loss_fwd_stats_ind(long n, const float* p, const float* const* t_slot, float* loss, float* stats,
+                                          void* workspace, size_t ws_bytes, void* stream) {
+    if (!stats || !t_slot) return fail(CSU_E_ARG, "bce_loss_fwd_stats_ind: null stats or slot");
+    return bce_fwd(n, p, nullptr, loss, stats, workspace, ws_bytes, stream, t_slot);
+}
+
+extern "C" int csu_bce_loss_bwd_ind(long n, const float* p, const float* const* t_slot, const float* dloss, float* dp,
+                                    void* stream) {
+    if (n < 1 || !p || !t_slot || !dloss || !dp) return fail(CSU_E_ARG, "bce_loss_bwd_ind: bad args");
+    bce_backward<<<grid_for(n), NT, 0, as_stream(stream)>>>(n, p, nullptr, t_slot, dloss, dp);
+    return check_launch("bce_loss_bwd_ind");
+}
+
+extern "C" int csu_ptr_slots_set(void* slots, const void* a, const void* b, void* stream) {
+    if (!slots) return fail(CSU_E_ARG, "ptr_slots_set: null slots");
+    ptr_slots_set<<<1, 64, 0, as_stream(stream)>>>((const void**)slots, a, b);
+    return check_launch("ptr_slots_set");
 }
 
 extern "C" int csu_pack_nhwc_bf16(int B, int C, int H, int W, int Cp, const float* x, void* y, void* stream) {
     if (B < 1 || C < 1 || H < 1 || W < 1 || Cp < C || Cp % 8 || !x || !y) return fail(CSU_E_ARG, "pack_nhwc_bf16: bad args");
     const long pixels = (long)B * H * W;
-    pack_nhwc<<<grid_for(pixels), NT, 0, as_stream(stream)>>>(pixels, C, Cp, (long)H * W, x, (bf16*)y);
+    pack_nhwc<<<grid_for(pixels), NT, 0, as_stream(stream)>>>(pixels, C, Cp, (long)H * W, x, nullptr, (bf16*)y);
     return check_launch("pack_nhwc_bf16");
 }
+
+extern "C" int csu_pack_nhwc_bf16_ind(int B, int C, int H, int W, int Cp, const float* const* x_slot, void* y, void* stream) {
+    if (B < 1 || C < 1 || H < 1 || W < 1 || Cp < C || Cp % 8 || !x_slot || !y)
+        return fail(CSU_E_ARG, "pack_nhwc_bf16_ind: bad args");
+    const long pixels = (long)B * H * W;
+    pack_nhwc<<<grid_for(pixels), NT, 0, as_stream(stream)>>>(pixels, C, Cp, (long)H * W, nullptr, x_slot, (bf16*)y);
+    return check_launch("pack_nhwc_bf16_ind");
+}
diff --git a/cswin-simam-unet_amd/csrc/reduce.hip b/cswin-simam-unet_amd/csrc/reduce.hip
--- a/cswin-simam-unet_amd/csrc/reduce.hip
+++ b/cswin-simam-unet_amd/csrc/reduce.hip
@@ -14,13 +14,13 @@
 }
 
 template <typename T>
-__global__ __launch_bounds__(NT) void colsum_pass1(long rows, long cols, int tpr, long rows_per_chunk,
-                                                   const T* __restrict__ in, float* __restrict__ out, OutMap om) {
+__device__ __forceinline__ void pass1_body(unsigned bx, unsigned by, long rows, long cols, int tpr, long rows_per_chunk,
+                                           const T* __restrict__ in, float* __restrict__ out, const OutMap& om) {
     constexpr int V = 16 / sizeof(T);
     __shared__ float red[NT][V + 1];
     const int cl = threadIdx.x % tpr, rl = threadIdx.x / tpr, rpi = NT / tpr;
-    const long c0 = ((long)blockIdx.x * tpr + cl) * V;
-    const long r0 = (long)blockIdx.y * rows_per_chunk;
+    const long c0 = ((long)bx * tpr + cl) * V;
+    const long r0 = (long)by * rows_per_chunk;
     const long r1 = min(rows, r0 + rows_per_chunk);
     float acc[V];
 #pragma unroll
@@ -65,7 +65,7 @@
                 if (d >= 0) out[d] = acc[j];
             }
         } else {
-            float* o = out + (long)blockIdx.y * cols + c0;
+            float* o = out + (long)by * cols + c0;
 #pragma unroll
             for (int j = 0; j < V; ++j)
                 if (c0 + j < cols) o[j] = acc[j];
@@ -73,11 +73,17 @@
     }
 }
 
-__global__ __launch_bounds__(NT) void colsum_pass2(long cols, int nchunks, const float* __restrict__ part,
-                                                   float* __restrict__ out, OutMap om) {
+template <typename T>
+__global__ __launch_bounds__(NT) void colsum_pass1(long rows, long cols, int tpr, long rows_per_chunk,
+                                                   const T* __restrict__ in, float* __restrict__ out, OutMap om) {
+    pass1_body<T>(blockIdx.x, blockIdx.y, rows, cols, tpr, rows_per_chunk, in, out, om);
+}
+
+__device__ __forceinline__ void pass2_body(unsigned bx, long cols, int nchunks, const float* __restrict__ part,
+                                           float* __restrict__ out, const OutMap& om) {
     __shared__ float red[8][33];
     const int cl = threadIdx.x & 31, lane = threadIdx.x >> 5;
-    const long c = (long)blockIdx.x * 32 + cl;
+    const long c = (long)bx * 32 + cl;
     float s0 = 0.f, s1 = 0.f;
     if (c < cols) {
         int k = lane;
@@ -95,6 +101,44 @@
         const long d = out_index(om, c);
         if (d >= 0) out[d] = s;
     }
+}
+
+__global__ __launch_bounds__(NT) void colsum_pass2(long cols, int nchunks, const float* __restrict__ part,
+                                                   float* __restrict__ out, OutMap om) {
+    pass2_body(blockIdx.x, cols, nchunks, part, out, om);
+}
+
+constexpr int CSB_MAX = 24;
+struct CsBatch1 {
+    const float* in[CSB_MAX];
+    float* out[CSB_MAX];
+    long rows[CSB_MAX], cols[CSB_MAX], rpc[CSB_MAX];
+    OutMap om[CSB_MAX];
+    int tpr[CSB_MAX], colblocks[CSB_MAX], b0[CSB_MAX + 1];
+    int count;
+};
+struct CsBatch2 {
+    const float* part[CSB_MAX];
+    float* out[CSB_MAX];
+    long cols[CSB_MAX];
+    OutMap om[CSB_MAX];
+    int nchunks[CSB_MAX], b0[CSB_MAX + 1];
+    int count;
+};
+
+__global__ __launch_bounds__(NT) void colsum_batch_pass1(CsBatch1 t) {
+    const int b = blockIdx.x;
+    int i = 0;
+    while (i + 1 < t.count && t.b0[i + 1] <= b) ++i;
+    const unsigned l = (unsigned)(b - t.b0[i]), cb = (unsigned)t.colblocks[i];
+    pass1_body<float>(l % cb, l / cb, t.rows[i], t.cols[i], t.tpr[i], t.rpc[i], t.in[i], t.out[i], t.om[i]);
+}
+
+__global__ __launch_bounds__(NT) void colsum_batch_pass2(CsBatch2 t) {
+    const int b = blockIdx.x;
+    int i = 0;
+    while (i + 1 < t.count && t.b0[i + 1] <= b) ++i;
+    pass2_body((unsigned)(b - t.b0[i]), t.cols[i], t.nchunks[i], t.part[i], t.out[i], t.om[i]);
 }
 
 struct Plan {
@@ -150,6 +194,67 @@
 
 extern "C" size_t csu_colsum_workspace(long rows, long cols, int dtype) { return colsum_workspace(rows, cols, dtype); }
 
+extern "C" int csu_colsum_batch(const csu_colsum_item* items, int count, void* stream) {
+    if (count < 0 || (count && !items)) return fail(CSU_E_ARG, "colsum_batch: bad args");
+    hipStream_t st = as_stream(stream);
+    for (int i = 0; i < count; ++i) {
+        const csu_colsum_item& it = items[i];
+        if (it.rows < 1 || it.cols < 1 || it.cols % 4 || !it.in || !it.out) return fail(CSU_E_ARG, "colsum_batch: bad item");
+        if (plan(it.rows, it.cols, 4).chunks > 1 && !it.ws) return fail(CSU_E_WORKSPACE, "colsum_batch: item needs a workspace");
+    }
+    CsBatch1 t;
+    t.count = 0;
+    t.b0[0] = 0;
+    auto flush1 = [&]() -> int {
+        if (!t.count) return 0;
+        colsum_batch_pass1<<<(unsigned)t.b0[t.count], NT, 0, st>>>(t);
+        t.count = 0;
+        return check_launch("colsum_batch");
+    };
+    for (int i = 0; i < count; ++i) {
+        const csu_colsum_item& it = items[i];
+        const Plan p = plan(it.rows, it.cols, 4);
+        const long blocks = (long)p.colblocks * p.chunks;
+        if (t.count == CSB_MAX || (long)t.b0[t.count] + blocks > (1L << 30))
+            if (int e = flush1()) return e;
+        const int c = t.count;
+        t.in[c] = it.in;
+        t.out[c] = p.chunks > 1 ? it.ws : it.out;
+        t.rows[c] = it.rows; t.cols[c] = it.cols; t.rpc[c] = p.rpc;
+        t.om[c] = p.chunks > 1 ? OutMap{0, 0, 0, 0, 0} : OutMap{it.map_on, it.N, it.khw, it.C, it.creal};
+        t.tpr[c] = p.tpr; t.colblocks[c] = p.colblocks;
+        t.b0[c + 1] = t.b0[c] + (int)blocks;
+        t.count = c + 1;
+    }
+    if (int e = flush1()) return e;
+    CsBatch2 u;
+    u.count = 0;
+    u.b0[0] = 0;
+    auto flush2 = [&]() -> int {
+        if (!u.count) return 0;
+        colsum_batch_pass2<<<(unsigned)u.b0[u.count], NT, 0, st>>>(u);
+        u.count = 0;
+        return check_launch("colsum_batch");
+    };
+    for (int i = 0; i < count; ++i) {
+        const csu_colsum_item& it = items[i];
+        const Plan p = plan(it.rows, it.cols, 4);
+        if (p.chunks <= 1) continue;
+        const long blocks = (it.cols + 31) / 32;
+        if (u.count == CSB_MAX || (long)u.b0[u.count] + blocks > (1L << 30))
+            if (int e = flush2()) return e;
+        const int c = u.count;
+        u.part[c] = it.ws;
+        u.out[c] = it.out;
+        u.cols[c] = it.cols;
+        u.om[c] = OutMap{it.map_on, it.N, it.khw, it.C, it.creal};
+        u.nchunks[c] = p.chunks;
+        u.b0[c + 1] = u.b0[c] + (int)blocks;
+        u.count = c + 1;
+    }
+    return flush2();
+}
+
 extern "C" int csu_colsum(long rows, long cols, int dtype, const void* in, float* out, void* workspace,
                           size_t ws_bytes, void* stream) {
     if (rows < 1 || cols < 1 || !in || !out) return fail(CSU_E_ARG, "colsum: bad args");
diff --git a/cswin-simam-unet_amd/csrc/wgrad.hip b/cswin-simam-unet_amd/csrc/wgrad.hip
--- a/cswin-simam-unet_amd/csrc/wgrad.hip
+++ b/cswin-simam-unet_amd/csrc/wgrad.hip
@@ -1,3 +1,4 @@
+#include <cstdint>
 #include <cstdlib>
 #include <type_traits>
 
@@ -328,7 +329,8 @@
 }
 
 __device__ __forceinline__ void wslab_sum(long blk, int N, int K, int TN, int TK, int chunks,
-                                          const float* __restrict__ slab, float* __restrict__ dst) {
+                                          const float* __restrict__ slab, float* __restrict__ dst, int ldd,
+                                          float* __restrict__ dstb) {
     __shared__ f32x4 red[NT];
     const int G = wslab_groups(chunks), QB = NT / G;
     const int g = threadIdx.x / QB, qi = threadIdx.x % QB;
@@ -338,16 +340,19 @@
     const long step = (long)TN * TK;
     const float* p = slab;
     long stride = 0;
-    const bool valid = e < NK + N;
+    const bool valid = e < NK || (e < NK + N && dstb);
+    float* o = dst;
     if (e < NK) {
         const int n = (int)(e / K), k = (int)(e % K);
         const long tile = (long)(n / TN) * kt + k / TK;
         p = slab + tile * chunks * step + (long)(n % TN) * TK + (k % TK);
         stride = step;
+        o = dst + (long)n * ldd + k;
     } else if (valid) {
         const int n = (int)(e - NK);
         p = slab + (long)nt * kt * chunks * step + ((long)(n / TN) * chunks) * TN + (n % TN);
         stride = TN;
+        o = dstb + n;
     }
     f32x4 a0 = {}, a1 = {}, a2 = {}, a3 = {};
     if (valid) {
@@ -362,7 +367,7 @@
     }
     const f32x4 s = (a0 + a1) + (a2 + a3);
     if (G == 1) {
-        if (valid) *reinterpret_cast<f32x4*>(dst + e) = s;
+        if (valid) *reinterpret_cast<f32x4*>(o) = s;
         return;
     }
     red[threadIdx.x] = s;
@@ -370,20 +375,21 @@
     if (g == 0 && valid) {
         f32x4 t = red[qi];
         for (int j = 1; j < G; ++j) t += red[j * QB + qi];
-        *reinterpret_cast<f32x4*>(dst + e) = t;
+        *reinterpret_cast<f32x4*>(o) = t;
     }
 }
 
 __global__ __launch_bounds__(NT) void wslab_reduce(int N, int K, int TN, int TK, int chunks,
                                                    const float* __restrict__ slab, float* __restrict__ dst) {
-    wslab_sum(blockIdx.x, N, K, TN, TK, chunks, slab, dst);
+    wslab_sum(blockIdx.x, N, K, TN, TK, chunks, slab, dst, K, dst + (long)N * K);
 }
 
 constexpr int WSB_MAX = 40;
 struct WsBatch {
     const float* slab[WSB_MAX];
     float* dst[WSB_MAX];
-    int N[WSB_MAX], K[WSB_MAX], tn[WSB_MAX], tk[WSB_MAX], chunks[WSB_MAX], b0[WSB_MAX + 1];
+    float* dstb[WSB_MAX];
+    int N[WSB_MAX], K[WSB_MAX], tn[WSB_MAX], tk[WSB_MAX], chunks[WSB_MAX], ldd[WSB_MAX], b0[WSB_MAX + 1];
     int count;
 };
 
@@ -391,7 +397,7 @@
     const int b = blockIdx.x;
     int i = 0;
     while (i + 1 < t.count && t.b0[i + 1] <= b) ++i;
-    wslab_sum(b - t.b0[i], t.N[i], t.K[i], t.tn[i], t.tk[i], t.chunks[i], t.slab[i], t.dst[i]);
+    wslab_sum(b - t.b0[i], t.N[i], t.K[i], t.tn[i], t.tk[i], t.chunks[i], t.slab[i], t.dst[i], t.ldd[i], t.dstb[i]);
 }
 
 int num_cus() {
@@ -633,8 +639,8 @@
     return 0;
 }
 
-extern "C" int csu_wslab_reduce_batch(const csu_wslab_item* items, int count, void* stream) {
-    if (count < 0 || (count && !items)) return fail(CSU_E_ARG, "wslab_reduce_batch: bad args");
+template <typename Get>
+static int wslab_reduce_batch_impl(int count, Get get, void* stream) {
     WsBatch t;
     t.count = 0;
     t.b0[0] = 0;
@@ -645,20 +651,38 @@
         return check_launch("wslab_reduce_batch");
     };
     for (int i = 0; i < count; ++i) {
-        const csu_wslab_item& it = items[i];
+        const csu_wslab_item_ld it = get(i);
         if (it.chunks <= 1) continue;
-        if (!it.slab || !it.dst || it.N % 4 || it.K % 4) return fail(CSU_E_ARG, "wslab_reduce_batch: bad item");
+        if (!it.slab || !it.dst || it.N % 4 || it.K % 4 || it.ldd < it.K) return fail(CSU_E_ARG, "wslab_reduce_batch: bad item");
         const long blocks = wslab_blocks(it.N, it.K, it.chunks);
         if (t.count == WSB_MAX || (long)t.b0[t.count] + blocks > (1L << 30))
             if (int e = flush()) return e;
         const int c = t.count;
         t.slab[c] = it.slab;
         t.dst[c] = it.dst;
-        t.N[c] = it.N; t.K[c] = it.K; t.tn[c] = it.tn; t.tk[c] = it.tk; t.chunks[c] = it.chunks;
+        t.dstb[c] = it.dst_b;
+        t.N[c] = it.N; t.K[c] = it.K; t.tn[c] = it.tn; t.tk[c] = it.tk; t.chunks[c] = it.chunks; t.ldd[c] = it.ldd;
         t.b0[c + 1] = t.b0[c] + (int)blocks;
         t.count = c + 1;
     }
     return flush();
+}
+
+extern "C" int csu_wslab_reduce_batch(const csu_wslab_item* items, int count, void* stream) {
+    if (count < 0 || (count && !items)) return fail(CSU_E_ARG, "wslab_reduce_batch: bad args");
+    return wslab_reduce_batch_impl(count, [&](int i) {
+        const csu_wslab_item& it = items[i];
+        return csu_wslab_item_ld{it.slab, it.dst, it.dst ? it.dst + (long)it.N * it.K : nullptr, it.N, it.K, it.tn, it.tk,
+                                 it.chunks, it.K};
+    }, stream);
+}
+
+extern "C" int csu_wslab_reduce_batch_ld(const csu_wslab_item_ld* items, int count, void* stream) {
+    if (count < 0 || (count && !items)) return fail(CSU_E_ARG, "wslab_reduce_batch_ld: bad args");
+    for (int i = 0; i < count; ++i)
+        if (items[i].ldd % 4 || ((uintptr_t)items[i].dst & 15) || ((uintptr_t)items[i].dst_b & 15))
+            return fail(CSU_E_ARG, "wslab_reduce_batch_ld: destination rows must be 16-byte aligned");
+    return wslab_reduce_batch_impl(count, [&](int i) { return items[i]; }, stream);
 }
 
 #ifdef WG_TIMING
diff --git a/cswin-simam-unet_amd/csu/_lib.py b/cswin-simam-unet_amd/csu/_lib.py
--- a/cswin-simam-unet_amd/csu/_lib.py
+++ b/cswin-simam-unet_amd/csu/_lib.py
@@ -32,6 +32,16 @@
 class WslabItem(ctypes.Structure):
     _fields_ = [("slab", c_void_p), ("dst", c_void_p), ("N", c_int32), ("K", c_int32), ("tn", c_int32), ("tk", c_int32),
                 ("chunks", c_int32), ("_pad", c_int32)]
+
+
+class WslabItemLd(ctypes.Structure):
+    _fields_ = [("slab", c_void_p), ("dst", c_void_p), ("dst_b", c_void_p), ("N", c_int32), ("K", c_int32), ("tn", c_int32),
+                ("tk", c_int32), ("chunks", c_int32), ("ldd", c_int32)]
+
+
+class ColsumItem(ctypes.Structure):
+    _fields_ = [("src", c_void_p), ("out", c_void_p), ("ws", c_void_p), ("rows", ctypes.c_int64), ("cols", ctypes.c_int64),
+                ("map_on", c_int32), ("N", c_int32), ("khw", c_int32), ("C", c_int32), ("creal", c_int32), ("_pad", c_int32)]
 
 
 class WgradGroupItem(ctypes.Structure):
@@ -195,6 +205,7 @@
     "csu_linear_wgrad_deferred": (ctypes.c_int, [ctypes.c_long, ctypes.c_int, ctypes.c_int, c_void_p, c_void_p, c_void_p,
                                                  c_void_p, c_size_t, ctypes.POINTER(WslabItem), c_void_p]),
     "csu_wslab_reduce_batch": (ctypes.c_int, [c_void_p, ctypes.c_int, c_void_p]),
+    "csu_wslab_reduce_batch_ld": (ctypes.c_int, [c_void_p, ctypes.c_int, c_void_p]),
     "csu_stripe_attn_bwd_ex": (ctypes.c_int, [ctypes.POINTER(StripeArgs), ctypes.c_int, c_void_p, c_void_p, c_void_p,
                                               c_void_p, c_void_p, c_void_p, c_void_p, c_size_t, ctypes.c_int, c_void_p]),
     "csu_stripe_lepe_nblk": (ctypes.c_int, [ctypes.POINTER(StripeArgs), ctypes.c_int]),
@@ -245,6 +256,9 @@
     "csu_bce_loss_fwd": (ctypes.c_int, [ctypes.c_long, c_void_p, c_void_p, c_void_p, c_void_p, c_size_t, c_void_p]),
     "csu_bce_loss_fwd_stats": (ctypes.c_int, [ctypes.c_long] + [c_void_p] * 5 + [c_size_t, c_void_p]),
     "csu_bce_loss_bwd": (ctypes.c_int, [ctypes.c_long, c_void_p, c_void_p, c_void_p, c_void_p, c_void_p]),
+    "csu_bce_loss_fwd_stats_ind": (ctypes.c_int, [ctypes.c_long] + [c_void_p] * 5 + [c_size_t, c_void_p]),
+    "csu_bce_loss_bwd_ind": (ctypes.c_int, [ctypes.c_long, c_void_p, c_void_p, c_void_p, c_void_p, c_void_p]),
+    "csu_ptr_slots_set": (ctypes.c_int, [c_void_p] * 4),
     "csu_seg_loss_workspace": (c_size_t, [ctypes.c_long, ctypes.c_int]),
     "csu_seg_loss_fwd": (ctypes.c_int, [ctypes.c_long, ctypes.c_int, c_void_p, c_void_p] + [c_float] * 6
                          + [c_void_p] * 4 + [c_size_t, c_void_p]),
@@ -267,6 +281,8 @@
                           c_void_p]),
     "csu_pack_nhwc_bf16": (ctypes.c_int, [ctypes.c_int, ctypes.c_int, ctypes.c_int, ctypes.c_int, ctypes.c_int, c_void_p,
                                           c_void_p, c_void_p]),
+    "csu_pack_nhwc_bf16_ind": (ctypes.c_int, [ctypes.c_int, ctypes.c_int, ctypes.c_int, ctypes.c_int, ctypes.c_int, c_void_p,
+                                              c_void_p, c_void_p]),
     "csu_stripe_lepe_wgrad": (ctypes.c_int, [ctypes.POINTER(StripeArgs), ctypes.c_int, c_void_p, c_void_p, c_void_p, c_size_t,
                                              c_void_p]),
     "csu_mlp_fwd": (ctypes.c_int, [ctypes.c_long, ctypes.c_int, c_void_p, c_void_p, c_void_p, c_void_p, c_void_p, c_void_p,
@@ -308,6 +324,10 @@
                                            c_void_p, c_void_p, c_size_t, ctypes.c_int, c_void_p]),
     "csu_conv2d_wgrad": (ctypes.c_int, [ctypes.POINTER(ConvGeom), ctypes.c_int, c_void_p, c_void_p, c_void_p, c_void_p,
                                         c_size_t, c_void_p]),
+    "csu_conv2d_wgrad_deferred": (ctypes.c_int, [ctypes.POINTER(ConvGeom), ctypes.c_int, c_void_p, c_void_p, ctypes.c_int,
+                                                 c_void_p, c_void_p, c_size_t, ctypes.c_int, ctypes.POINTER(ColsumItem),
+                                                 c_void_p]),
+    "csu_colsum_batch": (ctypes.c_int, [c_void_p, ctypes.c_int, c_void_p]),
     "csu_conv2d_wgrad_oihw": (ctypes.c_int, [ctypes.POINTER(ConvGeom), ctypes.c_int, c_void_p, c_void_p, ctypes.c_int,
                                              c_void_p, c_void_p, c_size_t, c_void_p]),
 }
diff --git a/cswin-simam-unet_amd/csu/ops.py b/cswin-simam-unet_amd/csu/ops.py
--- a/cswin-simam-unet_amd/csu/ops.py
+++ b/cswin-simam-unet_amd/csu/ops.py
@@ -288,7 +288,7 @@
 
 
 def deferred_pending() -> bool:
-    return bool(_LN_PENDING or _WG_DEFER or _WG_PENDING or _WG_POST or _LEPE_PENDING)
+    return bool(_LN_PENDING or _WG_DEFER or _WG_PENDING or _WG_POST or _LEPE_PENDING or _CS_PENDING)
 
 
 def _ln_param_reduce(pend, nbytes):
@@ -364,16 +364,22 @@
 _WG_PENDING: list = []
 _WG_DEFER: list = []
 _WG_POST: list = []
+DEFER_CONV_WGRAD = os.environ.get("CSU_DEFER_CONV_WGRAD", "1") != "0"
+CONCAT_INPLACE = os.environ.get("CSU_CONCAT_INPLACE", "1") != "0"
+_CS_PENDING: list = []
 
 
 def _wgrad_flush():
     defer, _WG_DEFER[:] = list(_WG_DEFER), []
+    pend_ld = []
     if defer:
         L = lib()
         dev = defer[0][0].device
         gitems = (_lib.WgradGroupItem * len(defer))()
         keep, flops, nbytes = [], 0, 0
-        for i, (dy2, x2, out) in enumerate(defer):
+        for i, ent in enumerate(defer):
+            dy2, x2, out = ent[:3]
+            place = ent[3] if len(ent) > 3 else None
             M, N = dy2.shape
             K = x2.shape[1]
             tn, tk, ch = ctypes.c_int(), ctypes.c_int(), ctypes.c_int()
@@ -383,7 +389,13 @@
             it = gitems[i]
             it.dy, it.x, it.dw_db, it.slab, it.M, it.N, it.K = dy2.data_ptr(), x2.data_ptr(), out.data_ptr(), \
                 (slab.data_ptr() if slab is not None else None), M, N, K
-            if ch.value > 1:
+            if place is not None:
+                assert ch.value > 1
+                w = _lib.WslabItemLd()
+                w.slab, w.dst, w.dst_b, w.ldd = slab.data_ptr(), place[0], place[1], place[2]
+                w.N, w.K, w.tn, w.tk, w.chunks = N, K, tn.value, tk.value, ch.value
+                pend_ld.append((w, out, slab))
+            elif ch.value > 1:
                 w = _lib.WslabItem()
                 w.slab, w.dst, w.N, w.K, w.tn, w.tk, w.chunks = slab.data_ptr(), out.data_ptr(), N, K, tn.value, tk.value, \
                     ch.value
@@ -391,18 +403,32 @@
             flops += 2 * M * N * K
             nbytes += M * (N + K) * 2 + (N * K + N) * 4
         _launch("linear_wgrad", lambda: L.csu_linear_wgrad_group(gitems, len(defer), stream_ptr(dev)), flops, nbytes)
+    _colsum_flush()
     pend, _WG_PENDING[:] = list(_WG_PENDING), []
+    for pl, struct, fn in ((pend, _lib.WslabItem, "csu_wslab_reduce_batch"), (pend_ld, _lib.WslabItemLd, "csu_wslab_reduce_batch_ld")):
+        if not pl:
+            continue
+        dev = pl[0][1].device
+        items = (struct * len(pl))()
+        nbytes = 0
+        for i, (it, out, work) in enumerate(pl):
+            items[i] = it
+            nbytes += it.chunks * (it.N * it.K + it.N) * 4 + (it.N * it.K + it.N) * 4
+        _launch("linear_wgrad", lambda: getattr(lib(), fn)(items, len(pl), stream_ptr(dev)), 0, nbytes)
+    _wgrad_post()
+
+
+def _colsum_flush():
+    pend, _CS_PENDING[:] = list(_CS_PENDING), []
     if not pend:
-        _wgrad_post()
         return
     dev = pend[0][1].device
-    items = (_lib.WslabItem * len(pend))()
+    items = (_lib.ColsumItem * len(pend))()
     nbytes = 0
     for i, (it, out, work) in enumerate(pend):
         items[i] = it
-        nbytes += it.chunks * (it.N * it.K + it.N) * 4 + (it.N * it.K + it.N) * 4
-    _launch("linear_wgrad", lambda: lib().csu_wslab_reduce_batch(items, len(pend), stream_ptr(dev)), 0, nbytes)
-    _wgrad_post()
+        nbytes += (it.rows * it.cols + out.numel()) * 4
+    _launch("conv_wgrad", lambda: lib().csu_colsum_batch(items, len(pend), stream_ptr(dev)), 0, nbytes)
 
 
 def _wgrad_post():
@@ -1121,6 +1147,17 @@
     return out
 
 
+_INPUT_SLOTS: dict = {}
+
+
+def _input_slot(t: torch.Tensor):
+    e = _INPUT_SLOTS.get(t.data_ptr()) if _INPUT_SLOTS else None
+    if e is None or t.dtype != torch.float32 or not t.is_contiguous():
+        return None
+    e[1] += 1
+    return e[0]
+
+
 class _BCELossFn(torch.autograd.Function):
 
     @staticmethod
@@ -1131,7 +1168,11 @@
         stats = torch.empty(3, dtype=torch.float32, device=p.device) if with_stats else None
         nws = lib().csu_bce_loss_workspace(n)
         ws = torch.empty(nws // 4, dtype=torch.float32, device=p.device)
-        if with_stats:
+        ctx.t_slot = slot = _input_slot(t) if with_stats else None
+        if slot is not None:
+            _launch("bce_loss", lambda: lib().csu_bce_loss_fwd_stats_ind(n, ptr(p), slot, ptr(loss), ptr(stats), ptr(ws), nws,
+                                                                         stream_ptr(p.device)), 12 * n, 8 * n, prec="f32")
+        elif with_stats:
             _launch("bce_loss", lambda: lib().csu_bce_loss_fwd_stats(n, ptr(p), ptr(t), ptr(loss), ptr(stats), ptr(ws), nws,
                                                                      stream_ptr(p.device)), 12 * n, 8 * n, prec="f32")
         else:
@@ -1149,8 +1190,12 @@
         g = g.float().contiguous()
         dp = torch.empty_like(p)
         n = p.numel()
-        _launch("bce_loss_bwd", lambda: lib().csu_bce_loss_bwd(n, ptr(p), ptr(t), ptr(g), ptr(dp), stream_ptr(p.device)),
-                6 * n, 12 * n, prec="f32")
+        if ctx.t_slot is not None:
+            _launch("bce_loss_bwd", lambda: lib().csu_bce_loss_bwd_ind(n, ptr(p), ctx.t_slot, ptr(g), ptr(dp),
+                                                                       stream_ptr(p.device)), 6 * n, 12 * n, prec="f32")
+        else:
+            _launch("bce_loss_bwd", lambda: lib().csu_bce_loss_bwd(n, ptr(p), ptr(t), ptr(g), ptr(dp), stream_ptr(p.device)),
+                    6 * n, 12 * n, prec="f32")
         return dp, None, None
 
 
@@ -1531,6 +1576,22 @@
 
 
 def _concat_wgrad(dy2, a2, b2, defer: bool = False, dest=None):
+    if defer and CONCAT_INPLACE and GROUP_WGRAD and dy2.dtype == torch.bfloat16:
+        M, N = dy2.shape
+        Ka, Kb = a2.shape[1], b2.shape[1]
+        K = Ka + Kb
+        out = dest if dest is not None else torch.empty(N * K + N, dtype=torch.float32, device=dy2.device)
+        ch = ctypes.c_int()
+        chunked = N % 8 == 0 and Ka % 8 == 0 and Kb % 8 == 0 and M < 2 ** 31 and out.data_ptr() % 16 == 0
+        for k in (Ka, Kb):
+            chunked = chunked and lib().csu_linear_wgrad_group_plan(M, N, k, None, None, ctypes.byref(ch)) > 0 and ch.value > 1
+        if chunked:
+            dyc = dy2.contiguous()
+            base = out.data_ptr()
+            _WG_DEFER.append((dyc, a2.contiguous(), out, (base, base + N * K * 4, K)))
+            _WG_DEFER.append((dyc, b2.contiguous(), out, (base + Ka * 4, None, K)))
+            _queue_flush()
+            return out[:N * K].view(N, K), out[N * K:]
     dwa, db = linear_wgrad(dy2, a2, defer=defer)
     dwb, _ = linear_wgrad(dy2, b2, defer=defer)
     if not defer:
@@ -2603,17 +2664,24 @@
     return g
 
 
-def _conv_wgrad(g, x, dy, dt, c_real=None, out=None):
+def _conv_wgrad(g, x, dy, dt, c_real=None, out=None, defer=False):
     L = lib()
     cr = g.C if c_real is None else c_real
     if out is None:
         out = torch.empty(g.N * g.KH * g.KW * cr + g.N, dtype=torch.float32, device=x.device)
     n = L.csu_conv2d_wgrad_workspace(ctypes.byref(g))
     work = torch.empty(max(n, 16), dtype=torch.uint8, device=x.device)
-    _launch("conv_wgrad", lambda: L.csu_conv2d_wgrad_oihw(ctypes.byref(g), dt, ptr(x), ptr(dy), cr, ptr(out), ptr(work),
-                                                          n, stream_ptr(x.device)),
-            2 * g.B * g.OH * g.OW * g.N * g.KH * g.KW * g.C,
-            (g.B * g.H * g.W * g.C + g.B * g.OH * g.OW * g.N) * x.element_size() + out.numel() * 4, prec=prec_of(x))
+    flops = 2 * g.B * g.OH * g.OW * g.N * g.KH * g.KW * g.C
+    nbytes = (g.B * g.H * g.W * g.C + g.B * g.OH * g.OW * g.N) * x.element_size() + out.numel() * 4
+    if defer:
+        it = _lib.ColsumItem()
+        _launch("conv_wgrad", lambda: L.csu_conv2d_wgrad_deferred(ctypes.byref(g), dt, ptr(x), ptr(dy), cr, ptr(out), ptr(work),
+                                                                  n, -1, ctypes.byref(it), stream_ptr(x.device)),
+                flops, nbytes, prec=prec_of(x))
+        _CS_PENDING.append((it, out, work))
+    else:
+        _launch("conv_wgrad", lambda: L.csu_conv2d_wgrad_oihw(ctypes.byref(g), dt, ptr(x), ptr(dy), cr, ptr(out), ptr(work),
+                                                              n, stream_ptr(x.device)), flops, nbytes, prec=prec_of(x))
     k = g.N * g.KH * g.KW * cr
     return out[:k].view(g.N, cr, g.KH, g.KW), out[k:]
 
@@ -2642,8 +2710,15 @@
             xn = x.permute(0, 3, 1, 2)
             if cd == torch.bfloat16 and x.dtype == torch.float32 and xn.is_contiguous():
                 xc = torch.empty(B, H, W, cp, dtype=cd, device=x.device)
-                _launch("pack_nhwc", lambda: lib().csu_pack_nhwc_bf16(B, C, H, W, cp, ptr(xn), ptr(xc), stream_ptr(x.device)),
-                        0, x.numel() * 4 + xc.numel() * 2, prec="f32")
+                slot = _input_slot(xn)
+                if slot is not None:
+                    _launch("pack_nhwc", lambda: lib().csu_pack_nhwc_bf16_ind(B, C, H, W, cp, slot, ptr(xc),
+                                                                              stream_ptr(x.device)),
+                            0, x.numel() * 4 + xc.numel() * 2, prec="f32")
+                else:
+                    _launch("pack_nhwc", lambda: lib().csu_pack_nhwc_bf16(B, C, H, W, cp, ptr(xn), ptr(xc),
+                                                                          stream_ptr(x.device)),
+                            0, x.numel() * 4 + xc.numel() * 2, prec="f32")
             else:
                 xc = torch.zeros(B, H, W, cp, dtype=cd, device=x.device)
                 xc[..., :C] = x
@@ -2709,6 +2784,12 @@
             dw, db = _side_run(wg, xc, dy)
             _late((weight, ctx.bias), (dw, db if has_b else None), side=True)
             return dx, dw, (db if has_b else None), None, None, None
+        if (DEFER_CONV_WGRAD and dy.dtype == torch.bfloat16 and weight.dtype == torch.float32
+                and bdt in (None, torch.float32) and _deferrable(weight, ctx.bias)):
+            dw, db = _conv_wgrad(g, xc, dy, dtype_code(dy), C, out=dest, defer=True)
+            _late((weight, ctx.bias), (dw, db if has_b else None))
+            _queue_flush()
+            return dx, dw, (db if has_b else None), None, None, None
         dw, db = wg()
         return dx, dw.to(weight.dtype), (db.to(bdt) if has_b else None), None, None, None
 
diff --git a/cswin-simam-unet_amd/csu/train.py b/cswin-simam-unet_amd/csu/train.py
--- a/cswin-simam-unet_amd/csu/train.py
+++ b/cswin-simam-unet_amd/csu/train.py
@@ -3,6 +3,7 @@
 from typing import Dict, List, Optional
 
 import contextlib
+import os
 import gc
 import warnings
 
@@ -440,6 +441,14 @@
     return opt
 
 
+INPUT_SLOTS = os.environ.get("CSU_INPUT_SLOTS", "1") != "0"
+
+
+def _ops():
+    from . import ops
+    return ops
+
+
 class GraphedTrainStep:
 
     def __init__(self, model, optimizer, criterion, example_x, example_t, autocast_dtype=None, warmup=3,
@@ -453,6 +462,8 @@
         self.dtype = autocast_dtype
         self.capture = bool(capture)
         self.graph = None
+        self._slots = self._held = None
+        self._direct = False
         if not self.capture:
             for _ in range(warmup):
                 self._body()
@@ -482,9 +493,14 @@
             prep()
         self.graph = torch.cuda.CUDAGraph()
         self.opt.zero_grad(set_to_none=True)
-        with _gc_paused(), torch.cuda.graph(self.graph, capture_error_mode=mode):
-            self.loss, self.out = self._body(zero=False)
-            self.stats = self._stats
+        uses = self._register_slots()
+        try:
+            with _gc_paused(), torch.cuda.graph(self.graph, capture_error_mode=mode):
+                self.loss, self.out = self._body(zero=False)
+                self.stats = self._stats
+        finally:
+            _ops()._INPUT_SLOTS.clear()
+        self._direct = uses is not None and [u[1] for u in uses] == [1, 1]
         fin = getattr(self.opt, "finish_capture", None)
         if fin is not None:
             fin()
@@ -512,9 +528,43 @@
         _ema_for(self.opt)
         return loss.detach(), out.detach()
 
+    def _register_slots(self):
+        from .model import CSWinTransformer
+        if not (INPUT_SLOTS and isinstance(self.model, CSWinTransformer) and self.crit is bce_loss and self.metrics
+                and self.dtype == torch.bfloat16 and self._slot_ok(self.x, self.x) and self._slot_ok(self.t, self.t)):
+            return None
+        from ._lib import lib
+        from .ops import stream_ptr
+        self._slots = torch.zeros(2, dtype=torch.int64, device=self.x.device)
+        if lib().csu_ptr_slots_set(self._slots.data_ptr(), self.x.data_ptr(), self.t.data_ptr(), stream_ptr(self.x.device)):
+            raise RuntimeError(lib().csu_last_error_string())
+        torch.cuda.current_stream(self.x.device).synchronize()
+        base = self._slots.data_ptr()
+        uses = [[base, 0], [base + 8, 0]]
+        _ops()._INPUT_SLOTS.update({self.x.data_ptr(): uses[0], self.t.data_ptr(): uses[1]})
+        return uses
+
+    @staticmethod
+    def _slot_ok(v, like) -> bool:
+        return (isinstance(v, torch.Tensor) and v.is_cuda and v.device == like.device and v.dtype == torch.float32
+                and v.shape == like.shape and v.is_contiguous() and v.data_ptr() % 16 == 0 and not v.requires_grad)
+
+    def _point(self, x, t):
+        from ._lib import lib
+        from .ops import stream_ptr
+        if lib().csu_ptr_slots_set(self._slots.data_ptr(), x.data_ptr(), t.data_ptr(), stream_ptr(self.x.device)):
+            raise RuntimeError(lib().csu_last_error_string())
+
     def __call__(self, x, t):
-        self.x.copy_(x, non_blocking=True)
-        self.t.copy_(t, non_blocking=True)
+        if self._direct and self._slot_ok(x, self.x) and self._slot_ok(t, self.t):
+            self._point(x, t)
+            self._held = (x, t)
+        else:
+            self.x.copy_(x, non_blocking=True)
+            self.t.copy_(t, non_blocking=True)
+            if self._held is not None:
+                self._point(self.x, self.t)
+                self._held = None
         if not self.capture:
             self.loss, self.out = self._body()
             self.stats = self._stats
diff --git a/include/csu.h b/include/csu.h
--- a/include/csu.h
+++ b/include/csu.h
@@ -138,6 +138,14 @@
 size_t csu_colsum_workspace(long rows, long cols, int dtype);
 int csu_colsum(long rows, long cols, int dtype, const void* in, float* out, void* workspace,
                size_t ws_bytes, void* stream);
+typedef struct {
+    const float* in;
+    float* out;
+    float* ws;
+    int64_t rows, cols;
+    int32_t map_on, N, khw, C, creal, _pad;
+} csu_colsum_item;
+int csu_colsum_batch(const csu_colsum_item* items, int count, void* stream);
 
 size_t csu_linear_wgrad_workspace(long M, int N, int K);
 int csu_linear_wgrad(long M, int N, int K, int dtype, const void* dy, const void* x, float* dw_db,
@@ -150,6 +158,13 @@
 int csu_linear_wgrad_deferred(long M, int N, int K, const void* dy, const void* x, float* dw_db,
                               void* workspace, size_t ws_bytes, csu_wslab_item* item, void* stream);
 int csu_wslab_reduce_batch(const csu_wslab_item* items, int count, void* stream);
+typedef struct {
+    const float* slab;
+    float* dst;
+    float* dst_b;
+    int32_t N, K, tn, tk, chunks, ldd;
+} csu_wslab_item_ld;
+int csu_wslab_reduce_batch_ld(const csu_wslab_item_ld* items, int count, void* stream);
 typedef struct {
     const void* dy;
     const void* x;
@@ -393,6 +408,8 @@
                                 float* dw_db, void* workspace, size_t ws_bytes, void* stream);
 int csu_conv2d_wgrad_ex(const csu_conv_geom* g, int dtype, const void* x, const void* dy, int c_real, float* dw_db,
                         void* workspace, size_t ws_bytes, int cfg, void* stream);
+int csu_conv2d_wgrad_deferred(const csu_conv_geom* g, int dtype, const void* x, const void* dy, int c_real, float* dw_db,
+                              void* workspace, size_t ws_bytes, int cfg, csu_colsum_item* item, void* stream);
 
 int csu_grad_join(long n, int adtype, const void* a, int bdtype, const void* b, float* out, void* out_bf16,
                   void* stream);
@@ -403,6 +420,11 @@
                            size_t ws_bytes, void* stream);
 int csu_bce_loss_bwd(long n, const float* p, const float* t, const float* dloss, float* dp, void* stream);
 int csu_pack_nhwc_bf16(int B, int C, int H, int W, int Cp, const float* x, void* y, void* stream);
+int csu_bce_loss_fwd_stats_ind(long n, const float* p, const float* const* t_slot, float* loss, float* stats,
+                               void* workspace, size_t ws_bytes, void* stream);
+int csu_bce_loss_bwd_ind(long n, const float* p, const float* const* t_slot, const float* dloss, float* dp, void* stream);
+int csu_pack_nhwc_bf16_ind(int B, int C, int H, int W, int Cp, const float* const* x_slot, void* y, void* stream);
+int csu_ptr_slots_set(void* slots, const void* a, const void* b, void* stream);
 
 size_t csu_seg_loss_workspace(long n, int rows);
 int csu_seg_loss_fwd(long n, int rows, const float* p, const float* t, float w_bce, float pos_weight, float w_tversky,
```
